# Dengzhi-USTC/A-robust-registration-loss

Measured on AMD Instinct MI355X. Metric: point-pairs/sec for loss fwd+bwd at B=8, N=M=4096, higher is better.
Workload: dtype f32

## Files before the change

a-robust-registration-loss_amd/csrc/rrl_cull.hip:

```cpp
#include <stdio.h>
#include <stdlib.h>

#include "rrl_ws.h"

#include "rrl_tree.h"
#include "rrl_chamfer_walk.h"


struct BuildArgs {
    const float *tri1, *tri2;
    const float *R, *t;
    float *tri1_out;
    float *ptri1, *ptri2;
    float4 *crec1, *crec2;
    float *apart;
    float4 *p0s1, *p0s2;
    int32_t *idx1, *idx2;
    float4 *grp1, *grp2;
    uint32_t *pmax;
    uint4 *zero_base;
    size_t zero_vec4;
    uint4 *g1;
    size_t g1_vec4;
    uint4 *z2;
// ... 577 lines not shown
        g.scale[c] = ext > 0.0f && ext < 3.0e38f ? 15.999f / ext : 0.0f;
    }
    g.p2 = fmaxf(fmaxf(red[0][6], red[1][6]), fmaxf(red[2][6], red[3][6]));
    return g;
}

__device__ __forceinline__ unsigned grid_cell(const CellGrid &g, const float4 r) {
    const float p[3] = {r.x, r.y, r.z};
    unsigned q[3];
#pragma unroll
    for (int c = 0; c < 3; ++c) {
        float v = (p[c] - g.mn[c]) * g.scale[c];
        q[c] = v >= 15.0f ? 15u : (v > 0.0f ? (unsigned)v : 0u);
    }
    return hilbert_cell(q[0], q[1], q[2]);
}

__global__ __launch_bounds__(256) void big_hist_kernel(const BuildArgs a, unsigned *__restrict__ histg) {
    __shared__ float red[4][8];
    const int cloud = blockIdx.z, b = blockIdx.y;
    const int n = cloud ? a.M : a.N;
    if ((int)blockIdx.x * 256 >= n) return;
    const int ng = (n + GRP - 1) / GRP;
    const float4 *crec = (cloud ? a.crec2 : a.crec1) + (size_t)b * ng * GRP;
    const CellGrid g = load_grid(a, cloud, b, n, red);
    if (blockIdx.x == 0 && threadIdx.x == 0) a.pmax[cloud * a.B + b] = __float_as_uint(g.p2);
    const int f = blockIdx.x * 256 + threadIdx.x;
    if (f < n) atomicAdd(&histg[((size_t)(cloud * a.B + b) * 2) * SORT_CELLS + grid_cell(g, crec[f])], 1u);
}

__global__ __launch_bounds__(256) void big_scatter_kernel(const BuildArgs a, unsigned *__restrict__ histg) {
    __shared__ float red[4][8];
    __shared__ unsigned base[SORT_CELLS];
    __shared__ unsigned wsum[4];
    const int cloud = blockIdx.z, b = blockIdx.y, tid = threadIdx.x, lane = tid & 63, wave = tid >> 6;
    const int n = cloud ? a.M : a.N;
    if ((int)blockIdx.x * 256 >= n) return;
    const int ng = (n + GRP - 1) / GRP;
    const float4 *crec = (cloud ? a.crec2 : a.crec1) + (size_t)b * ng * GRP;
    const int npad = (n + SGT - 1) / SGT * SGT;
    float4 *p0s = (cloud ? a.p0s2 : a.p0s1) + (size_t)b * npad;
    int32_t *idx = (cloud ? a.idx2 : a.idx1) + (size_t)b * npad;
    unsigned *cnt = histg + ((size_t)(cloud * a.B + b) * 2) * SORT_CELLS, *cur = cnt + SORT_CELLS;
    const int f = blockIdx.x * 256 + tid;
    const float4 r = f < n ? crec[f] : make_float4(0.0f, 0.0f, 0.0f, 0.0f);
    {
        unsigned h[16], tsum = 0;
#pragma unroll
        for (int k = 0; k < 16; ++k) { h[k] = cnt[16 * tid + k]; tsum += h[k]; }
        const unsigned inc = (unsigned)wave_incl_scan((int)tsum);
        if (lane == 63) wsum[wave] = inc;
        __syncthreads();
        unsigned run = inc - tsum;
        for (int w = 0; w < wave; ++w) run += wsum[w];
#pragma unroll
        for (int k = 0; k < 16; ++k) { base[16 * tid + k] = run; run += h[k]; }
    }
    const CellGrid g = load_grid(a, cloud, b, n, red);
    if (f < n) {
        const unsigned c = grid_cell(g, r);
        const unsigned s = base[c] + atomicAdd(&cur[c], 1u);
        p0s[s] = r;
        idx[s] = f;
    }
    if (blockIdx.x == 0)
        for (int s = n + tid; s < npad; s += 256) { p0s[s] = make_float4(0.0f, 0.0f, 0.0f, 0.0f); idx[s] = 0; }
}

__global__ __launch_bounds__(256) void big_sphere_kernel(const BuildArgs a) {
    const int cloud = blockIdx.z, b = blockIdx.y;
    const int n = cloud ? a.M : a.N;
    const int nsg = (n + SGT - 1) / SGT;
    const int hh = blockIdx.x * 256 + threadIdx.x;
    if (hh >= nsg * 2 * SGG) return;
    const float4 *r = (cloud ? a.p0s2 : a.p0s1) + (size_t)b * nsg * SGT;
    half_tree([&](int s_) { return r[s_]; }, hh, n, (cloud ? a.grp2 : a.grp1) + (size_t)b * nsg * NODE);
}

typedef const float __attribute__((address_space(4))) * kptr;
typedef const int __attribute__((address_space(4))) * kiptr;

static BuildArgs make_build_args(const float *tri1, const float *tri2, void *ws, const WsLayout &w, int B, int N, int M,
                                 int clouds, const RrlXform *xf, const float *line, int L, const RrlCall &o, bool chunked);
static unsigned rrl_chain_spin_limit(void) {
    static long v = -1;
    if (v < 0) { const char *e = getenv("RRL_CHAIN_SPIN"); v = e ? atol(e) : (1l << 18); if (v < 0 || v > 0x7fffffffl) v = 1l << 18; }
    return (unsigned)v;
}

namespace scan8 {
#include "rrl_cull_scan.inc"
}
#undef SPW
#undef SG_BITS
#undef HF_BITS
#undef WPB
#undef LPW
#undef ROWS
#undef WCCAP
#undef QA_CAP
#undef QC_CAP
#undef CULL_REGLINES
#ifndef SCAN16_QA_CAP
#define SCAN16_QA_CAP 384
#endif
#ifndef SCAN16_QC_CAP
#define SCAN16_QC_CAP 256
#endif
#ifndef SCAN16_WCCAP
#define SCAN16_WCCAP 128
#endif
namespace scan16 {
#define SPW 16
#define CULL_REGLINES 1
#define QA_CAP SCAN16_QA_CAP
#define QC_CAP SCAN16_QC_CAP
#define WCCAP SCAN16_WCCAP
#include "rrl_cull_scan.inc"
}
static_assert(scan8::kWPB == scan16::kWPB && scan8::kLPW == scan16::kLPW, "one line tiling for both variants");

struct CullGeom {
    int waves, spw, tiles, slices;
    bool fat, may_ride;
};
static CullGeom cull_geometry(int B, int N, int M, int L, int clouds, const RrlCall &o) {
    constexpr int WPB_ = scan8::kWPB, LPW_ = scan8::kLPW;
    const int nmax = clouds == 2 && M > N ? M : N;
    const int nsgmax = (nmax + SGT - 1) / SGT;
    const int lw = (L + LPW_ - 1) / LPW_;
    int waves = lw < WPB_ ? lw : WPB_, spw = scan8::kSPW;
    auto wgs = [&]() { return (long)clouds * B * ((lw + waves - 1) / waves) * ((nsgmax + spw - 1) / spw); };
    bool fat = (long)clouds * B * ((lw + waves - 1) / waves) * ((nsgmax + 15) / 16) >= 896 && lw >= WPB_;
    if (const char *e = getenv("RRL_CULL_FAT")) fat = e[0] == '1' ? (nsgmax > 8) : (e[0] == '0' ? false : fat);
    if (fat) spw = scan16::kSPW;
    while (!fat && wgs() < 768 && spw > 1) spw >>= 1;
    const bool may_ride = o.rider && !o.counters && (clouds == 2 || o.tar_ws) && lw >= WPB_ && B <= 32767 && N > 0 && M > 0;
    while (!fat && !may_ride && wgs() < 256 && waves > 2) waves >>= 1;
#ifdef RRL_EXPERIMENT
    if (const char *e = getenv("RRL_CULL_GEOM")) {
        int w_ = 0, s_ = 0;
        if (sscanf(e, "%d,%d", &w_, &s_) == 2 && w_ >= 1 && w_ <= WPB_ && s_ >= 1 && s_ <= scan16::kSPW) {
            waves = w_ < lw ? w_ : lw; spw = s_; fat = s_ > scan8::kSPW;
        }
    }
#endif
    CullGeom g;
    g.waves = waves; g.spw = spw; g.fat = fat; g.may_ride = may_ride;
    g.tiles = (lw + waves - 1) / waves; g.slices = (nsgmax + spw - 1) / spw;
    return g;
}

int rrl_cull_scan_can_fuse(int B, int N, int M, int L, const RrlCall &o) {
    if (B <= 0 || N <= 0 || M <= 0 || L <= 0 || (N > M ? N : M) > SORT_CAP) return 0;
    if (o.rider || o.counters || o.problems || o.tar_ws) return 0;
    if (const char *e = getenv("RRL_CHAIN")) if (e[0] == '0') return 0;
    const CullGeom g = cull_geometry(B, N, M, L, 2, o);
    if (g.waves != scan8::kWPB) return 0;
    const int spw = g.spw, nsg1 = (N + SGT - 1) / SGT, nsg2 = (M + SGT - 1) / SGT;
    const int nrec_b = (int)(((size_t)nsg1 * SGT + 64 * scan8::kWPB - 1) / (64 * scan8::kWPB));
    const long total = (long)B * (nrec_b + (long)g.tiles * ((nsg1 + spw - 1) / spw + (nsg2 + spw - 1) / spw));
    if (g.fat && total > 4000) return 0;
    if (nrec_b > 8 && total < 2048) return 0;
    return 1;
}

int rrl_launch_cull_scan(const float *line, void *ws, const WsLayout &w, int B, int N, int M, int L,
// ... 186 lines not shown
```

a-robust-registration-loss_amd/csrc/rrl_sparse.hip:

```cpp
#include <stdlib.h>
#include <string.h>

#include "rrl_ws.h"

#define FIX_SHIFT 40

#ifdef RRL_STAMPS
__device__ unsigned long long g_stamps[32];
#define STAMP(i) do { if (threadIdx.x == 0 && blockIdx.x == 0 && blockIdx.y == 0 && blockIdx.z == 0) g_stamps[i] = wall_clock64(); } while (0)
extern "C" int rrl_debug_stamps(unsigned long long *out) {
    return hipMemcpyFromSymbol(out, HIP_SYMBOL(g_stamps), sizeof(unsigned long long) * 32) == hipSuccess ? 0 : -1;
}
__device__ unsigned long long g_wstamps[12 * 2048];
#define STAMPW(i) do { if ((threadIdx.x & 63) == 0) { const unsigned wg_ = blockIdx.x + gridDim.x * (blockIdx.y + gridDim.y * blockIdx.z); \
    if (wg_ < 2048u) g_wstamps[(i) * 2048 + wg_] = wall_clock64(); } } while (0)
extern "C" int rrl_debug_wstamps(unsigned long long *out, int clear) {
    if (clear) { void *p_ = nullptr; if (hipGetSymbolAddress(&p_, HIP_SYMBOL(g_wstamps)) != hipSuccess) return -1; return hipMemset(p_, 0, sizeof(unsigned long long) * 12 * 2048) == hipSuccess ? 0 : -1; }
    return hipMemcpyFromSymbol(out, HIP_SYMBOL(g_wstamps), sizeof(unsigned long long) * 12 * 2048) == hipSuccess ? 0 : -1;
}
__device__ unsigned long long g_pstamps[8 * 2048];
#define STAMPP(i) do { if ((threadIdx.x & 63) == 0) { const unsigned wg_ = blockIdx.x + gridDim.x * (blockIdx.y + gridDim.y * blockIdx.z); \
    if (wg_ < 2048u) g_pstamps[(i) * 2048 + wg_] = wall_clock64(); } } while (0)
extern "C" int rrl_debug_pstamps(unsigned long long *out, int clear) {
    if (clear) { void *p_ = nullptr; if (hipGetSymbolAddress(&p_, HIP_SYMBOL(g_pstamps)) != hipSuccess) return -1; return hipMemset(p_, 0, sizeof(unsigned long long) * 8 * 2048) == hipSuccess ? 0 : -1; }
    return hipMemcpyFromSymbol(out, HIP_SYMBOL(g_pstamps), sizeof(unsigned long long) * 8 * 2048) == hipSuccess ? 0 : -1;
}
#define STAMPC(i) STAMPP(i)
#else
#define STAMP(i)
#define STAMPW(i)
#define STAMPP(i)
#endif
#include "rrl_sampler.h"

#include "rrl_stage_pair.inc"

static PairArgs pair_args(const float *tri1, const float *tri2, const float *line, void *ws, const WsLayout &w, int B, int N,
                          int M, int L, int s_m, int s_n, int e_m, int e_n, bool tally = true, const void *tar_ws = nullptr,
                          int Bt = 0) {
    PairArgs a;
    a.mhist = tally ? w.u32(ws, RRL_WS_MHIST) : nullptr;
    a.mctl = tally ? w.u32(ws, RRL_WS_MCTL) : nullptr;
    a.tri1 = tri1;
    a.tri2 = tri2;
    a.line = line;
    a.count1 = w.i32(ws, RRL_WS_COUNT1); a.hit1 = w.i32(ws, RRL_WS_HIT1);
    a.count2 = tar_ws ? w.i32(tar_ws, RRL_WS_COUNT2) : w.i32(ws, RRL_WS_COUNT2);
    a.hit2 = tar_ws ? w.i32(tar_ws, RRL_WS_HIT2) : w.i32(ws, RRL_WS_HIT2);
    a.kj = w.u8(ws, RRL_WS_KJ);
    a.sel_out = w.i32(ws, RRL_WS_SEL); a.nsel = w.i32(ws, RRL_WS_NSEL);
    a.hs1 = w.i32(ws, RRL_WS_HS1); a.hs2 = w.i32(ws, RRL_WS_HS2);
    a.w1 = w.f32(ws, RRL_WS_W1); a.w2 = w.f32(ws, RRL_WS_W2);
    a.Q1 = (float4 *)w.f32(ws, RRL_WS_Q1); a.Q2 = (float4 *)w.f32(ws, RRL_WS_Q2);
    a.D = w.f32(ws, RRL_WS_D); a.dc = w.f32(ws, RRL_WS_VALS);
    a.kjc = w.u8(ws, RRL_WS_KJC); a.blkcnt = w.i32(ws, RRL_WS_BLKCNT);
    a.lidc = w.u32(ws, RRL_WS_LIDC);
    a.vlist = w.f32(ws, RRL_WS_VLIST); a.vlcnt = w.i32(ws, RRL_WS_VLCNT);
    a.B = B; a.N = N; a.M = M; a.L = L;
    a.s_m = s_m; a.s_n = s_n; a.e_m = e_m; a.e_n = e_n;
    a.st1 = 9; a.st2 = 9;
    a.Bt = Bt;
    a.xcd_align = B % 8 == 0 && xcd_align_on();
    a.zc1 = a.zc2 = nullptr;
    return a;
}

static int line_pair_dist_impl(const float *tri1, const float *tri2, const float *line, void *ws, size_t ws_bytes, int B,
                               int N, int M, int L, int s_m, int s_n, int e_m, int e_n, const RrlCall &o, void *stream) {
    if (!tri1 || !tri2 || !line || !ws || B < 0 || N < 0 || M < 0 || L < 0 || L >= (1 << 24)) return RRL_E_ARG;
    if (s_m < 1 || s_n < 1 || e_m > RRL_MAX_HITS + 1 || e_n > RRL_MAX_HITS + 1) return RRL_E_RANGE;
    WsLayout w(B, N, M, L);
    if (ws_bytes < w.total) return RRL_E_WS;
    if (B == 0 || L == 0) return 0;
    PairArgs pa = pair_args(tri1, tri2, line, ws, w, B, N, M, L, s_m, s_n, e_m, e_n, true, o.tar_ws);
    pa.Bt = o.problems;
    if (o.plan.leave_clean) { pa.zc1 = w.i32(ws, RRL_WS_COUNT1); pa.zc2 = w.i32(ws, RRL_WS_COUNT2); }
    if (o.plan.reduce != RRL_RED_TAIL) pa.vlist = nullptr;
    if (o.plan.count_rides) {
        RrlCountRider *cr = o.count_rider;
        const int ctiles = (cr->n + 1023) / 1024;
        const CountKArgs c = {cr->rng_state, cr->r, cr->centers, cr->aabb2, cr->rows, cr->accept, cr->n_rows, cr->n,
                              cr->rounds, rrl_sample_prefilter(), ctiles, cr->rounds};
        const int pgx = (L + 1023) / 1024;
        hipLaunchKernelGGL(pair_count_kernel, dim3((unsigned)(ctiles * cr->rounds + pgx * B)), dim3(1024), 0,
                           (hipStream_t)stream, pa, c, pgx);
        RRL_LAUNCH_CHECK();
        cr->done = 1;
        return 0;
    }
    hipLaunchKernelGGL(line_pair_dist_kernel, dim3((unsigned)((L + 1023) / 1024), (unsigned)B), dim3(1024), 0,
                       (hipStream_t)stream, pa);
    RRL_LAUNCH_CHECK();
    return 0;
}

extern "C" int rrl_line_pair_dist_ex(const float *tri1, const float *tri2, const float *line,
                                     void *ws, size_t ws_bytes, int B, int N, int M, int L, int s_m,
                                     int s_n, int e_m, int e_n, int pool, const rrl_opts *opts, void *stream) {
    RrlCall o = rrl_resolve_opts(opts);
    rrl_plan(o, B, N, M, L, pool, RRL_SCAN_CULL, nullptr, nullptr, RRL_WANT_STAGE);
    return line_pair_dist_impl(tri1, tri2, line, ws, ws_bytes, B, N, M, L, s_m, s_n, e_m, e_n, o, stream);
}
extern "C" int rrl_line_pair_dist(const float *tri1, const float *tri2, const float *line,
                                  void *ws, size_t ws_bytes, int B, int N, int M, int L, int s_m,
                                  int s_n, int e_m, int e_n, int pool, void *stream) {
    return rrl_line_pair_dist_ex(tri1, tri2, line, ws, ws_bytes, B, N, M, L, s_m, s_n, e_m, e_n, pool, nullptr, stream);
}

#include "rrl_stage_reduce.inc"
#include "rrl_stage_tail.inc"

static int g_reduce_mode = -1;
extern "C" int rrl_set_reduce_mode(int mode) {
    if (mode < 0 || mode > 3) return RRL_E_ARG;
    g_reduce_mode = mode;
    return 0;
}
static int default_reduce_mode() {
    if (g_reduce_mode < 0) {
        const char *e = getenv("RRL_REDUCE");
        g_reduce_mode = !e ? 0 : (e[0] == 's' ? 1 : (e[0] == 't' ? 2 : (e[0] == 'x' ? 3 : 0)));
    }
    return g_reduce_mode;
}
static bool default_deterministic();
RrlCall rrl_resolve_opts(const rrl_opts *p) {
    RrlCall o{};
    rrl_opts v;
    memset(&v, 0, sizeof v);
    v.reduce_mode = v.deterministic = v.sort_parts = v.scan_variant = -1;
    if (p && p->struct_bytes >= 8) memcpy(&v, p, (size_t)p->struct_bytes < sizeof v ? (size_t)p->struct_bytes : sizeof v);
    o.flags = v.flags;
    o.reduce_mode = v.reduce_mode >= 0 && v.reduce_mode <= 3 ? v.reduce_mode : default_reduce_mode();
    o.deterministic = v.deterministic >= 0 ? (v.deterministic ? 1 : 0) : (default_deterministic() ? 1 : 0);
    o.sort_parts = v.sort_parts >= 0 && v.sort_parts <= 16 ? v.sort_parts : rrl_default_sort_parts();
    const int sv = v.scan_variant;
    o.scan_variant = (sv == 0 || sv == 1 || sv == 2 || sv == 4 || sv == 8) ? sv : rrl_default_scan_variant();
    o.order1 = v.order1;
    o.order2 = v.order2;
    if (v.scan_counters) { o.counters = (unsigned long long *)v.scan_counters; o.counter_rows = v.scan_counter_rows; }
    else rrl_default_scan_counters(&o.counters, &o.counter_rows);
    o.rider = v.chamfer;
    o.payload = v.payload;
    o.problems = v.problems > 0 ? v.problems : 0;
    o.chain_left = v.chain_left;
    return o;
}
static long g_spin_limit = -1;
extern "C" int rrl_set_spin_limit(long long polls) {
    if (polls < 0 || polls > 0xffffffffll) return RRL_E_ARG;
    g_spin_limit = (long)polls;
    return 0;
}
static unsigned spin_limit() {
    if (g_spin_limit < 0) {
        const char *e = getenv("RRL_SPIN_LIMIT");
        g_spin_limit = e ? atol(e) : (1l << 18);
        if (g_spin_limit < 0) g_spin_limit = 1l << 18;
    }
    return (unsigned)g_spin_limit;
}
static long xchg_capacity() {
    static long cap[64];
    int dev = 0;
    if (hipGetDevice(&dev) != hipSuccess || dev < 0 || dev >= 64) return 256;
    if (cap[dev] == 0) {
        hipDeviceProp_t p;
        int per_cu = 0;
        long c = 256;
        if (hipGetDeviceProperties(&p, dev) == hipSuccess &&
            hipOccupancyMaxActiveBlocksPerMultiprocessor(&per_cu, loss_reduce_tiled_kernel, 256, 0) == hipSuccess && per_cu > 0)
            c = (long)p.multiProcessorCount * per_cu;
#ifdef RRL_EXPERIMENT
        if (const char *e = getenv("RRL_XCHG_CAPACITY")) c = atol(e);
#endif
        cap[dev] = c < 1 ? 1 : (c > 4096 ? 4096 : c);
    }
    return cap[dev];
}
static long tail_max_wg() {
    static long v = -1;
    if (v < 0) {
        const char *e = nullptr;
#ifdef RRL_EXPERIMENT
        e = getenv("RRL_TAIL_MAX_WG");
#endif
        v = e ? atol(e) : 256;
        if (v < 1) v = 256;
    }
    return v;
}
static int reduce_kind(int mode, int B, int nblk, int pool, bool with_bwd) {
    if (pool || mode == 1) return RRL_RED_SINGLE;
    const bool xchg_ok = (long)B * nblk <= xchg_capacity();
    if (mode == 3) return xchg_ok && nblk >= 1 ? RRL_RED_XCHG : RRL_RED_SINGLE;
    const bool tail_ok = nblk <= TAIL_MAX_TILES && (long)B * nblk <= tail_max_wg();
    if (mode == 2 && tail_ok && nblk >= 1) return RRL_RED_TAIL;
    if (mode == 0 && tail_ok && with_bwd && nblk >= 2) return RRL_RED_TAIL;
    return xchg_ok && nblk >= 2 ? RRL_RED_XCHG : RRL_RED_SINGLE;
}
int rrl_cull_scan_can_fuse(int B, int N, int M, int L, const RrlCall &o);

int rrl_plan(RrlCall &o, int B, int N, int M, int L, int pool, int mode, const void *target_ws, const RrlXform *xf, int want) {
    RrlPlan &p = o.plan;
    p = RrlPlan{};
    const bool stage = want == RRL_WANT_STAGE, sorted = rrl_sorted_layout(N, M);
    const int nblk = (L + 1023) / 1024;
    p.scan_mode = mode == RRL_SCAN_CULL && !sorted ? RRL_SCAN_AUTO : mode;
    p.clouds = target_ws ? 1 : 2;
    const bool cull = p.scan_mode == RRL_SCAN_CULL;
    o.tar_ws = target_ws;
    o.xf = xf;
    if (stage) o.flags = 0;
    else if (o.problems >= B) o.problems = 0;
    if (!stage && o.problems > 0 && (B % o.problems != 0 || !xf || pool || target_ws || !cull || N <= 0 || M <= 0)) return RRL_E_ARG;
    if (o.prepared() && (!cull || (p.clouds == 2 && !o.order2 && !(o.flags & RRL_F_TARGET_KEPT)))) o.order1 = o.order2 = nullptr;
    p.build_clouds = o.target_kept() ? 1 : p.clouds;
    p.lmax_ready = !stage && sorted && B > 0 && (p.clouds == 2 && M > N ? M : N) > 0 && L > 0;
    const bool tile = !stage && L >= 1 && L <= 1024 && !pool && B > 0 && o.reduce_mode < 2;
    const bool ride = (want == RRL_WANT_DIRECT || (want == RRL_WANT_SCATTER && (tile || nblk >= 2))) && B > 0 && L > 0 &&
                      !o.deterministic;
    p.reduce = tile ? RRL_RED_TILE : reduce_kind(o.reduce_mode, B, nblk, pool, ride);
    p.tail_rpl2 = p.reduce == RRL_RED_TAIL && TAIL_LANES / nblk >= 48;
    p.bwd_rides = ride && (p.reduce == RRL_RED_TILE || p.reduce == RRL_RED_TAIL);
    p.payload_in_reduce = (want == RRL_WANT_SCATTER || want == RRL_WANT_SCATTER2) && o.payload && !p.bwd_rides && B > 0 &&
                          L > 1024 && p.reduce == RRL_RED_XCHG;
    const bool chain_path = B > 0 && L > 1024 && !pool && p.clouds == 2 && !o.problems && cull && N > 0 && M > 0 &&
                            (p.reduce == RRL_RED_XCHG || p.reduce == RRL_RED_TAIL);
    p.leave_clean = (o.flags & RRL_F_CHAIN) && chain_path;
    p.fused_build = p.leave_clean && (o.flags & RRL_F_CHAINED) && o.target_kept() && !o.count_rider && !o.write_rider &&
                    rrl_cull_scan_can_fuse(B, N, M, L, o);
    if (const RrlCountRider *cr = o.count_rider)
        p.count_rides = p.reduce != RRL_RED_TILE && B == 1 && L > 0 && cr->rounds > 0 && cr->n > 0 &&
                        (long)((cr->n + 1023) / 1024) * cr->rounds < 512 && cr->rows && cr->n_rows > 0;
    if (const RrlWriteRider *wr = o.write_rider) {
        const long wtiles = (wr->n + 1023) / 1024;
        const bool in_tail = p.bwd_rides && p.reduce == RRL_RED_TAIL, in_bwd = want == RRL_WANT_DIRECT && !p.bwd_rides;
        p.write_rides = (in_tail || in_bwd) && (!o.count_rider || p.count_rides) && B == 1 && L > 0 && wr->n > 0 &&
                        wr->rounds > 0 && wtiles * wr->rounds < 512 &&
                        sizeof(int32_t) * (size_t)wr->rounds * wtiles <= (in_tail ? 32 : 48) * 1024;
    }
    return 0;
}
struct TailBwd {
    const float *grad_loss, *src;
    float *gR, *gt, *payload;
    int transpose_r;
    float *grad_tri1;
};

static ReduceArgs reduce_args(void *ws, const WsLayout &w, float *loss, int B, int L, int s_m, int s_n, int e_m, int e_n,
                              int pool) {
    ReduceArgs r;
    r.kjc = w.u8(ws, RRL_WS_KJC); r.dc = w.f32(ws, RRL_WS_VALS); r.blkcnt = w.i32(ws, RRL_WS_BLKCNT);
    r.med_out = w.f32(ws, RRL_WS_MED); r.bcnt_out = w.i32(ws, RRL_WS_BCNT); r.bsum_out = w.i64(ws, RRL_WS_BSUM);
    r.info = w.i32(ws, RRL_WS_INFO); r.loss = loss; r.status = w.i32(ws, RRL_WS_STATUS);
    r.B = B; r.nblk = (L + 1023) / 1024;
    r.s_m = s_m; r.s_n = s_n; r.e_m = e_m; r.e_n = e_n; r.pool = pool;
    return r;
}

static int loss_reduce_impl(void *ws, size_t ws_bytes, float *loss, int B, int N, int M, int L, int s_m, int s_n, int e_m,
                            int e_n, int pool, const TailBwd *tb, const RrlCall &o, void *stream) {
    if (!ws || !loss || B < 0 || N < 0 || M < 0 || L < 0) return RRL_E_ARG;
    if (s_m < 1 || s_n < 1 || e_m > RRL_MAX_HITS + 1 || e_n > RRL_MAX_HITS + 1) return RRL_E_RANGE;
    WsLayout w(B, N, M, L);
    if (ws_bytes < w.total) return RRL_E_WS;
    if (B == 0) return 0;
    const int nblk = (L + 1023) / 1024;
    if (o.plan.reduce == RRL_RED_TAIL) {
        TailArgs t;
        t.lidc = w.u32(ws, RRL_WS_LIDC); t.dc = w.f32(ws, RRL_WS_VALS); t.blkcnt = w.i32(ws, RRL_WS_BLKCNT);
        t.vlist = w.f32(ws, RRL_WS_VLIST); t.vlcnt = w.i32(ws, RRL_WS_VLCNT);
        t.mhist = w.u32(ws, RRL_WS_MHIST); t.mctl = w.u32(ws, RRL_WS_MCTL);
        t.msum = (unsigned long long *)w.i64(ws, RRL_WS_MSUM);
        t.med_out = w.f32(ws, RRL_WS_MED); t.bcnt_out = w.i32(ws, RRL_WS_BCNT); t.bsum_out = w.i64(ws, RRL_WS_BSUM);
        t.info = w.i32(ws, RRL_WS_INFO); t.loss = loss; t.status = w.i32(ws, RRL_WS_STATUS);
        t.B = B; t.nblk = nblk; t.s_m = s_m; t.s_n = s_n; t.e_m = e_m; t.e_n = e_n;
        t.do_bwd = tb ? 1 : 0; t.N = N; t.L = L; t.transpose_r = tb ? tb->transpose_r : 0;
        t.hs1 = w.i32(ws, RRL_WS_HS1); t.w1 = w.f32(ws, RRL_WS_W1);
        t.Q1 = (const float4 *)w.f32(ws, RRL_WS_Q1); t.Q2 = (const float4 *)w.f32(ws, RRL_WS_Q2);
        t.grad_loss = tb ? tb->grad_loss : nullptr; t.src = tb ? tb->src : nullptr;
        t.gR = tb ? tb->gR : nullptr; t.gt = tb ? tb->gt : nullptr; t.payload = tb ? tb->payload : nullptr;
        t.grad_tri1 = tb ? tb->grad_tri1 : nullptr;
        t.Bt = o.problems;
        t.xcd_align = B % 8 == 0 && xcd_align_on();
        t.chain = o.plan.leave_clean ? w.u32(ws, RRL_WS_CHAIN) : nullptr;
        t.chain_flags = o.plan.fused_build;
        if (tb && o.plan.write_rides) {
            RrlWriteRider *wr = o.write_rider;
            const int wtiles = (wr->n + 1023) / 1024;
            const WriteKArgs wk = {wr->rng_state, wr->r, wr->centers, wr->accept, wr->lines, wr->filled, wr->n, wr->rounds, wtiles, wr->rounds};
            const dim3 g((unsigned)(wk.gx * wk.gy + nblk * B * TAIL_SUBS));
            const size_t lds = sizeof(int32_t) * (size_t)wk.rounds * wk.gx;
            if (t.grad_tri1) hipLaunchKernelGGL(tail_write_kernel<true>, g, dim3(TAIL_LANES), lds, (hipStream_t)stream, t, wk);
            else hipLaunchKernelGGL(tail_write_kernel<false>, g, dim3(TAIL_LANES), lds, (hipStream_t)stream, t, wk);
            wr->done = 1;
        } else {
            const dim3 g((unsigned)nblk, (unsigned)B, TAIL_SUBS);
#define RRL_TAIL(S_, R_) hipLaunchKernelGGL((loss_tail_kernel<S_, R_>), g, dim3(TAIL_LANES), 0, (hipStream_t)stream, t)
            if (t.grad_tri1) { if (o.plan.tail_rpl2) RRL_TAIL(true, 2); else RRL_TAIL(true, TAIL_RPL); }
            else { if (o.plan.tail_rpl2) RRL_TAIL(false, 2); else RRL_TAIL(false, TAIL_RPL); }
#undef RRL_TAIL
        }
        RRL_LAUNCH_CHECK();
        return 0;
    }
    if (o.plan.reduce == RRL_RED_XCHG) {
        TiledArgs t;
        t.kjc = w.u8(ws, RRL_WS_KJC); t.dc = w.f32(ws, RRL_WS_VALS); t.blkcnt = w.i32(ws, RRL_WS_BLKCNT);
        t.mhist = w.u32(ws, RRL_WS_MHIST); t.mctl = w.u32(ws, RRL_WS_MCTL); t.mcand = w.u32(ws, RRL_WS_MCAND);
        t.msum = (unsigned long long *)w.i64(ws, RRL_WS_MSUM);
        t.med_out = w.f32(ws, RRL_WS_MED); t.bcnt_out = w.i32(ws, RRL_WS_BCNT); t.bsum_out = w.i64(ws, RRL_WS_BSUM);
        t.info = w.i32(ws, RRL_WS_INFO); t.loss = loss; t.status = w.i32(ws, RRL_WS_STATUS);
        t.B = B; t.nblk = nblk; t.s_m = s_m; t.s_n = s_n; t.e_m = e_m; t.e_n = e_n;
        t.spin_limit = spin_limit();
        t.xcd_align = B % 8 == 0 && xcd_align_on();
        t.payload = o.plan.payload_in_reduce ? o.payload : nullptr;
        t.chain = o.plan.leave_clean ? w.u32(ws, RRL_WS_CHAIN) : nullptr;
        t.chain_flags = o.plan.fused_build;
        hipLaunchKernelGGL(loss_reduce_tiled_kernel, dim3((unsigned)nblk, (unsigned)B), dim3(256), 0, (hipStream_t)stream, t);
        RRL_LAUNCH_CHECK();
        return 0;
    }
    hipLaunchKernelGGL(loss_reduce_kernel, dim3((unsigned)(pool ? 1 : B)), dim3(1024), sizeof(int) * (size_t)(nblk + 1),
                       (hipStream_t)stream, reduce_args(ws, w, loss, B, L, s_m, s_n, e_m, e_n, pool));
    RRL_LAUNCH_CHECK();
    return 0;
}

extern "C" int rrl_loss_reduce_ex(void *ws, size_t ws_bytes, float *loss, int B, int N, int M, int L,
                                  int s_m, int s_n, int e_m, int e_n, int pool, const rrl_opts *opts, void *stream) {
    RrlCall o = rrl_resolve_opts(opts);
    rrl_plan(o, B, N, M, L, pool, RRL_SCAN_CULL, nullptr, nullptr, RRL_WANT_STAGE);
    return loss_reduce_impl(ws, ws_bytes, loss, B, N, M, L, s_m, s_n, e_m, e_n, pool, nullptr, o, stream);
}
extern "C" int rrl_loss_reduce(void *ws, size_t ws_bytes, float *loss, int B, int N, int M, int L,
                               int s_m, int s_n, int e_m, int e_n, int pool, void *stream) {
    return rrl_loss_reduce_ex(ws, ws_bytes, loss, B, N, M, L, s_m, s_n, e_m, e_n, pool, nullptr, stream);
}

__global__ void rows_blkcnt_kernel(int32_t *__restrict__ blkcnt, int nblk, int nrows) {
    const int t = blockIdx.x * blockDim.x + threadIdx.x;
    if (t < nblk) blkcnt[t] = min(1024, nrows - 1024 * t);
}

extern "C" int rrl_loss_reduce_rows(const float *rows16, const uint8_t *kj, int nrows, int32_t *blkcnt_scratch, float *loss,
                                    float *med, int32_t *bcnt, int64_t *bsum, int32_t *info, const int32_t *status,
                                    int s_m, int s_n, int e_m, int e_n, void *stream) {
    if (!rows16 || !kj || !blkcnt_scratch || !loss || !med || !bcnt || !bsum || !info || !status || nrows < 0) return RRL_E_ARG;
    if (s_m < 1 || s_n < 1 || e_m > RRL_MAX_HITS + 1 || e_n > RRL_MAX_HITS + 1) return RRL_E_RANGE;
    const int nblk = nrows > 0 ? (nrows + 1023) / 1024 : 1;
    hipLaunchKernelGGL(rows_blkcnt_kernel, dim3((unsigned)((nblk + 255) / 256)), dim3(256), 0, (hipStream_t)stream, blkcnt_scratch,
                       nblk, nrows);
    ReduceArgs r;
    r.kjc = kj; r.dc = rows16; r.blkcnt = blkcnt_scratch;
    r.med_out = med; r.bcnt_out = bcnt; r.bsum_out = bsum; r.info = info; r.loss = loss; r.status = status;
    r.B = 1; r.nblk = nblk; r.s_m = s_m; r.s_n = s_n; r.e_m = e_m; r.e_n = e_n; r.pool = 0;
    hipLaunchKernelGGL(loss_reduce_kernel, dim3(1), dim3(1024), sizeof(int) * (size_t)(nblk + 1), (hipStream_t)stream, r);
    RRL_LAUNCH_CHECK();
    return 0;
}

#include "rrl_stage_bwd.inc"

static int g_deterministic = -1;
extern "C" int rrl_set_deterministic(int on) {
    g_deterministic = on ? 1 : 0;
    return 0;
}
static bool default_deterministic() {
// ... 10 lines not shown
    a.hs1 = w.i32(ws, RRL_WS_HS1); a.hs2 = w.i32(ws, RRL_WS_HS2); a.bcnt = w.i32(ws, RRL_WS_BCNT); a.info = w.i32(ws, RRL_WS_INFO);
    a.w1 = w.f32(ws, RRL_WS_W1); a.w2 = w.f32(ws, RRL_WS_W2); a.D = w.f32(ws, RRL_WS_D); a.med = w.f32(ws, RRL_WS_MED);
    a.grad_loss = grad_loss;
    a.Q1 = (const float4 *)w.f32(ws, RRL_WS_Q1); a.Q2 = (const float4 *)w.f32(ws, RRL_WS_Q2);
    a.g1 = g1; a.g2 = g2; a.N = N; a.M = M; a.L = L;
    a.fx = nullptr; a.fxbits = 0; a.fxB = 0;
    return a;
}

static int scat_fx_bits_host(int L) {
    int lg = 1;
    while ((1 << lg) < L && lg < 30) ++lg;
    return 62 - lg;
}

static int loss_backward_impl(const float *tri1, const float *tri2, const void *ws,
                              size_t ws_bytes, const float *grad_loss, float *grad_tri1,
                              float *grad_tri2, int B, int N, int M, int L, int pool, bool zero1,
                              void *stream, bool deterministic = false) {
    if (!tri1 || !tri2 || !ws || !grad_loss || !grad_tri1) return RRL_E_ARG;
    if (B < 0 || N < 0 || M < 0 || L < 0) return RRL_E_ARG;
    WsLayout w(B, N, M, L);
    if (ws_bytes < w.total) return RRL_E_WS;
    hipStream_t s = (hipStream_t)stream;
    int rc;
    if (zero1 && (rc = rrl_fill(grad_tri1, 0u, sizeof(float) * 9 * (size_t)B * N, s))) return rc;
    if (grad_tri2 && (rc = rrl_fill(grad_tri2, 0u, sizeof(float) * 9 * (size_t)B * M, s))) return rc;
    if (B == 0 || L == 0) return 0;
    ScatArgs sa = scat_args(ws, w, grad_loss, grad_tri1, grad_tri2, N, M, L);
    if (deterministic && (N + M) > 0) {
        sa.fx = (unsigned long long *)((char *)const_cast<void *>(ws) + w.off[RRL_WS_GFIX]);
        sa.fxbits = scat_fx_bits_host(L);
        sa.fxB = B;
        if ((rc = rrl_fill(sa.fx, 0u, 8 * (size_t)B * (N + M) * 9 + 8 * (size_t)B, s))) return rc;
    }
    hipLaunchKernelGGL(loss_bwd_kernel, dim3((unsigned)((L + 1023) / 1024), (unsigned)B, BWDS_SUBS), dim3(256), 0, s, sa, B, pool,
                       B % 8 == 0 && xcd_align_on() ? 1 : 0);
    RRL_LAUNCH_CHECK();
    if (sa.fx) {
        const int nmax = grad_tri2 && M > N ? M : N;
        hipLaunchKernelGGL(scatter_fix_to_float_kernel, dim3((unsigned)(((size_t)nmax * 9 + 255) / 256), (unsigned)B, grad_tri2 ? 2u : 1u),
                           dim3(256), 0, s, sa, B, pool);
        RRL_LAUNCH_CHECK();
    }
    return 0;
}

extern "C" int rrl_loss_backward(const float *tri1, const float *tri2, const void *ws,
                                 size_t ws_bytes, const float *grad_loss, float *grad_tri1,
                                 float *grad_tri2, int B, int N, int M, int L, int pool,
                                 void *stream) {
    return loss_backward_impl(tri1, tri2, ws, ws_bytes, grad_loss, grad_tri1, grad_tri2, B, N, M, L,
                              pool, true, stream, default_deterministic());
}

int rrl_fused_backward(int B, int N, int M);
int rrl_launch_reg_bwd(const float *src, const float *R, float *g1, float *grad_src, float *partial,
                       float *gR, float *gt, float *payload, const float *loss, const int32_t *info,
                       int32_t *done, int B, int N, int transpose_r, hipStream_t s);

extern "C" size_t rrl_workspace_bytes(int B, int N, int M, int L) { return WsLayout(B, N, M, L).total; }

extern "C" int rrl_workspace_layout(int B, int N, int M, int L, size_t *offsets) {
    if (!offsets || B < 0 || N < 0 || M < 0 || L < 0) return RRL_E_ARG;
    WsLayout w(B, N, M, L);
    for (int i = 0; i < RRL_WS_FIELDS; ++i) offsets[i] = w.off[i];
    return 0;
}

int rrl_tri_prepare_clouds(const float *tri1, const float *tri2, void *ws, size_t ws_bytes, int B,
                           int N, int M, int L, int clouds, const RrlXform *xf, const float *line, const RrlCall &o,
                           void *stream);
int rrl_line_tri_scan_clouds(const float *line, void *ws, size_t ws_bytes, int B, int N, int M, int L,
                             int mode, int chunk, int clouds, int lmax_ready, const RrlCall &o, void *stream);

static int loss_forward_impl(const float *tri1, const float *tri2, const float *line, void *ws,
                             size_t ws_bytes, float *loss, int B, int N, int M, int L, int s_m,
                             int s_n, int e_m, int e_n, int pool, int chunk, RrlCall o, void *stream,
                             const TailBwd *tb = nullptr) {
    if (!tri1 || !tri2 || !line || !ws || !loss) return RRL_E_ARG;
    if (s_m < 1 || s_n < 1 || e_m > RRL_MAX_HITS + 1 || e_n > RRL_MAX_HITS + 1) return RRL_E_RANGE;
    if (o.tar_ws == ws) return RRL_E_ARG;
    const RrlPlan &p = o.plan;
    if (o.chain_left) *o.chain_left = p.leave_clean | (p.fused_build << 1);
    o.tri1_in = tri1;
    int rc;
    RrlRange step("rrl forward");
    if (!p.fused_build) {
        RrlRange r("K1' records + sort + tree");
        if ((rc = rrl_tri_prepare_clouds(tri1, tri2, ws, ws_bytes, B, N, M, L, p.build_clouds, o.xf, line, o, stream))) return rc;
    }
    {
        RrlRange r("K1 line<->triangle scan");
        if ((rc = rrl_line_tri_scan_clouds(line, ws, ws_bytes, B, N, M, L, p.scan_mode, chunk, p.clouds, p.lmax_ready, o, stream)))
            return rc;
    }
    if (p.reduce == RRL_RED_TILE) {
        RrlRange r("K2 + K3 + K4 (single tile)");
        WsLayout w(B, N, M, L);
        if (ws_bytes < w.total) return RRL_E_WS;
        const PairArgs pa = pair_args(tri1, tri2, line, ws, w, B, N, M, L, s_m, s_n, e_m, e_n, false, o.tar_ws, o.problems);
        const ReduceArgs ra = reduce_args(ws, w, loss, B, L, s_m, s_n, e_m, e_n, 0);
        const hipStream_t s = (hipStream_t)stream;
        if (tb && tb->grad_tri1) {
            hipLaunchKernelGGL(pair_reduce_scatter_kernel, dim3((unsigned)B), dim3(1024), sizeof(int) * 2, s, pa, ra,
                               scat_args(ws, w, tb->grad_loss, tb->grad_tri1, nullptr, N, M, L), tb->payload, w.u32(ws, RRL_WS_MCTL));
        } else if (tb) {
            SoloBwd sb;
            sb.kj = w.u8(ws, RRL_WS_KJ); sb.sel = w.i32(ws, RRL_WS_SEL); sb.nsel = w.i32(ws, RRL_WS_NSEL);
            sb.hs1 = w.i32(ws, RRL_WS_HS1); sb.bcnt = w.i32(ws, RRL_WS_BCNT); sb.info = w.i32(ws, RRL_WS_INFO);
            sb.w1 = w.f32(ws, RRL_WS_W1); sb.D = w.f32(ws, RRL_WS_D); sb.med = w.f32(ws, RRL_WS_MED);
            sb.grad_loss = tb->grad_loss; sb.src = tb->src; sb.loss = loss;
            sb.Q1 = (const float4 *)w.f32(ws, RRL_WS_Q1); sb.Q2 = (const float4 *)w.f32(ws, RRL_WS_Q2);
            sb.gR = tb->gR; sb.gt = tb->gt; sb.payload = tb->payload; sb.mctl = w.u32(ws, RRL_WS_MCTL);
            sb.B = B; sb.N = N; sb.L = L; sb.transpose_r = tb->transpose_r; sb.Bt = o.problems;
            hipLaunchKernelGGL(pair_reduce_bwd_kernel, dim3((unsigned)B), dim3(1024), sizeof(int) * 2, s, pa, ra, sb);
        } else {
            hipLaunchKernelGGL(pair_reduce_kernel, dim3((unsigned)B), dim3(1024), sizeof(int) * 2, s, pa, ra);
        }
        RRL_LAUNCH_CHECK();
        return 0;
    }
    {
        RrlRange r("K2 per-line distances");
        if ((rc = line_pair_dist_impl(tri1, tri2, line, ws, ws_bytes, B, N, M, L, s_m, s_n, e_m, e_n, o, stream))) return rc;
    }
    RrlRange r("K3+K4 median + Welsch reduce");
    return loss_reduce_impl(ws, ws_bytes, loss, B, N, M, L, s_m, s_n, e_m, e_n, pool, tb, o, stream);
}

extern "C" int rrl_loss_forward_ex(const float *tri1, const float *tri2, const float *line,
                                   void *ws, size_t ws_bytes, float *loss, int B, int N, int M,
                                   int L, int s_m, int s_n, int e_m, int e_n, int pool, int mode,
                                   int chunk, const void *target_ws, const rrl_opts *opts, void *stream) {
    RrlCall o = rrl_resolve_opts(opts);
    const int rc = rrl_plan(o, B, N, M, L, pool, mode, target_ws, nullptr, RRL_WANT_FORWARD);
    return rc ? rc : loss_forward_impl(tri1, tri2, line, ws, ws_bytes, loss, B, N, M, L, s_m, s_n, e_m, e_n, pool, chunk, o, stream);
}
extern "C" int rrl_loss_forward_cached(const float *tri1, const float *tri2, const float *line,
                                       void *ws, size_t ws_bytes, float *loss, int B, int N, int M,
                                       int L, int s_m, int s_n, int e_m, int e_n, int pool, int mode,
                                       int chunk, const void *target_ws, void *stream) {
    return rrl_loss_forward_ex(tri1, tri2, line, ws, ws_bytes, loss, B, N, M, L, s_m, s_n, e_m, e_n,
                               pool, mode, chunk, target_ws, nullptr, stream);
}

extern "C" int rrl_loss_forward_info(const float *tri1, const float *tri2, const float *line, void *ws,
                                     size_t ws_bytes, float *loss, int B, int N, int M, int L, int s_m,
                                     int s_n, int e_m, int e_n, int pool, int mode, int chunk,
                                     const void *target_ws, int32_t *host_info, void *stream) {
    if (!host_info) return RRL_E_ARG;
    int rc = rrl_loss_forward_ex(tri1, tri2, line, ws, ws_bytes, loss, B, N, M, L, s_m, s_n, e_m, e_n, pool, mode, chunk,
                                 target_ws, nullptr, stream);
    if (rc) return rc;
    const int G = pool ? 1 : B;
    if (G <= 0) return 0;
    WsLayout w(B, N, M, L);
    hipError_t e = hipMemcpyAsync(host_info, w.i32(ws, RRL_WS_INFO), sizeof(int32_t) * 4 * (size_t)G,
                                  hipMemcpyDeviceToHost, (hipStream_t)stream);
    if (e != hipSuccess) return (int)e;
    e = hipStreamSynchronize((hipStream_t)stream);
    return e == hipSuccess ? 0 : (int)e;
}

extern "C" int rrl_loss_forward(const float *tri1, const float *tri2, const float *line, void *ws,
                                size_t ws_bytes, float *loss, int B, int N, int M, int L, int s_m,
                                int s_n, int e_m, int e_n, int pool, int mode, int chunk,
                                void *stream) {
    return rrl_loss_forward_cached(tri1, tri2, line, ws, ws_bytes, loss, B, N, M, L, s_m, s_n, e_m,
                                   e_n, pool, mode, chunk, nullptr, stream);
}

extern "C" int rrl_registration_forward_ex(const float *src, const float *R, const float *t,
                                           const float *tri2, const float *line, void *ws,
                                           size_t ws_bytes, float *loss, int B, int N, int M,
                                           int L, int transpose_r, int s_m, int s_n, int e_m,
                                           int e_n, int mode, int chunk, const void *target_ws,
                                           const rrl_opts *opts, void *stream) {
    if (!src || !R || !t || !tri2 || !line || !ws || !loss) return RRL_E_ARG;
    if (B < 0 || N < 0 || M < 0 || L < 0) return RRL_E_ARG;
    WsLayout w(B, N, M, L);
    if (ws_bytes < w.total) return RRL_E_WS;
    const RrlXform xf = {src, R, t, transpose_r, 1};
    RrlCall o = rrl_resolve_opts(opts);
    const int rc = rrl_plan(o, B, N, M, L, 0, mode, target_ws, &xf, RRL_WANT_FORWARD);
    return rc ? rc : loss_forward_impl(w.f32(ws, RRL_WS_TRI1), tri2, line, ws, ws_bytes, loss, B, N, M, L, s_m, s_n, e_m, e_n, 0,
                                       chunk, o, stream);
}
extern "C" int rrl_registration_forward_cached(const float *src, const float *R, const float *t,
                                               const float *tri2, const float *line, void *ws,
                                               size_t ws_bytes, float *loss, int B, int N, int M,
                                               int L, int transpose_r, int s_m, int s_n, int e_m,
                                               int e_n, int mode, int chunk, const void *target_ws,
                                               void *stream) {
    return rrl_registration_forward_ex(src, R, t, tri2, line, ws, ws_bytes, loss, B, N, M, L, transpose_r, s_m, s_n,
                                       e_m, e_n, mode, chunk, target_ws, nullptr, stream);
}

extern "C" int rrl_registration_forward(const float *src, const float *R, const float *t,
                                        const float *tri2, const float *line, void *ws,
                                        size_t ws_bytes, float *loss, int B, int N, int M, int L,
                                        int transpose_r, int s_m, int s_n, int e_m, int e_n, int mode,
// ... 175 lines not shown
```

a-robust-registration-loss_amd/csrc/rrl_stage_pair.inc:

```
__device__ __forceinline__ void lds_barrier() { asm volatile("s_waitcnt lgkmcnt(0)\n\ts_barrier" ::: "memory"); }

#include "rrl_arith.h"

__device__ __forceinline__ void sort4(int *h, int n) {
#pragma unroll
    for (int i = 1; i < RRL_MAX_HITS; ++i)
#pragma unroll
        for (int j = RRL_MAX_HITS - 1; j >= i; --j)
            if (j < n && h[j] < h[j - 1]) { int t = h[j]; h[j] = h[j - 1]; h[j - 1] = t; }
}

#define SCAT_STRIDE 10
__device__ __forceinline__ void wave_scatter_rows(bool live, const float (&v)[9], unsigned rowkey, float *__restrict__ g1b,
                                                  float *__restrict__ g2b, unsigned *strip, int lane,
                                                  unsigned long long *fx1b = nullptr, unsigned long long *fx2b = nullptr,
                                                  double inv_unit = 0.0, int32_t *nonfinite = nullptr) {
    const unsigned long long mask = __ballot(live);
    const int nlive = __popcll(mask);
    if (nlive == 0) return;
    if (live) {
        unsigned *row = strip + __popcll(mask & ((1ull << lane) - 1ull)) * SCAT_STRIDE;
        row[0] = rowkey;
#pragma unroll
        for (int q = 0; q < 9; ++q) row[1 + q] = __float_as_uint(v[q]);
    }
    __builtin_amdgcn_fence(__ATOMIC_ACQ_REL, "wavefront");
    const int total = nlive * 9;
    for (int p = lane; p < total; p += 64) {
        const int rk = p / 9, e = p - rk * 9;
        const unsigned key = strip[rk * SCAT_STRIDE];
        const float val = __uint_as_float(strip[rk * SCAT_STRIDE + 1 + e]);
        if (fx1b) {
            if (!(fabsf(val) < INFINITY)) { atomicOr(&nonfinite[key >> 31], 1); continue; }
            const long long q = __double2ll_rn((double)val * inv_unit);
            if (q) atomicAdd(((key >> 31) ? fx2b : fx1b) + (size_t)(key & 0x7fffffffu) * 9 + e, (unsigned long long)q);
            continue;
        }
        float *dst = ((key >> 31) ? g2b : g1b) + (size_t)(key & 0x7fffffffu) * 9 + e;
        atomicAdd(dst, val);
    }
    __builtin_amdgcn_fence(__ATOMIC_ACQ_REL, "wavefront");
}

struct PairKeep {
    int total;
    int k, j;
    int f;
    float w[3];
    float4 q;
    float4 *sq;
    uint8_t *kjc_lds;
    float *dc_lds;
};

__device__ __forceinline__ void pair_hit(const float *__restrict__ tri1, const float *__restrict__ tri2,
                                         const float *__restrict__ line, const int32_t *__restrict__ hit1,
                                         const int32_t *__restrict__ hit2, int32_t *__restrict__ hs1,
                                         int32_t *__restrict__ hs2, float *__restrict__ w1,
                                         float *__restrict__ w2, float4 *__restrict__ Q1,
                                         float4 *__restrict__ Q2, float *__restrict__ D,
                                         float *__restrict__ dc_slot, float4 *s_q ,
                                         unsigned *s_mh ,
                                         int b, int N, int M, size_t gl, int k, int j, int sub, int st1,
                                         int st2, float *t2 ,
                                         int bi, size_t gli ,
                                         PairKeep *keep = nullptr) {
    const int cloud = sub >> 2, a = sub & 3;
    const int cnt = cloud ? j : k;
    float q[3] = {0.0f, 0.0f, 0.0f};
    if (a < cnt) {
        float ln[6];
        {
            const float2 *lp = (const float2 *)(line + gli * 6);
            const float2 a0 = lp[0], a1 = lp[1], a2 = lp[2];
            ln[0] = a0.x; ln[1] = a0.y; ln[2] = a1.x; ln[3] = a1.y; ln[4] = a2.x; ln[5] = a2.y;
        }
        int h[RRL_MAX_HITS];
        {
            const int4 r = cloud ? ((const int4 *)hit2)[gli] : ((const int4 *)hit1)[gl];
            const int rr[4] = {r.x, r.y, r.z, r.w};
#pragma unroll
            for (int t = 0; t < RRL_MAX_HITS; ++t) h[t] = t < cnt ? rr[t] : 0x7fffffff;
        }
        sort4(h, cnt);
        const int f = a == 0 ? h[0] : (a == 1 ? h[1] : (a == 2 ? h[2] : h[3]));
        const float *tb = cloud ? tri2 + (size_t)bi * M * st2 : tri1 + (size_t)b * N * st1;
        float w[3], c[9];
        tri_coords(tb, cloud ? st2 : st1, f, c);
        hit_weights(c, ln, w);
        inter_point(c, w, q);
        (cloud ? hs2 : hs1)[gl * RRL_MAX_HITS + a] = f;
        (cloud ? Q2 : Q1)[gl * RRL_MAX_HITS + a] = make_float4(q[0], q[1], q[2], 0.0f);
        float *wd = (cloud ? w2 : w1) + (gl * RRL_MAX_HITS + a) * 3;
#pragma unroll
        for (int cc = 0; cc < 3; ++cc) wd[cc] = w[cc];
        if (keep) {
            keep->f = f;
#pragma unroll
            for (int cc = 0; cc < 3; ++cc) keep->w[cc] = w[cc];
            keep->q = make_float4(q[0], q[1], q[2], 0.0f);
        }
    }
    s_q[sub] = make_float4(q[0], q[1], q[2], 0.0f);
    __builtin_amdgcn_fence(__ATOMIC_ACQ_REL, "wavefront");
#pragma unroll
    for (int e = 0; e < 2; ++e) {
        const int ee = 2 * sub + e, ra = ee >> 2, rb = ee & 3;
        t2[e] = INFINITY;
        if (ra < k && rb < j) {
            const float4 p1 = s_q[ra], p2 = s_q[4 + rb];
            float dx = p1.x - p2.x, dy = p1.y - p2.y, dz = p1.z - p2.z;
            float sq = dx * dx;
            sq = sq + dy * dy;
            sq = sq + dz * dz;
            D[gl * 16 + ra * j + rb] = sq;
            t2[e] = sq;
            if (s_mh) atomicAdd(&s_mh[(__float_as_uint(sq) >> 20) & 2047u], 1u);
        }
    }
    ((float2 *)dc_slot)[sub] = make_float2(t2[0], t2[1]);
}

__device__ __forceinline__ void xcd_sample_of(int lin, int gx, int &x, int &b) {
    const int slot = lin >> 3;
    x = slot % gx;
    b = (lin & 7) + 8 * (slot / gx);
}
static int xcd_align_on() {
    static int v = -1;
    if (v < 0) {
        v = 1;
#ifdef RRL_EXPERIMENT
        if (const char *e = getenv("RRL_XCD_ALIGN")) v = e[0] == '0' ? 0 : 1;
#endif
    }
    return v;
}

struct PairArgs {
    const float *tri1, *tri2, *line;
    const int32_t *count1, *hit1, *count2, *hit2;
    uint8_t *kj;
    int32_t *sel_out, *nsel, *hs1, *hs2;
    float *w1, *w2;
    float4 *Q1, *Q2;
    float *D, *dc;
    uint8_t *kjc;
    uint32_t *lidc;
    float *vlist;
    int32_t *vlcnt;
    int32_t *blkcnt;
    uint32_t *mhist, *mctl;
    int B, N, M, L, s_m, s_n, e_m, e_n, st1, st2;
    int Bt;
    int xcd_align;
    int32_t *zc1, *zc2;
};

__device__ __forceinline__ void pair_body(const PairArgs &a, int b, int tile, int ntile, PairKeep *keep = nullptr) {
    __shared__ int s_list[1024];
    __shared__ int s_wave[16];
    __shared__ int s_total;
    __shared__ float4 s_q[128][8];
    __shared__ unsigned s_mh[2048];
    __shared__ unsigned s_bc[16];
    __shared__ unsigned s_nv;
    const int tid = threadIdx.x, lane = tid & 63, wave = tid >> 6;
    const int L = a.L;
    const int bi = (a.Bt > 0 && b >= a.Bt) ? b % a.Bt : b;
    int base_reg = 0;
    if (wave == 0) STAMPP(0);
    const bool tally = a.mhist != nullptr;
    if (tally) {
        s_mh[tid] = 0u;
        s_mh[tid + 1024] = 0u;
        if (tid < 16) s_bc[tid] = 0u;
        if (tid == 0) s_nv = 0u;
    }
    {
        const int l = tile * 1024 + tid;
        bool sel = false;
        unsigned kjb = 0;
        if (l < L) {
            const size_t gl = (size_t)b * L + l;
            const int k = a.count1[gl], j = a.count2[(size_t)bi * L + l];
            if (a.zc1) { a.zc1[gl] = 0; a.zc2[gl] = 0; }
            sel = k >= a.s_m && k < a.e_m && j >= a.s_n && j < a.e_n;
            kjb = sel ? (unsigned)(k | (j << 4)) : 0u;
            a.kj[gl] = (uint8_t)kjb;
        }
        const unsigned long long mask = __ballot(sel);
        if (lane == 0) s_wave[wave] = __popcll(mask);
        if (wave == 0) STAMPP(1);
        lds_barrier();
        if (sel && tally) atomicAdd(&s_bc[((kjb & 15u) - 1u) * 4u + ((kjb >> 4) - 1u)], 1u);
        const int cw = lane < 16 ? s_wave[lane] : 0;
        const int iw = wave_incl_scan(cw);
        const int wbase = __builtin_amdgcn_readlane(iw - cw, wave), acc = __builtin_amdgcn_readlane(iw, 15);
        if (tid == 0) {
            s_total = acc;
            base_reg = acc ? atomicAdd(&a.nsel[b], acc) : 0;
        }
        if (sel) s_list[wbase + __popcll(mask & ((1ull << lane) - 1ull))] = (int)((unsigned)l | (kjb << 24));
        lds_barrier();
    }
    const size_t Lp = (size_t)ntile * 1024;
    const int total = s_total;
    STAMP(1);
    if (wave == 0) STAMPP(2);
    if (keep) {
        keep->total = total; keep->k = keep->j = 0; keep->f = 0; keep->sq = s_q[tid >> 3];
        keep->w[0] = keep->w[1] = keep->w[2] = 0.0f; keep->q = make_float4(0.0f, 0.0f, 0.0f, 0.0f);
    }
    if (tid == 0) a.blkcnt[(size_t)b * ntile + tile] = total;
    float *vl = tally && a.vlist ? a.vlist + ((size_t)b * ntile + tile) * 16384 : nullptr;
    for (int r0 = 0; r0 < total; r0 += 128) {
        const int rank = r0 + (tid >> 3), sub = tid & 7;
        float t2[2] = {INFINITY, INFINITY};
        unsigned nvl = 0;
        if (rank < total) {
            const unsigned e = (unsigned)s_list[rank];
            const int l = (int)(e & 0xffffffu), k = (int)((e >> 24) & 15u), j = (int)(e >> 28);
            const size_t gl = (size_t)b * L + l;
            const size_t slot = (size_t)b * Lp + (size_t)tile * 1024 + rank;
            if (sub == 0) {
                a.kjc[slot] = (uint8_t)(k | (j << 4));
                if (a.lidc) a.lidc[slot] = e;
            }
            pair_hit(a.tri1, a.tri2, a.line, a.hit1, a.hit2, a.hs1, a.hs2, a.w1, a.w2, a.Q1, a.Q2, a.D, a.dc + slot * 16,
                     s_q[tid >> 3], tally ? s_mh : nullptr, b, a.N, a.M, gl, k, j, sub, a.st1, a.st2, t2, bi, (size_t)bi * L + l,
                     r0 == 0 ? keep : nullptr);
            if (keep && r0 == 0) {
                keep->k = k; keep->j = j;
                if (keep->dc_lds) {
                    ((float2 *)(keep->dc_lds + rank * 16))[sub] = make_float2(t2[0], t2[1]);
                    if (sub == 0) keep->kjc_lds[rank] = (uint8_t)(k | (j << 4));
                }
            }
            nvl = (((2 * sub) >> 2) < k && ((2 * sub) & 3) < j ? 1u : 0u) | (((2 * sub + 1) >> 2) < k && ((2 * sub + 1) & 3) < j ? 2u : 0u);
        }
        if (vl) {
            const unsigned mine = (nvl & 1u) + (nvl >> 1);
            const unsigned incl = (unsigned)wave_incl_scan((int)mine);
            unsigned wbase = 0;
            if (lane == 63 && incl) wbase = atomicAdd(&s_nv, incl);
            wbase = (unsigned)__builtin_amdgcn_readlane((int)wbase, 63);
            unsigned at = wbase + incl - mine;
            if (nvl & 1u) vl[at++] = t2[0];
            if (nvl & 2u) vl[at] = t2[1];
        }
    }
    STAMP(2);
    if (wave == 0) STAMPP(3);
    if (tally) {
        lds_barrier();
        uint32_t *mh = a.mhist + (size_t)b * 2048;
#pragma unroll
        for (int q = 0; q < 2; ++q) {
            const unsigned v = s_mh[tid + 1024 * q];
            if (v) atomicAdd(&mh[tid + 1024 * q], v);
        }
        if (tid < 16 && s_bc[tid]) atomicAdd(&a.mctl[(size_t)b * 64 + tid], s_bc[tid]);
        if (vl) {
            const unsigned nv = s_nv;
            if (tid == 0) a.vlcnt[(size_t)b * ntile + tile] = (int)nv;
            if (tid < ((4u - (nv & 3u)) & 3u)) vl[nv + tid] = -1.0f;
        } else if (tid == 0 && a.vlcnt) {
            a.vlcnt[(size_t)b * ntile + tile] = -1;
        }
    }
    if (wave == 0) STAMPP(4);
    if (wave == 0) {
        const int base = __builtin_amdgcn_readfirstlane(base_reg);
        for (int i = lane; i < total; i += 64) a.sel_out[(size_t)b * L + base + i] = s_list[i] & 0xffffff;
    }
    if (wave == 0) STAMPP(5);
}

__global__ __launch_bounds__(1024) void line_pair_dist_kernel(const PairArgs a) {
    int tile = blockIdx.x, b = blockIdx.y;
    if (a.xcd_align) xcd_sample_of(tile + (int)gridDim.x * b, (int)gridDim.x, tile, b);
    pair_body(a, b, tile, (int)gridDim.x);
}

struct CountKArgs {
    const unsigned long long *rng_state;
    const float *r, *centers, *aabb2, *rows;
    unsigned long long *accept;
    int n_rows, n, rounds, prefilter, gx, gy;
};
__global__ __launch_bounds__(1024) void pair_count_kernel(const PairArgs a, const CountKArgs c, int pair_gx) {
    __shared__ SampleCountLds clds;
    const int ncount = c.gx * c.gy, lin = (int)blockIdx.x;
    if (lin < ncount) {
        sample_count_body(clds, nullptr, c.rng_state, c.r, c.centers, nullptr, c.aabb2, c.accept, 1, c.n, c.rounds, c.prefilter, 0,
                          lin % c.gx, lin / c.gx, 0, c.gx, c.rows, c.n_rows);
        return;
    }
    const int l2 = lin - ncount;
    pair_body(a, l2 / pair_gx, l2 % pair_gx, pair_gx);
}
```

a-robust-registration-loss_amd/csrc/rrl_stage_tail.inc:

```
#define TAIL_MAX_TILES 32
#define TAIL_LANES 512
#define TAIL_LINES 64
#ifndef TAIL_SUBS
#define TAIL_SUBS 4
#endif
#ifndef TAIL_RPL
#define TAIL_RPL 4
#endif
#define MCTL_LSUM 34

struct TailArgs {
    const uint32_t *lidc;
    const float *dc;
    const float *vlist;
    const int32_t *vlcnt;
    const int32_t *blkcnt;
    const uint32_t *mhist;
    uint32_t *mctl;
    unsigned long long *msum;
    float *med_out;
    int32_t *bcnt_out;
    int64_t *bsum_out;
    int32_t *info;
    float *loss;
    const int32_t *status;
    int B, nblk, s_m, s_n, e_m, e_n;
    int do_bwd, N, L, transpose_r;
    const int32_t *hs1;
    const float *w1;
    const float4 *Q1, *Q2;
    const float *grad_loss, *src;
    float *gR, *gt, *payload;
    float *grad_tri1;
    int Bt;
    int xcd_align;
    uint32_t *chain;
    int chain_flags;
};


__device__ __forceinline__ void tail_payload(const TailArgs &a, float lv) {
    atomicAdd(&a.payload[1], 1.0f);
    if (lv != lv) { atomicMax((unsigned *)&a.payload[0], 0x7fc00000u); return; }
    const unsigned long long mine = (unsigned long long)((double)lv * (double)(1ll << FIX_SHIFT) + 0.5);
    const unsigned long long old = __hip_atomic_fetch_add((unsigned long long *)(a.mctl + MCTL_LSUM), mine, __ATOMIC_RELAXED,
                                                          __HIP_MEMORY_SCOPE_AGENT);
    const float tot = (float)((double)(old + mine) * (1.0 / (double)(1ll << FIX_SHIFT)));
    atomicMax((unsigned *)&a.payload[0], __float_as_uint(tot));
}

__device__ __forceinline__ void tiled_payload(float *payload, uint32_t *mctl, float lv) {
    TailArgs t;
    t.payload = payload; t.mctl = mctl;
    tail_payload(t, lv);
}

template <bool SCATTER, int RPL>
__device__ __forceinline__ void tail_body(const TailArgs &a, int tile_in, int b_in, int sub) {
    __shared__ unsigned s_vals[MCAND_CAP];
    __shared__ unsigned s_wtot[TAIL_LANES / 64];
    __shared__ unsigned s_pick[3];
    __shared__ unsigned s_whist[128];
    __shared__ unsigned long long s_sum[32];
    __shared__ unsigned s_flag[2];
    __shared__ unsigned s_med, s_ncand;
    __shared__ int s_cnt[16];
    __shared__ int s_pref[TAIL_MAX_TILES + 1];
    __shared__ int s_vpref[TAIL_MAX_TILES + 1];
    __shared__ int s_misc[3];
    __shared__ float s_red[4][12];
    __shared__ unsigned s_scat[4][64 * SCAT_STRIDE];
    constexpr int NW = TAIL_LANES / 64, BPL = 2048 / TAIL_LANES;
    const int tid = threadIdx.x, lane = tid & 63, wave = tid >> 6;
    const int nblk = a.nblk;
    int tile = tile_in, b = b_in;
    if (a.xcd_align) xcd_sample_of(tile + nblk * b, nblk, tile, b);
    const size_t Lp = (size_t)nblk * 1024;
    uint32_t *ctl = a.mctl + (size_t)b * 64;
    const float *__restrict__ dc = a.dc;
    const uint32_t *__restrict__ lidc = a.lidc;
    const size_t slot0 = (size_t)b * Lp + (size_t)tile * 1024;
    const bool do_bwd = a.do_bwd != 0;
    constexpr bool scatter = SCATTER;
    if (wave == 0) STAMPW(0);

    const int mycnt = a.blkcnt[(size_t)b * nblk + tile];
    const int bc = tid < nblk ? a.blkcnt[(size_t)b * nblk + tid] : 0;
    const int vraw = tid < nblk ? a.vlcnt[(size_t)b * nblk + tid] : 0;
    const int vc = vraw > 0 ? (vraw + 3) >> 2 : 0;
    const int h = tid & 3;
    int r = sub * TAIL_LINES + (tid >> 2);
    unsigned kl_raw = 0u;
    float4 dr_raw = make_float4(INFINITY, INFINITY, INFINITY, INFINITY);
    if (tid < 4 * TAIL_LINES) {
        kl_raw = lidc[slot0 + r];
        dr_raw = ((const float4 *)(dc + (slot0 + r) * 16))[h];
    }
    unsigned hb[BPL];
    {
        const uint4 hq = ((const uint4 *)(a.mhist + (size_t)b * 2048))[tid];
        hb[0] = hq.x; hb[1] = hq.y; hb[2] = hq.z; hb[3] = hq.w;
        static_assert(BPL == 4, "one 16-byte load of the histogram per lane");
    }
    const unsigned bkt = tid < 16 ? ctl[tid] : 0u;
    const float gl_in0 = do_bwd ? a.grad_loss[b] : 0.0f;
    int st0;
    bool chain_tmo = false;
    if (a.chain_flags) {
        const uint4 cw = *(const uint4 *)(a.chain + 4 * (size_t)b);
        st0 = (int)cw.y;
        chain_tmo = cw.w != 0u;
    } else {
        st0 = a.status[0];
    }
    const int LPT = TAIL_LANES / nblk;
    const int vt = tid / LPT, vq = tid - vt * LPT;
    const bool vlane = vt < nblk;
    const float4 *__restrict__ vbase = (const float4 *)(a.vlist + ((size_t)b * nblk + (vlane ? vt : 0)) * 16384);
    float4 vpre[RPL];
#pragma unroll
    for (int u = 0; u < RPL; ++u)
        vpre[u] = vlane ? vbase[vq + LPT * u] : make_float4(-1.0f, -1.0f, -1.0f, -1.0f);
    if (sub * TAIL_LINES >= mycnt && !(tile == 0 && sub == 0)) return;
    bool mine_on = tid < 4 * TAIL_LINES && r < mycnt;
    unsigned kl = mine_on ? kl_raw : 0u;
    float dr[4];
    dr[0] = mine_on ? dr_raw.x : INFINITY; dr[1] = mine_on ? dr_raw.y : INFINITY;
    dr[2] = mine_on ? dr_raw.z : INFINITY; dr[3] = mine_on ? dr_raw.w : INFINITY;
    auto load_line = [&]() {
        kl = 0u;
#pragma unroll
        for (int q = 0; q < 4; ++q) dr[q] = INFINITY;
        if (mine_on) {
            kl = lidc[slot0 + r];
            const float4 v = ((const float4 *)(dc + (slot0 + r) * 16))[h];
            dr[0] = v.x; dr[1] = v.y; dr[2] = v.z; dr[3] = v.w;
        }
    };
    const float gl_in = gl_in0;
    if (tid < 32) s_sum[tid] = 0ull;
    if (tid < 2) s_flag[tid] = 0u;
    if (tid == 0) s_ncand = 0u;
    if (tid < 16) s_cnt[tid] = (int)bkt;
    __builtin_amdgcn_fence(__ATOMIC_ACQ_REL, "wavefront");
    if (vraw < 0) atomicOr(&s_flag[1], 1u);
    if (wave == 0) {
        const int incl = wave_incl_scan(bc), vincl = wave_incl_scan(vc);
        if (lane < nblk) { s_pref[lane + 1] = incl; s_vpref[lane + 1] = vincl; }
        if (lane == 0) { s_pref[0] = 0; s_vpref[0] = 0; }
        const int wl = min((bc + TAIL_LINES - 1) / TAIL_LINES, TAIL_SUBS);
        const int nl = wave_sum_i(lane < nblk ? (lane == 0 && wl == 0 ? 1 : wl) : 0);
        const int vm = (int)wave_max((float)vc);
        const int kk = lane / 4 + 1, jj = (lane & 3) + 1;
        const int cn = __popcll(__ballot(lane < 16 && bkt > 0u && kk >= a.s_m && kk < a.e_m && jj >= a.s_n && jj < a.e_n));
        if (lane == 0) { s_misc[0] = nl; s_misc[1] = vm; s_misc[2] = cn; }
    }
    int k, j;

    bool bwd_live;
    float4 q1;
    float qx[4], qy[4], qz[4], wq[3], xs[9];
    int fhit;
    auto request_line = [&]() {
        k = (int)((kl >> 24) & 15u); j = (int)(kl >> 28);
        bwd_live = do_bwd && mine_on && h < k;
        q1 = make_float4(0.0f, 0.0f, 0.0f, 0.0f);
        fhit = 0;
#pragma unroll
        for (int q = 0; q < 3; ++q) wq[q] = 0.0f;
#pragma unroll
        for (int o = 0; o < RRL_MAX_HITS; ++o) { qx[o] = qy[o] = qz[o] = 0.0f; }
        if (bwd_live) {
            const size_t gl = (size_t)b * a.L + (kl & 0xffffffu);
            fhit = a.hs1[gl * 4 + h];
            q1 = a.Q1[gl * 4 + h];
            const float *w = a.w1 + (gl * 4 + h) * 3;
#pragma unroll
            for (int q = 0; q < 3; ++q) wq[q] = w[q];
#pragma unroll
            for (int o = 0; o < RRL_MAX_HITS; ++o)
                if (o < j) { const float4 t = a.Q2[gl * 4 + o]; qx[o] = t.x; qy[o] = t.y; qz[o] = t.z; }
        }
    };
    auto request_source = [&]() {
#pragma unroll
        for (int q = 0; q < 9; ++q) xs[q] = 0.0f;
        if (bwd_live && !scatter) {
            const float *x = a.src + ((size_t)((a.Bt > 0 && b >= a.Bt) ? b % a.Bt : b) * a.N + fhit) * 9;
#pragma unroll
            for (int q = 0; q < 9; ++q) xs[q] = x[q];
        }
    };
    request_line();
    lds_barrier();
    if (wave == 0) STAMPW(8);
    const int myvc = vlane ? s_vpref[vt + 1] - s_vpref[vt] : 0;
    const int nlive = s_misc[0], vmax = s_misc[1];

    auto pick_bin = [&](unsigned rank_in, bool have_rank) -> unsigned {
        unsigned tsum = 0;
#pragma unroll
        for (int q = 0; q < BPL; ++q) tsum += hb[q];
        const unsigned incl = (unsigned)wave_incl_scan((int)tsum);
        if (have_rank) lds_barrier();
        if (lane == 63) s_wtot[wave] = incl;
        lds_barrier();
        unsigned base = 0, total = 0;
#pragma unroll
        for (int w = 0; w < NW; ++w) {
            const unsigned v = s_wtot[w];
            if (w < wave) base += v;
            total += v;
        }
        const unsigned rank = have_rank ? rank_in : (total ? (total - 1) / 2 : 0u);
        unsigned e = base + incl - tsum;
        if (rank >= e && rank < e + tsum) {
#pragma unroll
            for (int q = 0; q < BPL; ++q) {
                if (rank >= e && rank < e + hb[q]) { s_pick[0] = (unsigned)(BPL * tid + q); s_pick[1] = rank - e; s_pick[2] = hb[q]; }
                e += hb[q];
            }
        }
        lds_barrier();
        return total;
    };
    const unsigned n = pick_bin(0u, false);
    if (wave == 0) STAMPW(1);
    if (n == 0) {
        if (tid < 16) a.bcnt_out[b * 16 + tid] = 0;
        if (tid < 32) a.bsum_out[(size_t)b * 32 + tid] = 0;
        if (tid == 0) {
            a.med_out[b] = 0.0f;
            a.loss[b] = 0.0f;
            a.info[b * 4 + 0] = 0; a.info[b * 4 + 1] = 0; a.info[b * 4 + 2] = 0; a.info[b * 4 + 3] = st0;
            if (chain_tmo) a.loss[b] = __builtin_nanf("");
            if (a.chain) *(uint4 *)(a.chain + 4 * (size_t)b) = make_uint4(0u, 0u, 0u, 0u);
        }
        return;
    }
    const unsigned bin = s_pick[0], r1 = s_pick[1], pop = s_pick[2];
    unsigned prefix = bin << 20;

    auto stream_rows = [&](bool pre, auto &&after_issue, auto &&fn) {
        bool first = true;
        for (int g0 = 0; g0 < vmax; g0 += LPT * RPL) {
            float4 v[RPL];
#pragma unroll
            for (int u = 0; u < RPL; ++u) {
                const int g = g0 + vq + LPT * u;
                v[u] = make_float4(-1.0f, -1.0f, -1.0f, -1.0f);
                if (g < myvc) v[u] = pre && g0 == 0 ? vpre[u] : vbase[g];
            }
            if (first) { after_issue(); first = false; }
            fn(v);
        }
        if (first) after_issue();
    };
    auto each16 = [](const float4 *v, auto &&g) {
#pragma unroll
        for (int u = 0; u < RPL; ++u) {
            g(__float_as_uint(v[u].x)); g(__float_as_uint(v[u].y));
            g(__float_as_uint(v[u].z)); g(__float_as_uint(v[u].w));
        }
    };

    if (pop <= MCAND_CAP) {
        stream_rows(true, [&]() { request_source(); }, [&](const float4 *v) {
            unsigned mine = 0;
            each16(v, [&](unsigned x) { mine += (x >> 20) == bin ? 1u : 0u; });
            const unsigned incl = (unsigned)wave_incl_scan((int)mine);
            unsigned wbase = 0;
            if (lane == 63 && incl) wbase = atomicAdd(&s_ncand, incl);
            wbase = (unsigned)__builtin_amdgcn_readlane((int)wbase, 63);
            unsigned at = wbase + incl - mine;
            each16(v, [&](unsigned x) {
                if ((x >> 20) == bin) { if (at < MCAND_CAP) s_vals[at] = x; ++at; }
            });
        });
        lds_barrier();
        if (wave == 0) STAMPW(9);
        if (tid < 64) {
            const unsigned m = wave_select20(s_vals, pop, prefix, r1, s_whist, tid);
            if (tid == 0) s_med = m;
        }
        if (wave == 0) STAMPW(10);
        lds_barrier();
        prefix = s_med;
    } else {
        request_source();
        unsigned rk = r1;
        for (int pass = 1; pass <= 2; ++pass) {
            const int sh = pass == 1 ? 9 : 0, width = pass == 1 ? 11 : 9, hi = sh + width;
            const unsigned dmask = (1u << width) - 1u;
            lds_barrier();
#pragma unroll
            for (int q = 0; q < BPL; ++q) s_vals[tid + TAIL_LANES * q] = 0u;
            lds_barrier();
            const unsigned pre = prefix;
            stream_rows(false, [&]() {}, [&](const float4 *v) {
                each16(v, [&](unsigned x) {
                    if (((x ^ pre) >> hi) == 0u) atomicAdd(&s_vals[(x >> sh) & dmask], 1u);
                });
            });
            lds_barrier();
#pragma unroll
            for (int q = 0; q < BPL; ++q) hb[q] = s_vals[BPL * tid + q];
            pick_bin(rk, true);
            prefix |= s_pick[0] << sh;
            rk = s_pick[1];
        }
    }
    const float med = __uint_as_float(prefix);
    if (wave == 0) STAMPW(2);

    const int C = s_misc[2];
    auto finish = [&]() {
    STAMPW(3);
    if (lane < 32) {
        const unsigned long long v = s_sum[lane];
        if (v) atomicAdd(&a.msum[(size_t)b * 32 + lane], v);
    }
    if (lane == 32 && s_flag[1]) atomicOr(&ctl[MCTL_BAD], 1u);
    asm volatile("s_waitcnt vmcnt(0)" ::: "memory");
    STAMPW(4);
    unsigned last = 0;
    if (lane == 0)
        last = __hip_atomic_fetch_add(&ctl[MCTL_TICK2], 1u, __ATOMIC_RELAXED, __HIP_MEMORY_SCOPE_AGENT) == (unsigned)(nlive - 1) ? 1u : 0u;
    STAMPW(5);
    if (!__builtin_amdgcn_readfirstlane((int)last)) return;

    unsigned long long tot = 0ull;
    unsigned anybad = 0u;
    if (lane < 32) {
        tot = __hip_atomic_load(&a.msum[(size_t)b * 32 + lane], __ATOMIC_RELAXED, __HIP_MEMORY_SCOPE_AGENT);
        a.bsum_out[(size_t)b * 32 + lane] = (int64_t)tot;
        __hip_atomic_store(&a.msum[(size_t)b * 32 + lane], 0ull, __ATOMIC_RELAXED, __HIP_MEMORY_SCOPE_AGENT);
    } else if (lane < 48) {
        a.bcnt_out[b * 16 + lane - 32] = s_cnt[lane - 32];
    } else if (lane == 48) {
        anybad = ld_agent(&ctl[MCTL_BAD]);
    }
    const bool bad = __builtin_amdgcn_readlane((int)anybad, 48) != 0;
    const unsigned long long trow = __shfl(tot, (2 * lane) & 63), tcol = __shfl(tot, (2 * lane + 1) & 63);
    const BucketFinal f = bucket_final(trow, tcol, lane < 16 ? s_cnt[lane] : 0, lane, a.s_m, a.s_n, a.e_m, a.e_n);
    STAMPW(11);
    if (lane == 0) {
        const float accl = f.acc;
        const int Cn = f.C, nselected = f.nselected, nvalues = f.nvalues;
        const float lv = bad || chain_tmo ? __builtin_nanf("") : (Cn ? accl / (float)Cn : 0.0f);
        a.med_out[b] = med;
        a.loss[b] = lv;
        a.info[b * 4 + 0] = Cn;
        a.info[b * 4 + 1] = nselected;
        a.info[b * 4 + 2] = nvalues;
        a.info[b * 4 + 3] = st0;
        st_agent(&ctl[MCTL_TICK2], 0u); st_agent(&ctl[MCTL_BAD], 0u);
        if (a.chain) *(uint4 *)(a.chain + 4 * (size_t)b) = make_uint4(0u, 0u, 0u, 0u);
        if (do_bwd && a.payload && Cn > 0) tail_payload(a, lv);
    }
    STAMPW(6);
    };
    const bool single_chunk = mycnt <= TAIL_SUBS * TAIL_LINES;
    float acc[12];
#pragma unroll
    for (int q = 0; q < 12; ++q) acc[q] = 0.0f;
    for (int chunk = sub;; chunk += TAIL_SUBS) {
    if (chunk != sub) {
        r = chunk * TAIL_LINES + (tid >> 2);
        mine_on = tid < 4 * TAIL_LINES && r < mycnt;
        load_line();
        request_line();
        request_source();
    }
    int arg_b_own = 0, arg_a[4] = {0, 0, 0, 0};
    float er[4] = {0.0f, 0.0f, 0.0f, 0.0f};
    if (wave < 4) {
        const int jmax = (int)wave_max((float)j);
        float wr[4];
#pragma unroll
        for (int bb = 0; bb < RRL_MAX_HITS; ++bb) {
            const float d = dr[bb];
            wr[bb] = INFINITY;
            if (bb < jmax) {
                const float e = expf(-(d / med) / 2.0f);
                er[bb] = e;
                if (d < INFINITY) wr[bb] = 1.0f - e;
            }
        }
        float bestw = wr[0];
#pragma unroll
        for (int bb = 1; bb < RRL_MAX_HITS; ++bb)
            if (wr[bb] < bestw) { bestw = wr[bb]; arg_b_own = bb; }
        const float dmin = fminf(fminf(dr[0], dr[1]), fminf(dr[2], dr[3]));
        const float rowterm = dr[0] == dmin ? wr[0] : (dr[1] == dmin ? wr[1] : (dr[2] == dmin ? wr[2] : wr[3]));
        float W[16], Dm[16];
#pragma unroll
        for (int bb = 0; bb < RRL_MAX_HITS; ++bb) {
            W[0 + bb] = quad_bcast<0>(wr[bb]); W[4 + bb] = quad_bcast<1>(wr[bb]);
            W[8 + bb] = quad_bcast<2>(wr[bb]); W[12 + bb] = quad_bcast<3>(wr[bb]);
            Dm[0 + bb] = quad_bcast<0>(dr[bb]); Dm[4 + bb] = quad_bcast<1>(dr[bb]);
            Dm[8 + bb] = quad_bcast<2>(dr[bb]); Dm[12 + bb] = quad_bcast<3>(dr[bb]);
        }
        float colterm[4];
#pragma unroll
        for (int bb = 0; bb < RRL_MAX_HITS; ++bb) {
            float best = W[bb];
            int m = 0;
#pragma unroll
            for (int aa = 1; aa < RRL_MAX_HITS; ++aa)
                if (W[aa * 4 + bb] < best) { best = W[aa * 4 + bb]; m = aa; }
            arg_a[bb] = m;
            const float cmin = fminf(fminf(Dm[bb], Dm[4 + bb]), fminf(Dm[8 + bb], Dm[12 + bb]));
            colterm[bb] = Dm[bb] == cmin ? W[bb] : (Dm[4 + bb] == cmin ? W[4 + bb] : (Dm[8 + bb] == cmin ? W[8 + bb] : W[12 + bb]));
        }
        const float rt0 = quad_bcast<0>(rowterm), rt1 = quad_bcast<1>(rowterm), rt2 = quad_bcast<2>(rowterm), rt3 = quad_bcast<3>(rowterm);
        if (mine_on && h == 0) {
            float row = 0.0f, col = 0.0f;
            if (0 < k) row += rt0;
            if (1 < k) row += rt1;
            if (2 < k) row += rt2;
            if (3 < k) row += rt3;
#pragma unroll
            for (int q = 0; q < RRL_MAX_HITS; ++q)
                if (q < j) col += colterm[q];
            if (!(row <= 4.0f) || !(col <= 4.0f)) { atomicOr(&s_flag[1], 1u); row = col = 0.0f; }
            const int bi = (k - 1) * 4 + (j - 1);
            atomicAdd(&s_sum[bi * 2 + 0], (unsigned long long)((double)row * (double)(1ll << FIX_SHIFT) + 0.5));
            atomicAdd(&s_sum[bi * 2 + 1], (unsigned long long)((double)col * (double)(1ll << FIX_SHIFT) + 0.5));
        }
    }
    if (single_chunk) {
        lds_barrier();
        if (wave == NW - 1) finish();
    }
    float sv[9] = {0.0f, 0.0f, 0.0f, 0.0f, 0.0f, 0.0f, 0.0f, 0.0f, 0.0f};
    bool sc_live = false;
    if (bwd_live && C > 0) {
        const int S = s_cnt[(k - 1) * 4 + (j - 1)];
        const float wkj = expf(-0.5f * (float)abs(k - j));
        const float scale = gl_in * wkj / (float)C;
        const float inv_row = 1.0f / ((float)S * (float)k), inv_col = 1.0f / ((float)S * (float)j);
        float gq[3] = {0.0f, 0.0f, 0.0f};
#pragma unroll
        for (int o = 0; o < RRL_MAX_HITS; ++o) {
            if (o >= j) continue;
            float sw = 0.0f;
            if (arg_b_own == o) sw += inv_row;
            if (arg_a[o] == h) sw += inv_col;
            if (sw == 0.0f) continue;
            const float gD = scale * sw * er[o] / (2.0f * med);
            gq[0] += 2.0f * (q1.x - qx[o]) * gD;
            gq[1] += 2.0f * (q1.y - qy[o]) * gD;
            gq[2] += 2.0f * (q1.z - qz[o]) * gD;
        }
        if (scatter) {
#pragma unroll
            for (int kk = 0; kk < 3; ++kk) {
                const float wk = wq[kk] / 3.0f;
#pragma unroll
                for (int cc = 0; cc < 3; ++cc) sv[3 * kk + cc] = wk * gq[cc];
            }
            sc_live = true;
        } else {
#pragma unroll
        for (int kk = 0; kk < 3; ++kk) {
            const float wk = wq[kk] / 3.0f;
            float gv[3];
#pragma unroll
            for (int cc = 0; cc < 3; ++cc) gv[cc] = wk * gq[cc];
#pragma unroll
            for (int cc = 0; cc < 3; ++cc) {
                const float xc = xs[3 * kk + cc];
#pragma unroll
                for (int jj = 0; jj < 3; ++jj) acc[cc * 3 + jj] = fmaf(xc, gv[jj], acc[cc * 3 + jj]);
                acc[9 + cc] += gv[cc];
            }
        }
        }
    }
    if (scatter && wave < 4)
        wave_scatter_rows(sc_live, sv, (unsigned)fhit, a.grad_tri1 + (size_t)b * a.N * 9, nullptr, s_scat[wave], lane);
    if ((chunk + TAIL_SUBS) * TAIL_LINES >= mycnt) break;
    }
    if (do_bwd && !scatter && wave < 4) {
#pragma unroll
        for (int q = 0; q < 12; ++q) acc[q] = wave_sum(acc[q]);
        if (lane == 0)
#pragma unroll
            for (int q = 0; q < 12; ++q) s_red[wave][q] = acc[q];
    }
    __syncthreads();
#ifdef TAIL_EXP_NOFINAL
    return;
#endif
    if (wave == 1 && do_bwd && !scatter && mycnt > 0 && lane < 12) {
        const int q = lane;
        const float v = (s_red[0][q] + s_red[1][q]) + (s_red[2][q] + s_red[3][q]);
        int o = q;
        if (q < 9 && a.transpose_r) o = (q % 3) * 3 + q / 3;
        if (q < 9) atomicAdd(&a.gR[b * 9 + o], v); else atomicAdd(&a.gt[b * 3 + (q - 9)], v);
        if (a.payload) atomicAdd(&a.payload[2 + o], v);
    }
    if (wave == 0) STAMPW(7);
    if (wave != 0 || single_chunk) return;
    finish();
}

template <bool SCATTER, int RPL>
__global__ __launch_bounds__(TAIL_LANES) __attribute__((amdgpu_waves_per_eu(4, 8))) void loss_tail_kernel(const TailArgs a) {
    tail_body<SCATTER, RPL>(a, (int)blockIdx.x, (int)blockIdx.y, (int)blockIdx.z);
}

struct WriteKArgs {
    unsigned long long *rng_state;
    const float *r, *centers;
    const unsigned long long *accept;
    float *lines;
    int32_t *filled;
    int n, rounds, gx, gy;
};
template <bool SCATTER>
__global__ __launch_bounds__(TAIL_LANES) __attribute__((amdgpu_waves_per_eu(4, 8))) void tail_write_kernel(const TailArgs a,
                                                                                                          const WriteKArgs c) {
    extern __shared__ int s_tc_dyn[];
    const int nwrite = c.gx * c.gy, lin = (int)blockIdx.x;
    if (lin < nwrite) {
        sample_write_body<TAIL_LANES>(s_tc_dyn, nullptr, c.rng_state, c.r, c.centers, nullptr, nullptr, c.accept, c.lines, c.filled, 1,
                                      c.n, c.rounds, lin % c.gx, lin / c.gx, 0, c.gx, (unsigned)nwrite);
        return;
    }
    const int l2 = lin - nwrite, per = a.nblk * a.B;
    tail_body<SCATTER, TAIL_RPL>(a, l2 % a.nblk, (l2 / a.nblk) % a.B, l2 / per);
}

__global__ __launch_bounds__(1024) void pair_reduce_kernel(const PairArgs pa, const ReduceArgs ra) {
    __shared__ __attribute__((aligned(16))) float s_dct[128 * 16];
    __shared__ uint8_t s_kjct[128];
    PairKeep kp;
    kp.kjc_lds = s_kjct; kp.dc_lds = s_dct;
    pair_body(pa, (int)blockIdx.x, 0, 1, &kp);
    const bool small = kp.total <= 128;
    if (!small) __threadfence_block();
    __syncthreads();
    SoloReduce so;
    so.total = kp.total; so.kjc = small ? s_kjct : nullptr; so.dc = small ? s_dct : nullptr; so.fwave = 0;
    reduce_body(ra, (int)blockIdx.x, &so);
}
```

a-robust-registration-loss_amd/csrc/rrl_ws.h:

```cpp
#pragma once
#include "rrl_common.h"

struct WsLayout {
    size_t off[RRL_WS_FIELDS];
    size_t total, zero_bytes;
    size_t state_off, state_bytes;

    __host__ WsLayout(int B, int N, int M, int L) {
        const size_t b = (size_t)(B > 0 ? B : 0), n = (size_t)(N > 0 ? N : 0),
                     m = (size_t)(M > 0 ? M : 0), l = (size_t)(L > 0 ? L : 0);
        const size_t bytes[RRL_WS_FIELDS] = {
            4 * 4,
            4 * b,
            4 * b,
            4 * 2 * b,
            4 * b * l,
            4 * b * l,
            4 * b * l * 4,
            4 * b * l * 4,
            4 * b * n * 12,
            4 * b * m * 12,
            16 * b * ((n + 63) / 64) * 64,
            16 * b * ((m + 63) / 64) * 64,
            4 * b * ((n + 63) / 64) * 64,
// ... 12 lines not shown
            4 * b * l * 16,
            4 * b * l * 16,
            4 * b * l * 16,
            4 * b * ((l + 1023) / 1024) * 1024 * 16,
            4 * b,
            4 * b * 16,
            8 * b * 32,
            4 * b * 4,
            4 * b * n * 9,
            4 * b * n * 9,
            4 * b * 12 * ((3 * n + 1023) / 1024 + 1),
            4 * (b * 12 + 16),
            b * ((l + 1023) / 1024) * 1024,
            4 * b * ((l + 1023) / 1024 + 1),
            (n > 4096 || m > 4096) ? 4 * 2 * b * 2 * 4096 : 16,
            4 * b * n,
            4 * b * m,
            4 * b * 2048,
            4 * b * 64,
            8 * b * 32,
            4 * b * 2048,
            4 * b * 64 * 2,
            4 * b * ((l + 1023) / 1024) * 1024,
            4 * b * ((l + 1023) / 1024) * 16384,
            4 * b * ((l + 1023) / 1024 + 1),
            4 * b * 4,
            8 * b * (n + m) * 9 + 4 * 2 * b,
        };
        size_t o = 0;
        for (int i = 0; i < RRL_WS_FIELDS; ++i) {
            off[i] = o;
            o += (bytes[i] + 255) & ~(size_t)255;
            if (i == RRL_WS_COUNT2) zero_bytes = o;
            if (i == RRL_WS_MSUM) { state_off = off[RRL_WS_MHIST]; state_bytes = o - state_off; }
        }
        total = o;
    }
    __host__ float *f32(void *ws, int f) const { return (float *)((char *)ws + off[f]); }
    __host__ int32_t *i32(void *ws, int f) const { return (int32_t *)((char *)ws + off[f]); }
    __host__ uint8_t *u8(void *ws, int f) const { return (uint8_t *)((char *)ws + off[f]); }
    __host__ int64_t *i64(void *ws, int f) const { return (int64_t *)((char *)ws + off[f]); }
    __host__ uint32_t *u32(void *ws, int f) const { return (uint32_t *)((char *)ws + off[f]); }
    __host__ const float *f32(const void *ws, int f) const { return (const float *)((const char *)ws + off[f]); }
    __host__ const int32_t *i32(const void *ws, int f) const { return (const int32_t *)((const char *)ws + off[f]); }
    __host__ const uint8_t *u8(const void *ws, int f) const { return (const uint8_t *)((const char *)ws + off[f]); }
    __host__ const uint32_t *u32(const void *ws, int f) const { return (const uint32_t *)((const char *)ws + off[f]); }
};

typedef rrl_chamfer_rider RrlChamRider;

struct RrlCountRider {
    const unsigned long long *rng_state;
    const float *r, *centers, *aabb2;
    const float *rows;
    int n_rows;
    unsigned long long *accept;
    int n, rounds;
    int done;
};

struct RrlWriteRider {
    unsigned long long *rng_state;
    const float *r, *centers;
    const unsigned long long *accept;
    float *lines;
    int32_t *filled;
    int n, rounds;
    int done;
};

struct RrlXform;
enum { RRL_WANT_STAGE, RRL_WANT_FORWARD, RRL_WANT_SCATTER, RRL_WANT_SCATTER2, RRL_WANT_DIRECT };
enum { RRL_RED_SINGLE, RRL_RED_XCHG, RRL_RED_TAIL, RRL_RED_TILE };
struct RrlPlan {
    int scan_mode;
    int clouds, build_clouds;
    int lmax_ready;
    int reduce, tail_rpl2;
    int bwd_rides;
    int payload_in_reduce;
    int leave_clean;
    int fused_build;
    int count_rides, write_rides;
};
struct RrlCall {
    int flags;
    int reduce_mode;
    int deterministic;
    int sort_parts;
    int scan_variant;
    const int32_t *order1, *order2;
    unsigned long long *counters;
    long long counter_rows;
    void *clear_ptr;
    size_t clear_bytes;
    RrlChamRider *rider;
    RrlCountRider *count_rider;
    RrlWriteRider *write_rider;
    int problems;
    float *payload;
    const void *tar_ws;
    int32_t *chain_left;
    const RrlXform *xf;
    const float *tri1_in;
    RrlPlan plan;
    __host__ bool prepared() const { return order1 != nullptr; }
    __host__ bool target_kept() const { return order1 != nullptr && (flags & RRL_F_TARGET_KEPT); }
};
RrlCall rrl_resolve_opts(const rrl_opts *o);
int rrl_plan(RrlCall &o, int B, int N, int M, int L, int pool, int mode, const void *target_ws, const RrlXform *xf, int want);
inline bool rrl_sorted_layout(int N, int M) { return (N > M ? N : M) <= rrl_sort_capacity(); }
int rrl_sample_count_pass(const uint64_t *rng_state, const float *r, const float *centers, const float *aabb1, const float *aabb2,
                          int32_t *tile_counts, int B, int n, int rounds, void *stream);
int rrl_sample_write_pass(uint64_t *rng_state, const float *r, const float *centers, float *lines, int32_t *filled,
                          int32_t *tile_counts, int B, int n, int rounds, void *stream);
int rrl_sample_prefilter(void);
int rrl_registration_step_call(const float *src, const float *R, const float *t, const float *tri2, const float *line,
                               void *ws, size_t ws_bytes, float *loss, const float *grad_loss, float *gR, float *gt,
                               float *payload, int B, int N, int M, int L, int transpose_r, int s_m, int s_n, int e_m, int e_n,
                               int mode, int chunk, const void *target_ws, RrlCall o, void *stream);
int rrl_default_sort_parts(void);
void rrl_default_scan_counters(unsigned long long **buf, long long *rows);
int rrl_default_scan_variant(void);

struct RrlXform {
    const float *src, *R, *t;
    int transpose_r;
    int zero_g1;
};
```

a-robust-registration-loss_amd/rrl_hip/_lib.py:

```python
import ctypes
import os

import torch

from .build import LIB

_c = ctypes
_P = _c.c_void_p
_I = _c.c_int

_Z = _c.c_size_t
_SIGS = {
    "rrl_workspace_layout": [_I, _I, _I, _I, _P],
    "rrl_wide_workspace_layout": [_I, _I, _I, _I, _P],
    "rrl_loss_forward_wide": [_P, _P, _P, _P, _Z, _P, _Z, _P] + [_I] * 11 + [_P, _P],
    "rrl_loss_backward_wide": [_P, _Z, _P, _P, _P] + [_I] * 5 + [_P],
    "rrl_loss_forward": [_P, _P, _P, _P, _Z, _P] + [_I] * 11 + [_P],
    "rrl_loss_backward": [_P, _P, _P, _Z, _P, _P, _P] + [_I] * 5 + [_P],
    "rrl_registration_forward": [_P] * 6 + [_Z, _P] + [_I] * 11 + [_P],
    "rrl_registration_forward_cached": [_P] * 6 + [_Z, _P] + [_I] * 11 + [_P, _P],
    "rrl_loss_forward_cached": [_P, _P, _P, _P, _Z, _P] + [_I] * 11 + [_P, _P],
    "rrl_loss_forward_info": [_P, _P, _P, _P, _Z, _P] + [_I] * 11 + [_P, _P, _P],
    "rrl_registration_backward": [_P] * 4 + [_Z] + [_P] * 6 + [_I] * 5 + [_P],
    "rrl_registration_step": [_P] * 6 + [_Z] + [_P] * 5 + [_I] * 11 + [_P, _P],
    "rrl_loss_forward_ex": [_P, _P, _P, _P, _Z, _P] + [_I] * 11 + [_P, _P, _P],
    "rrl_registration_forward_ex": [_P] * 6 + [_Z, _P] + [_I] * 11 + [_P, _P, _P],
    "rrl_registration_backward_ex": [_P] * 4 + [_Z] + [_P] * 6 + [_I] * 5 + [_P, _P],
    "rrl_registration_step_ex": [_P] * 6 + [_Z] + [_P] * 5 + [_I] * 11 + [_P, _P, _P],
    "rrl_loss_step_ex": [_P] * 6 + [_Z] + [_P] * 4 + [_I] * 11 + [_P, _P, _P],
    "rrl_cloud_order": [_P, _P, _P, _Z, _I, _I, _P],
    "rrl_cloud_order_points": [_P, _P, _P, _Z, _I, _I, _P],
    "rrl_tri_prepare_ex": [_P, _P, _P, _Z, _I, _I, _I, _I, _P, _P],
    "rrl_line_tri_scan_ex": [_P, _P, _Z] + [_I] * 6 + [_P, _P],
    "rrl_loss_reduce_ex": [_P, _Z, _P] + [_I] * 9 + [_P, _P],
    "rrl_line_pair_dist_ex": [_P, _P, _P, _P, _Z] + [_I] * 9 + [_P, _P],
    "rrl_tri_prepare": [_P, _P, _P, _Z, _I, _I, _I, _I, _P],
    "rrl_line_tri_scan": [_P, _P, _Z] + [_I] * 6 + [_P],
    "rrl_line_pair_dist": [_P, _P, _P, _P, _Z] + [_I] * 9 + [_P],
    "rrl_loss_reduce": [_P, _Z, _P] + [_I] * 9 + [_P],
    "rrl_loss_reduce_rows": [_P, _P, _I, _P, _P, _P, _P, _P, _P, _P, _I, _I, _I, _I, _P],
    "rrl_shard_payload": [_P, _P, _Z, _P, _P, _P, _I, _I, _I, _I, _P],
    "rrl_set_scan_variant": [_I],
    "rrl_demo_epoch": [_P, _P],
    "rrl_set_spin_limit": [_c.c_longlong],
    "rrl_debug_occupy": [_I, _I, _c.c_longlong, _P],
    "rrl_set_deterministic": [_I],
    "rrl_set_reduce_mode": [_I],
    "rrl_set_sort_parts": [_I],
    "rrl_scan_timing_enable": [_I],
    "rrl_scan_timing_collect": [_P, _I],
    "rrl_scan_counters": [_P, _c.c_longlong],
    "rrl_chamfer_counters": [_P, _c.c_longlong],
    "rrl_chamfer_group_means": [_P, _Z, _P, _I, _I, _I, _I, _P],
    "rrl_rigid_apply_fwd": [_P, _P, _P, _P, _I, _I, _I, _I, _P],
    "rrl_rigid_bwd_blocks": [_I],
    "rrl_rigid_apply_bwd": [_P] * 7 + [_I] * 4 + [_P],
    "rrl_chamfer_fwd": [_P] * 5 + [_I] * 3 + [_P],
    "rrl_chamfer_bwd": [_P] * 7 + [_I] * 3 + [_P],
    "rrl_chamfer_tree_fwd": [_P, _P, _P, _Z, _P, _P, _P, _I, _I, _I, _P],
    "rrl_chamfer_from_loss": [_P, _P, _Z, _I, _I, _I, _I, _P, _Z, _P, _P, _P, _P],
    "rrl_chamfer_tree_fwd_ex": [_P, _P, _P, _Z, _P, _P, _P, _I, _I, _I, _P, _P, _P, _c.c_longlong, _P],
    "rrl_chamfer_from_loss_ex": [_P, _P, _Z, _I, _I, _I, _I, _P, _Z, _P, _P, _P, _P, _c.c_longlong, _P],
    "rrl_aabb": [_P, _P, _I, _I, _P],
    "rrl_box_accept": [_P, _P, _P, _P, _P, _I, _I, _P],
    "rrl_log_row": [_P, _P, _P, _P, _P, _c.c_longlong, _P, _P],
    "rrl_se3_adam_step": [_P] * 8 + [_c.c_double] * 3 + [_P] * 7 + [_c.c_longlong, _P, _P, _I, _P, _P],
    "rrl_rigid_apply_aabb": [_P, _P, _P, _P, _P, _I, _I, _I, _P],
    "rrl_se3_exp": [_P, _P, _P, _I, _P],
    "rrl_se3_exp_bwd": [_P, _P, _P, _P, _I, _P],
    "rrl_adam_gated": [_P] * 7 + [_I, _c.c_double, _c.c_double, _c.c_double, _P],
    "rrl_dense_scan": [_P, _P, _P, _P, _P, _I, _I, _I, _P],
    "rrl_fps": [_P, _P, _P, _P, _I, _I, _I, _P],
    "rrl_knn3": [_P, _P, _P, _I, _I, _I, _P],
    "rrl_sample_lines": [_P] * 8 + [_I] * 3 + [_P],
    "rrl_sample_lines_rng": [_P] * 8 + [_I] * 3 + [_P],
}
EXPORTS = sorted(list(_SIGS) + ["rrl_version", "rrl_workspace_bytes", "rrl_chamfer_workspace_bytes",
                                 "rrl_cloud_order_workspace_bytes", "rrl_wide_workspace_bytes", "rrl_sort_capacity"])

F_TARGET_KEPT = 1
F_CHAIN = 2
F_CHAINED = 4


class ChamferRider(ctypes.Structure):
    _fields_ = [("ws", _P), ("ws_bytes", _Z), ("best_x", _P), ("best_y", _P), ("value", _P), ("done", _c.c_int32)]


class Opts(ctypes.Structure):
    _fields_ = [("struct_bytes", _c.c_int32), ("flags", _c.c_int32), ("reduce_mode", _c.c_int32),
                ("deterministic", _c.c_int32), ("sort_parts", _c.c_int32), ("scan_variant", _c.c_int32),
                ("order1", _P), ("order2", _P), ("scan_counters", _P), ("scan_counter_rows", _c.c_longlong),
                ("chamfer", _P), ("payload", _P), ("problems", _c.c_int32), ("chain_left", _P)]

    def __init__(self, flags=0, reduce_mode=-1, deterministic=-1, sort_parts=-1, scan_variant=-1, order1=None,
                 order2=None, scan_counters=None, scan_counter_rows=0, chamfer=None, payload=None, problems=0,
                 chain_left=None):
        super().__init__(ctypes.sizeof(Opts), int(flags), int(reduce_mode), int(deterministic), int(sort_parts),
                         int(scan_variant), order1, order2, scan_counters, int(scan_counter_rows), chamfer, payload,
                         int(problems), chain_left)

class DemoEpochArgs(ctypes.Structure):
    _fields_ = [("struct_bytes", _c.c_int32), ("N", _c.c_int32), ("M", _c.c_int32), ("L", _c.c_int32),
                ("rounds", _c.c_int32), ("transpose_r", _c.c_int32),
                ("rng_state", _P), ("radius", _P), ("centers", _P), ("box1", _P), ("box2", _P), ("lines", _P),
                ("filled", _P), ("tile_counts", _P),
                ("src_tri", _P), ("tar_tri", _P), ("R", _P), ("T", _P), ("ws", _P), ("ws_bytes", _Z), ("loss", _P),
                ("grad_loss", _P), ("gR", _P), ("gt", _P), ("opts", _P),
                ("cham_ws", _P), ("cham_ws_bytes", _Z), ("best_x", _P), ("best_y", _P), ("cham_value", _P),
                ("xi", _P), ("m", _P), ("v", _P), ("adam_state", _P), ("lr", _P), ("b1", _c.c_double), ("b2", _c.c_double),
                ("eps", _c.c_double), ("table", _P), ("cursor", _P), ("table_rows", _c.c_longlong), ("row", _P),
                ("pipeline", _P)]


_lib = None


class RRLError(RuntimeError):
    pass


def load():
    global _lib
    if _lib is not None:
        return _lib
    if not os.path.exists(LIB):
        raise RRLError(
# ... 29 lines not shown
```

a-robust-registration-loss_amd/rrl_hip/ops.py:

```python
import ctypes
import os
import sys

import torch

from . import _lib
from ._lib import RRLError, check

SCAN_STRICT, SCAN_LAZY, SCAN_AUTO, SCAN_CULL = 0, 1, 2, 3
_MODES = {"strict": SCAN_STRICT, "lazy": SCAN_LAZY, "auto": SCAN_AUTO, "cull": SCAN_CULL}

_WS_FIELDS = [
    ("status", torch.int32, lambda B, N, M, L, G: (4,)),
    ("nvals", torch.int32, lambda B, N, M, L, G: (B,)),
    ("nsel", torch.int32, lambda B, N, M, L, G: (B,)),
    ("pmax", torch.float32, lambda B, N, M, L, G: (2, B)),
    ("count1", torch.int32, lambda B, N, M, L, G: (B, L)),
    ("count2", torch.int32, lambda B, N, M, L, G: (B, L)),
    ("hit1", torch.int32, lambda B, N, M, L, G: (B, L, 4)),
    ("hit2", torch.int32, lambda B, N, M, L, G: (B, L, 4)),
    ("ptri1", torch.float32, lambda B, N, M, L, G: (B, N, 12)),
    ("ptri2", torch.float32, lambda B, N, M, L, G: (B, M, 12)),
    ("p0s1", torch.float32, lambda B, N, M, L, G: (B, (N + 63) // 64 * 64, 4)),
    ("p0s2", torch.float32, lambda B, N, M, L, G: (B, (M + 63) // 64 * 64, 4)),
# ... 297 lines not shown
    return _p(tgt.ws)


_scratch_bytes = {}


def _scratch_size(entry, *dims):
    nb = _scratch_bytes.get((entry, *dims))
    if nb is None:
        nb = _scratch_bytes[(entry, *dims)] = int(getattr(_lib.load(), entry)(*dims))
    return nb


_sort_cap = []


def sort_capacity():
    if not _sort_cap:
        _sort_cap.append(int(_lib.load().rrl_sort_capacity()))
    return _sort_cap[0]


def cloud_order(tri):
    dev = _home(tri)
    if not isinstance(tri, torch.Tensor) or tri.dim() != 3 or tri.shape[-1] not in (3, 9):
        raise ValueError("cloud_order takes pseudo-triangles (B, n, 9) or points (B, n, 3)")
    t = _prep(tri, "tri", None, dev)
    B, n, _ = t.shape
    if n > sort_capacity():
        raise ValueError(f"clouds beyond {sort_capacity()} triangles are not sorted (the dense scan serves them)")
    order = torch.zeros(B, (n + 63) // 64 * 64, dtype=torch.int32, device=dev)
    if B == 0 or n == 0:
        return order
    ws = torch.empty(_scratch_size("rrl_cloud_order_workspace_bytes", B, n), dtype=torch.uint8, device=dev)
    _run(dev, "rrl_cloud_order" if t.shape[-1] == 9 else "rrl_cloud_order_points", _p(t), _p(order), _p(ws), ws.numel(), B, n)
    return order


def _check_order(order, B, n, dev, name):
    if order is None:
        return None
    if not (isinstance(order, torch.Tensor) and order.dtype == torch.int32 and order.is_cuda and order.device == dev
            and order.is_contiguous() and tuple(order.shape) == (B, (n + 63) // 64 * 64)):
        raise ValueError(f"{name} must be the contiguous int32 (B, 64 ceil(n / 64)) = {(B, (n + 63) // 64 * 64)} tensor of "
                         f"ops.cloud_order on the op's GPU ({dev}); got "
                         + (f"{order.dtype} {tuple(order.shape)} on {order.device}" if isinstance(order, torch.Tensor) else repr(type(order))))
    if ORDER_DEBUG and n > 0:
        srt = torch.sort(order[:, :n].to(torch.int64), dim=1).values
        if not bool((srt == torch.arange(n, device=dev)).all()):
            raise ValueError(f"{name}: every row's first n entries must be a permutation of [0, n)")
    return order


ORDER_DEBUG = os.environ.get("RRL_ORDER_DEBUG", "0") == "1"


_REDUCE = {"auto": 0, "single": 1, "tiled": 2, "xchg": 3}


class ChamferRide:

    def __init__(self, B, N, M, dev):
        nb = _scratch_size("rrl_chamfer_workspace_bytes", B, N, M)
        self.dims = (B, N, M)
        self.ws = torch.empty(nb, dtype=torch.uint8, device=dev)
        self.bx = torch.empty(B, N, dtype=torch.int64, device=dev)
        self.by = torch.empty(B, M, dtype=torch.int64, device=dev)
        self.val = torch.empty(1, device=dev)
        self.c = _lib.ChamferRider(_p(self.ws), nb, _p(self.bx), _p(self.by), _p(self.val), 0)

    @property
    def done(self):
        return bool(self.c.done)

    def arm(self):
        self.c.done = 0
        return self


def make_opts(order1=None, order2=None, target_kept=False, reduce_mode=None, deterministic=None, sort_parts=None,
              scan_variant=None, counters=None, chamfer=None, payload=None, problems=None, chain=0, chain_left=None):
    if order1 is None and order2 is None and not target_kept and reduce_mode is None and deterministic is None \
            and sort_parts is None and scan_variant is None and counters is None and chamfer is None and payload is None \
            and not problems and not chain:
        return None
    o = _lib.Opts(flags=(_lib.F_TARGET_KEPT if target_kept else 0) | int(chain),
                  chain_left=ctypes.addressof(chain_left) if chain_left is not None else None,
                  reduce_mode=-1 if reduce_mode is None else _REDUCE.get(reduce_mode, reduce_mode),
                  deterministic=-1 if deterministic is None else int(bool(deterministic)),
                  sort_parts=-1 if sort_parts is None else int(sort_parts),
                  scan_variant=-1 if scan_variant is None else int(scan_variant),
                  order1=order1.data_ptr() if order1 is not None else None,
                  order2=order2.data_ptr() if order2 is not None else None,
                  scan_counters=counters.data_ptr() if counters is not None else None,
                  scan_counter_rows=counters.shape[0] if counters is not None else 0,
                  chamfer=ctypes.addressof(chamfer.c) if chamfer is not None else None,
                  payload=payload.data_ptr() if payload is not None else None, problems=int(problems or 0))
    o.keep = (order1, order2, counters, chamfer, payload, chain_left)
    o.ride = chamfer
    return o


def _optr(opts):
    return ctypes.byref(opts) if opts is not None else None


def _arm_ride(opts):
    ride = getattr(opts, "ride", None)
    if ride is not None:
        ride.arm()
    return ride


def _keep_ride(st, ride):
    st.cham_ride = ride if (ride is not None and ride.done) else None


def loss_forward_raw(tri1, tri2, line, rng=(1, 1, 5, 5), pool=False, mode="cull", chunk=0,
                     staged=False, target_from=None, opts=None, state=None):
    lib = _lib.load()
    B, N, _ = tri1.shape
    M, L = tri2.shape[1], line.shape[1]
    G = 1 if pool else B
    s_m, s_n, e_m, e_n = _check_range(rng, "loss_forward_raw (target_from / cached forwards)")
    dev = tri1.device
    if tri2.device != dev or line.device != dev:
        raise ValueError("tri1, tri2 and line must live on the same GPU")
    if state is not None:
        if tuple(state.dims) != (B, N, M, L, G) or state.ws.device != dev:
            raise ValueError("state was made for another shape / device")
        st = state
    else:
        st = LossState(B, N, M, L, G, dev)
    st.target_state = getattr(target_from, "target_state", None) or target_from
    ws, nb = _p(st.ws), st.nbytes
    op = _optr(opts)
    ride = _arm_ride(opts)
    with _guard(dev):
        s = _stream(dev)
        if not staged:
            check(lib.rrl_loss_forward_ex(_p(tri1), _p(tri2), _p(line), ws, nb, _p(st.loss), B, N, M,
                                          L, s_m, s_n, e_m, e_n, int(pool), _MODES[mode], int(chunk),
                                          _target_ws(target_from, B, N, M, L), op, s),
                  "rrl_loss_forward")
            _keep_ride(st, ride)
            return st
        check(lib.rrl_tri_prepare_ex(_p(tri1), _p(tri2), ws, nb, B, N, M, L, op, s), "rrl_tri_prepare")
        if staged == "mixed":
            op = None
        check(lib.rrl_line_tri_scan_ex(_p(line), ws, nb, B, N, M, L, _MODES[mode], int(chunk), op, s),
              "rrl_line_tri_scan")
        check(lib.rrl_line_pair_dist_ex(_p(tri1), _p(tri2), _p(line), ws, nb, B, N, M, L, s_m, s_n, e_m,
                                        e_n, int(pool), op, s), "rrl_line_pair_dist")
        check(lib.rrl_loss_reduce_ex(ws, nb, _p(st.loss), B, N, M, L, s_m, s_n, e_m, e_n, int(pool), op, s),
              "rrl_loss_reduce")
    _keep_ride(st, ride)
    return st


def loss_forward_wide(tri1, tri2, line, rng, pool=False, mode="cull", chunk=0, opts=None):
    if _deterministic[0] or (opts is not None and opts.deterministic == 1):
        raise ValueError(_wide_refusal("deterministic-gradient mode (set_deterministic(True))"))
    (s_m, s_n, e_m, e_n), _ = _classify_range(rng)
    B, N, _ = tri1.shape
    M, L = tri2.shape[1], line.shape[1]
    G = 1 if pool else B
    dev = tri1.device
# ... 358 lines not shown
        ctx.set_materialize_grads(False)
        _IntersectionLoss.last_state = st
        return st.loss.view(-1), info, status

    @staticmethod
    def backward(ctx, g_loss, _g1, _g2):
        if g_loss is None or ctx.st is None:
            return (None,) * 12
        st, src, Rm, tri2 = ctx.st, ctx.src, ctx.Rm, ctx.tri2
        tr, want_payload, Rshape, tshape, sdev, Rdev, tdev = ctx.meta
        B, N, M, L, _ = st.dims
        if ctx.multi and ctx.needs_input_grad[0]:
            raise RRLError("a multi-pose evaluation returns dL/dR, dL/dt only (src_tri must not require grad)")
        g = g_loss if (g_loss.device == src.device and g_loss.is_contiguous()) else \
            g_loss.to(device=src.device, dtype=torch.float32).contiguous()
        if not ctx.needs_input_grad[0] and not getattr(st, "gacc_used", False):
            out = st.gacc
            st.gacc_used = True
        else:
            out = torch.empty(B * 12 + 14, dtype=torch.float32, device=src.device)
        gR, gt, payload = out[:B * 9], out[B * 9:B * 12], out[B * 12:B * 12 + 14]
        gsrc = torch.empty_like(src) if ctx.needs_input_grad[0] else None
        with _guard(src.device):
            check(_lib.load().rrl_registration_backward_ex(
                _p(src), _p(Rm), _p(tri2), _p(st.ws), st.nbytes, _p(st.loss), _p(g), _p(gsrc), _p(gR),
                _p(gt), _p(payload) if want_payload else None, B, N, M, L, tr, _optr(ctx.opts), _stream(src.device)),
                "rrl_registration_backward")
        st.payload = payload if want_payload else None
        return (gsrc.to(sdev) if gsrc is not None else None, gR.reshape(Rshape).to(Rdev),
                gt.reshape(tshape).to(tdev), None, None, None, None, None, None, None, None, None)


def registration_loss(src_tri, R, t, tar_tri, line, rng=(1, 1, 5, 5), transpose_r=True,
                      mode="cull", chunk=0, want_payload=False, target_from=None, order1=None, order2=None, opts=None,
                      chamfer=False):
    Bt = src_tri.shape[0]
    Binst = R.reshape(-1, 3, 3).shape[0]
    problems = Bt if (Binst != Bt and Bt > 0 and Binst % Bt == 0) else 0
    if problems and (target_from is not None or mode != "cull"):
        raise ValueError("a multi-pose evaluation scans its target itself, in scan mode cull")
    if opts is None and (chamfer or order1 is not None or order2 is not None or problems):
        opts = _with_ride(None, order1, order2, chamfer, Binst, src_tri.reshape(Bt, -1, 9).shape[1],
                          tar_tri.reshape(tar_tri.shape[0], -1, 9).shape[1], _home(src_tri, tar_tri, line, R, t), problems)
    return _RegistrationLoss.apply(src_tri, R, t, tar_tri, line, tuple(rng), transpose_r, mode,
                                   chunk, want_payload, target_from, opts)


class _Step:

    def __init__(self, what, src_tri, tar_tri, n_lines, rng, transpose_r, mode, chunk, prepared, src_order, tar_order,
                 chamfer, poses, chain):
        dev = _home(src_tri, tar_tri)
        self.dev = dev
        self.src = _prep(src_tri, "src_tri", 9, dev)
        self.tar = _prep(tar_tri, "tar_tri", 9, dev)
        if self.src.dim() != 3 or self.tar.dim() != 3 or self.src.shape[0] != self.tar.shape[0]:
            raise ValueError("src_tri/tar_tri must be (B, n, 9) with the same B")
        Bt, N, _ = self.src.shape
        M, L = self.tar.shape[1], int(n_lines)
        if Bt == 0 or L <= 0:
            raise ValueError(f"{what} needs a non-empty batch and line set")
        self.poses, self.Bt = int(poses), Bt
        if self.poses < 1 or (self.poses > 1 and (mode != "cull" or max(N, M) > sort_capacity())):
            raise ValueError(f"poses must be >= 1; a multi-pose step runs scan mode cull on clouds <= {sort_capacity()} "
                             "triangles")
        B = Bt * self.poses
        self.dims = (B, N, M, L)
        self.rng = _check_range(rng, what)
        self.tr, self.mode, self.chunk = int(bool(transpose_r)), _MODES[mode], int(chunk)
        self.st = LossState(B, N, M, L, B, dev)
        self.ride = ChamferRide(B, N, M, dev) if chamfer else None
        self.chamfer_value = None
        self._extra = dict(chamfer=self.ride, problems=Bt if self.poses > 1 else None)
        self.ones = torch.ones(B, dtype=torch.float32, device=dev)
        if prepared is None:
            prepared = os.environ.get("RRL_PREPARED", "1") != "0"
        self.prepared = bool(prepared) and mode == "cull" and max(N, M) <= sort_capacity()
        self._kept_key = None
        self.keep_target = True
        self.chain = bool(chain)
        self._chain_left = ctypes.c_int32(0)
        self._chain_ready = False
        self.fused = False
        self.order1 = self.order2 = None
        if self.prepared:
            self.order1 = _check_order(src_order, Bt, N, dev, "src_order") if src_order is not None else cloud_order(self.src)
            self.order2 = _check_order(tar_order, Bt, M, dev, "tar_order") if tar_order is not None else cloud_order(self.tar)
        self._lib = _lib.load()

    def invalidate_target(self):
        self._kept_key = None

    def _set_opts(self):
        kw = dict(order1=self.order1, order2=self.order2, **self._extra)
        self._opts = make_opts(**kw)
        self._opts_kept = make_opts(target_kept=True, **kw) if self.prepared else self._opts
        self._optr, self._optr_kept = _optr(self._opts), _optr(self._opts_kept)
        self._chain_ready = False
        if self.prepared:
            kw["chain_left"] = self._chain_left
            self._opts_c = (make_opts(chain=_lib.F_CHAIN, **kw), make_opts(target_kept=True, chain=_lib.F_CHAIN, **kw),
                            make_opts(target_kept=True, chain=_lib.F_CHAIN | _lib.F_CHAINED, **kw))
            self._optr_c = tuple(_optr(o) for o in self._opts_c)

    def _pick(self, chain, target_from=None):
        op, key = self._optr, None
        if self.prepared:
            key = _write_key(self.tar) if (self.keep_target and target_from is None) else None
            kept = key is not None and key == self._kept_key
            if chain:
                op = self._optr_c[2 if (kept and self._chain_ready) else (1 if kept else 0)]
            elif kept:
                op = self._optr_kept
            self._kept_key = None
        self._chain_ready = False
        self._chain_left.value = 0
        return op, key

    def _done(self, key):
        self._kept_key = key
        self._chain_ready = self.prepared and bool(self._chain_left.value & 1)
        self.fused = bool(self._chain_left.value & 2)
        self.st.counts_cleared = self._chain_ready
        _IntersectionLoss.last_state = self.st
        if self.ride is not None:
            _keep_ride(self.st, self.ride)
            self.chamfer_value = chamfer_from_state(self.st)
        return self._out


class RegistrationStep(_Step):

    ONE_CALL = os.environ.get("RRL_ONE_CALL", "1") != "0"

    def __init__(self, src_tri, tar_tri, n_lines, rng=(1, 1, 5, 5), transpose_r=True, mode="cull", chunk=0,
                 want_payload=False, prepared=None, src_order=None, tar_order=None, reduce_mode=None, deterministic=None,
                 sort_parts=None, chamfer=False, poses=1, chain=False):
        super().__init__("RegistrationStep", src_tri, tar_tri, n_lines, rng, transpose_r, mode, chunk, prepared, src_order,
                         tar_order, chamfer, poses, chain)
        self._extra.update(reduce_mode=reduce_mode, deterministic=deterministic, sort_parts=sort_parts)
        B, N, M, L = self.dims
        gacc = self.st.gacc
        self.gR, self.gt = gacc[:B * 9].view(B, 3, 3), gacc[B * 9:B * 12].view(B, 3)
        self.payload = gacc[B * 12:B * 12 + 14] if want_payload else None
        self._fixed_f = (_p(self.st.ws), self.st.nbytes, _p(self.st.loss), B, N, M, L, self.tr, *self.rng, self.mode,
                         self.chunk, None)
        self._fixed_b = (_p(self.st.ws), self.st.nbytes, _p(self.st.loss))
        self._tail_b = (None, _p(gacc[:B * 9]), _p(gacc[B * 9:B * 12]), _p(self.payload), B, N, M, L, self.tr)
        self._head_s = (_p(self.st.ws), self.st.nbytes, _p(self.st.loss))
        self._tail_s = (_p(gacc[:B * 9]), _p(gacc[B * 9:B * 12]), _p(self.payload), B, N, M, L, self.tr, *self.rng,
                        self.mode, self.chunk, None)
        self._out = (self.st.loss.view(-1), self.gR, self.gt, self.payload, self.st.info)
        self._set_opts()

    def __call__(self, R, t, line, grad_loss=None, src_tri=None, tar_tri=None, target_from=None, src_order=None,
                 tar_order=None):
        B, N, M, L = self.dims
        Bt = self.Bt
        dev = self.dev
        if src_tri is not None:
            self.src = _prep(src_tri, "src_tri", 9, dev)
        if tar_tri is not None:
            self.tar = _prep(tar_tri, "tar_tri", 9, dev)
        if tuple(self.src.shape) != (Bt, N, 9) or tuple(self.tar.shape) != (Bt, M, 9):
            raise ValueError(f"src_tri {(Bt, N, 9)} / tar_tri {(Bt, M, 9)} expected")
        if self.poses > 1 and target_from is not None:
            raise ValueError("a multi-pose step scans its target itself")
        if self.prepared and (src_tri is not None or src_order is not None or tar_tri is not None or tar_order is not None):
            if src_tri is not None or src_order is not None:
                self.order1 = _check_order(src_order, Bt, N, dev, "src_order") if src_order is not None else cloud_order(self.src)
            if tar_tri is not None or tar_order is not None:
                self.order2 = _check_order(tar_order, Bt, M, dev, "tar_order") if tar_order is not None else cloud_order(self.tar)
                self._kept_key = None
            self._set_opts()
        op, key = self._pick(self.chain and RegistrationStep.ONE_CALL and target_from is None, target_from)
        Rm, tv, ln = _prep(R, "R", None, dev), _prep(t, "t", None, dev), _prep(line, "line", 6, dev)
        if Rm.numel() != B * 9 or tv.numel() != B * 3 or tuple(ln.shape) != (Bt, L, 6):
            raise ValueError("R (poses * B, 3, 3), t (poses * B, 3), line (B, L, 6) expected")
        g = self.ones if grad_loss is None else _prep(grad_loss, "grad_loss", None, dev)
        lib, s = self._lib, _stream(dev)
        tail_s, fixed_f = self._tail_s, self._fixed_f
        if target_from is not None:
            if target_from is self.st:
                raise ValueError("target_from must be another evaluation's state")
            tws = _target_ws(target_from, B, N, M, L)
            tail_s, fixed_f = tail_s[:-1] + (tws,), fixed_f[:-1] + (tws,)
        self.st.target_state = getattr(target_from, "target_state", None) or target_from
        if self.ride is not None:
            self.ride.arm()
        with _guard(dev):
            if RegistrationStep.ONE_CALL:
                check(lib.rrl_registration_step_ex(_p(self.src), _p(Rm), _p(tv), _p(self.tar), _p(ln), *self._head_s, _p(g),
                                                   *tail_s, op, s), "rrl_registration_step")
            else:
                check(lib.rrl_registration_forward_ex(_p(self.src), _p(Rm), _p(tv), _p(self.tar), _p(ln), *fixed_f, op, s),
                      "rrl_registration_forward")
                check(lib.rrl_registration_backward_ex(_p(self.src), _p(Rm), _p(self.tar), *self._fixed_b, _p(g), *self._tail_b, op, s),
                      "rrl_registration_backward")
        return self._done(key)


class LossStep(_Step):

    def __init__(self, src_tri, tar_tri, n_lines, rng=(1, 1, 5, 5), transpose_r=True, mode="cull", chunk=0,
                 prepared=None, src_order=None, tar_order=None, chamfer=False, want_payload=False, poses=1, chain=True,
                 deterministic=None):
        super().__init__("LossStep", src_tri, tar_tri, n_lines, rng, transpose_r, mode, chunk, prepared, src_order,
                         tar_order, chamfer, poses, chain)
        B, N, M, L = self.dims
        self.grad = torch.empty(B, N, 9, dtype=torch.float32, device=self.dev)
        self.payload = self.st.gacc[B * 12:B * 12 + 14] if want_payload else None
        self._extra.update(payload=self.payload, deterministic=deterministic)
        if self.prepared:
            self._extra["chain_left"] = self._chain_left
        self._out = (self.st.loss.view(-1), self.grad, self.st.info)
        self._c_fixed = (_p(self.st.ws), self.st.nbytes, _p(self.st.loss))
        self._c_tail = (_p(self.grad), None, B, N, M, L, self.tr, *self.rng, self.mode, self.chunk, None)
        self._p_ones = _p(self.ones)
        self._set_opts()

    def __call__(self, R, t, line, grad_loss=None):
        B, N, M, L = self.dims
        dev = self.dev
        Rm = _prep(R, "R", None, dev) if R is not None else None
        tv = _prep(t, "t", None, dev) if t is not None else None
        ln = _prep(line, "line", 6, dev)
        if (Rm is None) != (tv is None) or (Rm is not None and (Rm.numel() != B * 9 or tv.numel() != B * 3)) \
                or tuple(ln.shape) != (self.Bt, L, 6) or (self.poses > 1 and Rm is None):
            raise ValueError("R (poses * B, 3, 3) and t (poses * B, 3) (or both None for poses = 1), line (B, L, 6) expected")
        g = self.ones if grad_loss is None else _prep(grad_loss, "grad_loss", None, dev)
        op, key = self._pick(self.chain)
        if self.ride is not None:
            self.ride.arm()
        with _guard(dev):
            check(self._lib.rrl_loss_step_ex(_p(self.src), _p(Rm), _p(tv), _p(self.tar), _p(ln), *self._c_fixed,
                                             self._p_ones if g is self.ones else _p(g), *self._c_tail, op, _stream(dev)),
                  "rrl_loss_step")
        return self._done(key)


def registration_step_raw(src_tri, R, t, tar_tri, line, rng=(1, 1, 5, 5), transpose_r=True, order1=None, order2=None,
                          chamfer=False):
    dev = src_tri.device
    Bt, N, _ = src_tri.shape
    M, L = tar_tri.shape[1], line.shape[1]
    B = R.shape[0]
    if not (tar_tri.shape[0] == line.shape[0] == Bt and t.shape[0] == B) or Bt == 0 or B % Bt or L <= 0:
        raise ValueError("src_tri / tar_tri / line share B_t > 0; R, t hold k * B_t poses; L > 0")
    problems = Bt if B != Bt else 0
    s_m, s_n, e_m, e_n = _check_range(rng, "registration_step_raw")
    st = LossState(B, N, M, L, B, dev)
    ride = ChamferRide(B, N, M, dev) if chamfer else None
    opts = make_opts(order1=_check_order(order1, Bt, N, dev, "order1"), order2=_check_order(order2, Bt, M, dev, "order2"),
                     chamfer=ride, problems=problems)
    gacc = st.gacc
    ones = _ones_cache.get((B, dev))
    if ones is None:
        if len(_ones_cache) > 32:
            _ones_cache.clear()
        ones = _ones_cache[(B, dev)] = torch.ones(B, dtype=torch.float32, device=dev)
    _arm_ride(opts)
    with _guard(dev):
        check(_lib.load().rrl_registration_step_ex(
            _p(src_tri), _p(R), _p(t), _p(tar_tri), _p(line), _p(st.ws), st.nbytes, _p(st.loss), _p(ones),
            _p(gacc[:B * 9]), _p(gacc[B * 9:B * 12]), None, B, N, M, L, int(transpose_r), s_m, s_n, e_m, e_n, SCAN_CULL, 0, None,
            _optr(opts), _stream(dev)), "rrl_registration_step")
    st.target_state = None
    _keep_ride(st, ride)
    _IntersectionLoss.last_state = st
    return st.loss.view(-1), gacc[:B * 9].view(B, 3, 3), gacc[B * 9:B * 12].view(B, 3), st.info, st


_ones_cache = {}


def set_deterministic(on):
    check(_lib.load().rrl_set_deterministic(int(bool(on))), "rrl_set_deterministic")
    _deterministic[0] = bool(on)


def set_reduce_mode(mode):
    check(_lib.load().rrl_set_reduce_mode(_REDUCE[mode]), "rrl_set_reduce_mode")


def set_spin_limit(polls):
    check(_lib.load().rrl_set_spin_limit(int(1 << 18 if polls is None else polls)), "rrl_set_spin_limit")


def debug_occupy(workgroups, lanes, seconds, stream=None):
    dev = require_gpu()
    raw = ctypes.c_void_p(stream.cuda_stream) if stream is not None else _stream(dev)
    check(_lib.load().rrl_debug_occupy(int(workgroups), int(lanes), int(seconds * 1e8), raw), "rrl_debug_occupy")


def set_sort_parts(parts):
    check(_lib.load().rrl_set_sort_parts(int(parts)), "rrl_set_sort_parts")


def last_state():
    return _IntersectionLoss.last_state


def scan_timing(every):
    check(_lib.load().rrl_scan_timing_enable(int(every)), "rrl_scan_timing_enable")


def scan_timing_collect(max_n=1024):
    buf = (ctypes.c_float * max_n)()
    n = _lib.load().rrl_scan_timing_collect(buf, max_n)
    return [float(buf[i]) for i in range(n)]


_counter_buf = None


def scan_counters(on, rows=1 << 17, raw=False):
    global _counter_buf
    prev = _counter_buf
    if on:
        _counter_buf = torch.zeros(int(rows), 16, dtype=torch.int64, device=require_gpu())
        check(_lib.load().rrl_scan_counters(_p(_counter_buf), int(rows)), "rrl_scan_counters")
    else:
        _counter_buf = None
        check(_lib.load().rrl_scan_counters(None, 0), "rrl_scan_counters")
    if prev is None:
        return None
    return prev if raw else prev.sum(0)


_cham_counter_buf = None


def chamfer_counters(on, raw=False, rows=1 << 19):
    global _cham_counter_buf
    prev = _cham_counter_buf
    _cham_counter_buf = torch.zeros(16 * int(rows), dtype=torch.int64, device=require_gpu()) if on else None
    check(_lib.load().rrl_chamfer_counters(_p(_cham_counter_buf), int(rows) if on else 0), "rrl_chamfer_counters")
    if prev is None:
        return None
    return prev.reshape(-1, 16) if raw else prev.reshape(-1, 16).sum(0)


class _RigidApply(torch.autograd.Function):
    @staticmethod
    def forward(ctx, x, R, t, transpose_r, channel_first):
        dev = _home(x, R, t)
        xs = _prep(x, "x", None, dev)
        Rm, tv = _prep(R, "R", None, dev), _prep(t, "t", None, dev)
        B = Rm.shape[0]
        n = xs.numel() // (3 * B)
        y = torch.empty_like(xs)
        _run(dev, "rrl_rigid_apply_fwd", _p(xs), _p(Rm), _p(tv), _p(y), B, n, int(transpose_r), int(channel_first))
        ctx.save_for_backward(xs, Rm)
        ctx.meta = (B, n, int(transpose_r), int(channel_first), x.device, R.device, t.device,
                    R.shape, t.shape)
        return y.to(x.device)

    @staticmethod
    def backward(ctx, gy):
        lib = _lib.load()
        xs, Rm = ctx.saved_tensors
        B, n, tr, cf, xdev, Rdev, tdev, Rshape, tshape = ctx.meta
        g = gy.detach().to(device=xs.device, dtype=torch.float32).contiguous()
        gx = torch.empty_like(xs) if ctx.needs_input_grad[0] else None
        gR = torch.empty(B, 3, 3, device=xs.device)
        gt = torch.empty(B, 3, device=xs.device)
        nblk = lib.rrl_rigid_bwd_blocks(n)
        partial = torch.empty(B, max(nblk, 1), 12, device=xs.device)
        _run(xs.device, "rrl_rigid_apply_bwd", _p(xs), _p(Rm), _p(g), _p(gx), _p(gR), _p(gt), _p(partial), B, n, tr, cf)
        return (gx.to(xdev) if gx is not None else None, gR.reshape(Rshape).to(Rdev),
                gt.reshape(tshape).to(tdev), None, None)
# ... 258 lines not shown
```

include/rrl.h:

```cpp
#ifndef RRL_H
#define RRL_H

#include <stddef.h>
#include <stdint.h>

#ifdef __cplusplus
extern "C" {
#endif

#define RRL_MAX_HITS 4
#define RRL_WIDE_MAX_HITS 8
#define RRL_E_ARG (-1)
#define RRL_E_RANGE (-2)
#define RRL_E_WS (-3)

#define RRL_SCAN_STRICT 0
#define RRL_SCAN_LAZY 1
#define RRL_SCAN_AUTO 2
#define RRL_SCAN_CULL 3

enum {
    RRL_WS_STATUS = 0,
    RRL_WS_NVALS,
    RRL_WS_NSEL,
// ... 129 lines not shown
                          int e_m, int e_n, int pool, int mode, int chunk, const void *target_ws,
                          int32_t *host_info, void *stream);
int rrl_set_deterministic(int on);
int rrl_registration_backward(const float *src, const float *R, const float *tri2, void *ws,
                              size_t ws_bytes, const float *loss, const float *grad_loss,
                              float *grad_src, float *gR, float *gt, float *payload, int B, int N,
                              int M, int L, int transpose_r, void *stream);

int rrl_registration_step(const float *src, const float *R, const float *t, const float *tri2,
                          const float *line, void *ws, size_t ws_bytes, float *loss, const float *grad_loss,
                          float *gR, float *gt, float *payload, int B, int N, int M, int L, int transpose_r,
                          int s_m, int s_n, int e_m, int e_n, int mode, int chunk, const void *target_ws,
                          void *stream);

size_t rrl_cloud_order_workspace_bytes(int B, int n);
int rrl_cloud_order(const float *tri, int32_t *order, void *ws, size_t ws_bytes, int B, int n, void *stream);
int rrl_cloud_order_points(const float *pts, int32_t *order, void *ws, size_t ws_bytes, int B, int n, void *stream);

int rrl_loss_forward_ex(const float *tri1, const float *tri2, const float *line, void *ws, size_t ws_bytes,
                        float *loss, int B, int N, int M, int L, int s_m, int s_n, int e_m, int e_n, int pool,
                        int mode, int chunk, const void *target_ws, const rrl_opts *opts, void *stream);
int rrl_registration_forward_ex(const float *src, const float *R, const float *t, const float *tri2,
                                const float *line, void *ws, size_t ws_bytes, float *loss, int B, int N, int M,
                                int L, int transpose_r, int s_m, int s_n, int e_m, int e_n, int mode, int chunk,
                                const void *target_ws, const rrl_opts *opts, void *stream);
int rrl_registration_backward_ex(const float *src, const float *R, const float *tri2, void *ws, size_t ws_bytes,
                                 const float *loss, const float *grad_loss, float *grad_src, float *gR, float *gt,
                                 float *payload, int B, int N, int M, int L, int transpose_r, const rrl_opts *opts,
                                 void *stream);
int rrl_registration_step_ex(const float *src, const float *R, const float *t, const float *tri2,
                             const float *line, void *ws, size_t ws_bytes, float *loss, const float *grad_loss,
                             float *gR, float *gt, float *payload, int B, int N, int M, int L, int transpose_r,
                             int s_m, int s_n, int e_m, int e_n, int mode, int chunk, const void *target_ws,
                             const rrl_opts *opts, void *stream);

int rrl_loss_step_ex(const float *tri1, const float *R, const float *t, const float *tri2, const float *line,
                     void *ws, size_t ws_bytes, float *loss, const float *grad_loss, float *grad_tri1,
                     float *grad_tri2, int B, int N, int M, int L, int transpose_r, int s_m, int s_n, int e_m,
                     int e_n, int mode, int chunk, const void *target_ws, const rrl_opts *opts, void *stream);

size_t rrl_wide_workspace_bytes(int B, int N, int M, int L);
int rrl_wide_workspace_layout(int B, int N, int M, int L, size_t *offsets);
int rrl_loss_forward_wide(const float *tri1, const float *tri2, const float *line, void *ws, size_t ws_bytes, void *wws,
                          size_t wws_bytes, float *loss, int B, int N, int M, int L, int s_m, int s_n, int e_m, int e_n,
                          int pool, int mode, int chunk, const rrl_opts *opts, void *stream);
int rrl_loss_backward_wide(const void *wws, size_t wws_bytes, const float *grad_loss, float *grad_tri1, float *grad_tri2,
                           int B, int N, int M, int L, int pool, void *stream);


int rrl_tri_prepare(const float *tri1, const float *tri2, void *ws, size_t ws_bytes, int B, int N,
                    int M, int L, void *stream);

int rrl_tri_prepare_ex(const float *tri1, const float *tri2, void *ws, size_t ws_bytes, int B, int N,
                       int M, int L, const rrl_opts *opts, void *stream);

int rrl_line_tri_scan(const float *line, void *ws, size_t ws_bytes, int B, int N, int M, int L,
                      int mode, int chunk, void *stream);

int rrl_line_tri_scan_ex(const float *line, void *ws, size_t ws_bytes, int B, int N, int M, int L,
                         int mode, int chunk, const rrl_opts *opts, void *stream);
int rrl_line_pair_dist_ex(const float *tri1, const float *tri2, const float *line, void *ws,
                          size_t ws_bytes, int B, int N, int M, int L, int s_m, int s_n, int e_m,
                          int e_n, int pool, const rrl_opts *opts, void *stream);

int rrl_line_pair_dist(const float *tri1, const float *tri2, const float *line, void *ws,
                       size_t ws_bytes, int B, int N, int M, int L, int s_m, int s_n, int e_m,
                       int e_n, int pool, void *stream);

int rrl_loss_reduce(void *ws, size_t ws_bytes, float *loss, int B, int N, int M, int L, int s_m,
                    int s_n, int e_m, int e_n, int pool, void *stream);

int rrl_loss_reduce_ex(void *ws, size_t ws_bytes, float *loss, int B, int N, int M, int L, int s_m,
                       int s_n, int e_m, int e_n, int pool, const rrl_opts *opts, void *stream);

int rrl_loss_reduce_rows(const float *rows16, const uint8_t *kj, int nrows, int32_t *blkcnt_scratch, float *loss,
                         float *med, int32_t *bcnt, int64_t *bsum, int32_t *info, const int32_t *status, int s_m,
                         int s_n, int e_m, int e_n, void *stream);

int rrl_set_reduce_mode(int mode);

int rrl_set_sort_parts(int parts);

int rrl_set_spin_limit(long long polls);
int rrl_debug_occupy(int workgroups, int lanes, long long ticks, void *stream);

int rrl_set_scan_variant(int lines_per_lane);

int rrl_scan_timing_enable(int on);
int rrl_scan_timing_collect(float *ms, int max_n);

int rrl_scan_counters(uint64_t *dev_counters, long long rows);

int rrl_shard_payload(const float *loss, const void *ws, size_t ws_bytes, const float *gR,
                      const float *gt, float *out, int B, int N, int M, int L, void *stream);

int rrl_rigid_apply_fwd(const float *x, const float *R, const float *t, float *y, int B, int n,
                        int transpose_r, int channel_first, void *stream);
int rrl_rigid_bwd_blocks(int n);
int rrl_rigid_apply_bwd(const float *x, const float *R, const float *gy, float *gx, float *gR,
                        float *gt, float *partial, int B, int n, int transpose_r,
                        int channel_first, void *stream);

int rrl_se3_exp(const float *xi, float *R, float *T, int B, void *stream);
int rrl_se3_exp_bwd(const float *xi, const float *gR, const float *gT, float *gxi, int B, void *stream);
int rrl_adam_gated(float *p, const float *g, float *m, float *v, float *state, const float *lr,
                   const int32_t *gate, int n, double b1, double b2, double eps, void *stream);

int rrl_log_row(const float *loss, const float *value, const int32_t *info, float *table,
                long long *cursor, long long nrows, float *row, void *stream);

int rrl_se3_adam_step(float *xi, const float *gR, const float *gT, float *m, float *v, float *state,
                      const float *lr, const int32_t *gate, double b1, double b2, double eps, float *R, float *T,
                      float *gxi, const float *loss, const float *value, float *table, long long *cursor,
                      long long nrows, float *row, const float *aabb_rows, int n_aabb_rows, float *box, void *stream);

typedef struct rrl_demo_epoch_args {
    int32_t struct_bytes, N, M, L, rounds, transpose_r;
    uint64_t *rng_state; const float *radius, *centers; float *box1; const float *box2; float *lines; int32_t *filled, *tile_counts;
    const float *src_tri, *tar_tri; float *R, *T; void *ws; size_t ws_bytes; float *loss; const float *grad_loss; float *gR, *gt;
    const rrl_opts *opts;
    void *cham_ws; size_t cham_ws_bytes; uint64_t *best_x, *best_y; float *cham_value;
    float *xi, *m, *v, *adam_state; const float *lr; double b1, b2, eps; float *table; long long *cursor; long long table_rows; float *row;
    int32_t *pipeline;
} rrl_demo_epoch_args;
int rrl_demo_epoch(const rrl_demo_epoch_args *args, void *stream);

int rrl_chamfer_fwd(const float *x, const float *y, uint64_t *best_x, uint64_t *best_y,
                    float *value, int B, int N, int M, void *stream);
size_t rrl_chamfer_workspace_bytes(int B, int N, int M);
int rrl_chamfer_tree_fwd(const float *x, const float *y, void *ws, size_t ws_bytes, uint64_t *best_x,
                         uint64_t *best_y, float *value, int B, int N, int M, void *stream);
int rrl_chamfer_from_loss(void *ws_src, const void *ws_tar, size_t loss_ws_bytes, int B, int N, int M,
                          int L, void *ws, size_t ws_bytes, uint64_t *best_x, uint64_t *best_y, float *value,
                          void *stream);
int rrl_chamfer_counters(uint64_t *dev_counters, long long rows);
int rrl_chamfer_group_means(const void *cham_ws, size_t cham_ws_bytes, float *values, int G, int B, int N, int M,
                            void *stream);
int rrl_chamfer_tree_fwd_ex(const float *x, const float *y, void *ws, size_t ws_bytes, uint64_t *best_x,
                            uint64_t *best_y, float *value, int B, int N, int M, const int32_t *order_x,
                            const int32_t *order_y, uint64_t *counters, long long counter_rows, void *stream);
int rrl_chamfer_from_loss_ex(void *ws_src, const void *ws_tar, size_t loss_ws_bytes, int B, int N, int M,
                             int L, void *ws, size_t ws_bytes, uint64_t *best_x, uint64_t *best_y, float *value,
                             uint64_t *counters, long long counter_rows, void *stream);
int rrl_chamfer_bwd(const float *x, const float *y, const uint64_t *best_x,
                    const uint64_t *best_y, const float *grad_value, float *gx, float *gy, int B,
                    int N, int M, void *stream);

int rrl_dense_scan(const float *tri, const float *line, float *norm_d, uint8_t *label,
                   int32_t *status, int B, int N, int L, void *stream);

int rrl_aabb(const float *v, float *aabb, int B, int n, void *stream);
int rrl_rigid_apply_aabb(const float *x, const float *R, const float *t, float *y, float *aabb, int B, int n,
                         int transpose_r, void *stream);
int rrl_box_accept(const float *lines, const float *aabb1, const float *aabb2, uint8_t *mask,
                   int32_t *hits, int B, int n, void *stream);
int rrl_sample_lines(const float *rands, const float *r, const float *centers, const float *aabb1,
                     const float *aabb2, float *lines, int32_t *filled, int32_t *tile_counts, int B,
                     int n, int rounds, void *stream);
int rrl_sample_lines_rng(uint64_t *rng_state, const float *r, const float *centers, const float *aabb1,
                         const float *aabb2, float *lines, int32_t *filled, int32_t *tile_counts, int B,
                         int n, int rounds, void *stream);

int rrl_fps(const float *pts, const int32_t *start, int32_t *out_idx, float *dist_scratch, int B,
            int n, int S, void *stream);
int rrl_knn3(const float *pts, const int32_t *query_idx, int32_t *nn, int B, int n, int S,
             void *stream);
// ... 6 lines not shown
```

Baseline: 44600 billion.

## Fuse pair and tail reduce stages into one persistent launch with flag handoff

Adds a combined pair_tail kernel. Its leading blocks run the pair stage and publish their outputs with cache-bypassing stores plus an arrival counter, and its trailing blocks run the tail reduction and backward pass. This replaces separate launches and their inter-kernel gaps with in-kernel producer/consumer synchronisation, gated by an occupancy-based capacity check. It also generalises the tail geometry to wider workgroups. The cost is spin-waiting, reliance on co-residency of producer and consumer blocks, and extra atomic-store traffic.

```diff
diff --git a/a-robust-registration-loss_amd/csrc/rrl_cull.hip b/a-robust-registration-loss_amd/csrc/rrl_cull.hip
--- a/a-robust-registration-loss_amd/csrc/rrl_cull.hip
+++ b/a-robust-registration-loss_amd/csrc/rrl_cull.hip
@@ -683,7 +683,7 @@
 
 static BuildArgs make_build_args(const float *tri1, const float *tri2, void *ws, const WsLayout &w, int B, int N, int M,
                                  int clouds, const RrlXform *xf, const float *line, int L, const RrlCall &o, bool chunked);
-static unsigned rrl_chain_spin_limit(void) {
+unsigned rrl_chain_spin_limit(void) {
     static long v = -1;
     if (v < 0) { const char *e = getenv("RRL_CHAIN_SPIN"); v = e ? atol(e) : (1l << 18); if (v < 0 || v > 0x7fffffffl) v = 1l << 18; }
     return (unsigned)v;
diff --git a/a-robust-registration-loss_amd/csrc/rrl_sparse.hip b/a-robust-registration-loss_amd/csrc/rrl_sparse.hip
--- a/a-robust-registration-loss_amd/csrc/rrl_sparse.hip
+++ b/a-robust-registration-loss_amd/csrc/rrl_sparse.hip
@@ -65,6 +65,15 @@
     return a;
 }
 
+static PairArgs call_pair_args(const float *tri1, const float *tri2, const float *line, void *ws, const WsLayout &w, int B, int N,
+                               int M, int L, int s_m, int s_n, int e_m, int e_n, const RrlCall &o) {
+    PairArgs pa = pair_args(tri1, tri2, line, ws, w, B, N, M, L, s_m, s_n, e_m, e_n, true, o.tar_ws);
+    pa.Bt = o.problems;
+    if (o.plan.leave_clean) { pa.zc1 = w.i32(ws, RRL_WS_COUNT1); pa.zc2 = w.i32(ws, RRL_WS_COUNT2); }
+    if (o.plan.reduce != RRL_RED_TAIL) pa.vlist = nullptr;
+    return pa;
+}
+
 static int line_pair_dist_impl(const float *tri1, const float *tri2, const float *line, void *ws, size_t ws_bytes, int B,
                                int N, int M, int L, int s_m, int s_n, int e_m, int e_n, const RrlCall &o, void *stream) {
     if (!tri1 || !tri2 || !line || !ws || B < 0 || N < 0 || M < 0 || L < 0 || L >= (1 << 24)) return RRL_E_ARG;
@@ -72,10 +81,7 @@
     WsLayout w(B, N, M, L);
     if (ws_bytes < w.total) return RRL_E_WS;
     if (B == 0 || L == 0) return 0;
-    PairArgs pa = pair_args(tri1, tri2, line, ws, w, B, N, M, L, s_m, s_n, e_m, e_n, true, o.tar_ws);
-    pa.Bt = o.problems;
-    if (o.plan.leave_clean) { pa.zc1 = w.i32(ws, RRL_WS_COUNT1); pa.zc2 = w.i32(ws, RRL_WS_COUNT2); }
-    if (o.plan.reduce != RRL_RED_TAIL) pa.vlist = nullptr;
+    const PairArgs pa = call_pair_args(tri1, tri2, line, ws, w, B, N, M, L, s_m, s_n, e_m, e_n, o);
     if (o.plan.count_rides) {
         RrlCountRider *cr = o.count_rider;
         const int ctiles = (cr->n + 1023) / 1024;
@@ -109,6 +115,8 @@
 
 #include "rrl_stage_reduce.inc"
 #include "rrl_stage_tail.inc"
+unsigned rrl_chain_spin_limit(void);
+#include "rrl_stage_pairtail.inc"
 
 static int g_reduce_mode = -1;
 extern "C" int rrl_set_reduce_mode(int mode) {
@@ -240,6 +248,8 @@
                         wr->rounds > 0 && wtiles * wr->rounds < 512 &&
                         sizeof(int32_t) * (size_t)wr->rounds * wtiles <= (in_tail ? 32 : 48) * 1024;
     }
+    p.pair_tail = !stage && p.reduce == RRL_RED_TAIL && !o.deterministic && !o.count_rider && !o.write_rider && B > 0 &&
+                  pair_tail_serves(B, nblk);
     return 0;
 }
 struct TailBwd {
@@ -260,6 +270,31 @@
     return r;
 }
 
+static TailArgs tail_args(void *ws, const WsLayout &w, float *loss, int B, int N, int L, int s_m, int s_n, int e_m, int e_n,
+                          const TailBwd *tb, const RrlCall &o) {
+    const int nblk = (L + 1023) / 1024;
+    TailArgs t;
+    t.lidc = w.u32(ws, RRL_WS_LIDC); t.dc = w.f32(ws, RRL_WS_VALS); t.blkcnt = w.i32(ws, RRL_WS_BLKCNT);
+    t.vlist = w.f32(ws, RRL_WS_VLIST); t.vlcnt = w.i32(ws, RRL_WS_VLCNT);
+    t.mhist = w.u32(ws, RRL_WS_MHIST); t.mctl = w.u32(ws, RRL_WS_MCTL);
+    t.msum = (unsigned long long *)w.i64(ws, RRL_WS_MSUM);
+    t.med_out = w.f32(ws, RRL_WS_MED); t.bcnt_out = w.i32(ws, RRL_WS_BCNT); t.bsum_out = w.i64(ws, RRL_WS_BSUM);
+    t.info = w.i32(ws, RRL_WS_INFO); t.loss = loss; t.status = w.i32(ws, RRL_WS_STATUS);
+    t.B = B; t.nblk = nblk; t.s_m = s_m; t.s_n = s_n; t.e_m = e_m; t.e_n = e_n;
+    t.do_bwd = tb ? 1 : 0; t.N = N; t.L = L; t.transpose_r = tb ? tb->transpose_r : 0;
+    t.hs1 = w.i32(ws, RRL_WS_HS1); t.w1 = w.f32(ws, RRL_WS_W1);
+    t.Q1 = (const float4 *)w.f32(ws, RRL_WS_Q1); t.Q2 = (const float4 *)w.f32(ws, RRL_WS_Q2);
+    t.grad_loss = tb ? tb->grad_loss : nullptr; t.src = tb ? tb->src : nullptr;
+    t.gR = tb ? tb->gR : nullptr; t.gt = tb ? tb->gt : nullptr; t.payload = tb ? tb->payload : nullptr;
+    t.grad_tri1 = tb ? tb->grad_tri1 : nullptr;
+    t.Bt = o.problems;
+    t.xcd_align = B % 8 == 0 && xcd_align_on();
+    t.chain = o.plan.leave_clean ? w.u32(ws, RRL_WS_CHAIN) : nullptr;
+    t.chain_flags = o.plan.fused_build;
+    t.spin_limit = rrl_chain_spin_limit();
+    return t;
+}
+
 static int loss_reduce_impl(void *ws, size_t ws_bytes, float *loss, int B, int N, int M, int L, int s_m, int s_n, int e_m,
                             int e_n, int pool, const TailBwd *tb, const RrlCall &o, void *stream) {
     if (!ws || !loss || B < 0 || N < 0 || M < 0 || L < 0) return RRL_E_ARG;
@@ -269,24 +304,7 @@
     if (B == 0) return 0;
     const int nblk = (L + 1023) / 1024;
     if (o.plan.reduce == RRL_RED_TAIL) {
-        TailArgs t;
-        t.lidc = w.u32(ws, RRL_WS_LIDC); t.dc = w.f32(ws, RRL_WS_VALS); t.blkcnt = w.i32(ws, RRL_WS_BLKCNT);
-        t.vlist = w.f32(ws, RRL_WS_VLIST); t.vlcnt = w.i32(ws, RRL_WS_VLCNT);
-        t.mhist = w.u32(ws, RRL_WS_MHIST); t.mctl = w.u32(ws, RRL_WS_MCTL);
-        t.msum = (unsigned long long *)w.i64(ws, RRL_WS_MSUM);
-        t.med_out = w.f32(ws, RRL_WS_MED); t.bcnt_out = w.i32(ws, RRL_WS_BCNT); t.bsum_out = w.i64(ws, RRL_WS_BSUM);
-        t.info = w.i32(ws, RRL_WS_INFO); t.loss = loss; t.status = w.i32(ws, RRL_WS_STATUS);
-        t.B = B; t.nblk = nblk; t.s_m = s_m; t.s_n = s_n; t.e_m = e_m; t.e_n = e_n;
-        t.do_bwd = tb ? 1 : 0; t.N = N; t.L = L; t.transpose_r = tb ? tb->transpose_r : 0;
-        t.hs1 = w.i32(ws, RRL_WS_HS1); t.w1 = w.f32(ws, RRL_WS_W1);
-        t.Q1 = (const float4 *)w.f32(ws, RRL_WS_Q1); t.Q2 = (const float4 *)w.f32(ws, RRL_WS_Q2);
-        t.grad_loss = tb ? tb->grad_loss : nullptr; t.src = tb ? tb->src : nullptr;
-        t.gR = tb ? tb->gR : nullptr; t.gt = tb ? tb->gt : nullptr; t.payload = tb ? tb->payload : nullptr;
-        t.grad_tri1 = tb ? tb->grad_tri1 : nullptr;
-        t.Bt = o.problems;
-        t.xcd_align = B % 8 == 0 && xcd_align_on();
-        t.chain = o.plan.leave_clean ? w.u32(ws, RRL_WS_CHAIN) : nullptr;
-        t.chain_flags = o.plan.fused_build;
+        const TailArgs t = tail_args(ws, w, loss, B, N, L, s_m, s_n, e_m, e_n, tb, o);
         if (tb && o.plan.write_rides) {
             RrlWriteRider *wr = o.write_rider;
             const int wtiles = (wr->n + 1023) / 1024;
@@ -463,7 +481,7 @@
     if (s_m < 1 || s_n < 1 || e_m > RRL_MAX_HITS + 1 || e_n > RRL_MAX_HITS + 1) return RRL_E_RANGE;
     if (o.tar_ws == ws) return RRL_E_ARG;
     const RrlPlan &p = o.plan;
-    if (o.chain_left) *o.chain_left = p.leave_clean | (p.fused_build << 1);
+    if (o.chain_left) *o.chain_left = p.leave_clean | (p.fused_build << 1) | (p.pair_tail << 2);
     o.tri1_in = tri1;
     int rc;
     RrlRange step("rrl forward");
@@ -499,6 +517,15 @@
         } else {
             hipLaunchKernelGGL(pair_reduce_kernel, dim3((unsigned)B), dim3(1024), sizeof(int) * 2, s, pa, ra);
         }
+        RRL_LAUNCH_CHECK();
+        return 0;
+    }
+    if (p.pair_tail) {
+        RrlRange r("K2 + K3 + K4 (one launch)");
+        WsLayout w(B, N, M, L);
+        if (ws_bytes < w.total) return RRL_E_WS;
+        launch_pair_tail(call_pair_args(tri1, tri2, line, ws, w, B, N, M, L, s_m, s_n, e_m, e_n, o),
+                         tail_args(ws, w, loss, B, N, L, s_m, s_n, e_m, e_n, tb, o), (hipStream_t)stream);
         RRL_LAUNCH_CHECK();
         return 0;
     }
diff --git a/a-robust-registration-loss_amd/csrc/rrl_stage_pair.inc b/a-robust-registration-loss_amd/csrc/rrl_stage_pair.inc
--- a/a-robust-registration-loss_amd/csrc/rrl_stage_pair.inc
+++ b/a-robust-registration-loss_amd/csrc/rrl_stage_pair.inc
@@ -1,4 +1,7 @@
 __device__ __forceinline__ void lds_barrier() { asm volatile("s_waitcnt lgkmcnt(0)\n\ts_barrier" ::: "memory"); }
+
+#define MCTL_PT_ARR 24
+#define MCTL_PT_TMO 25
 
 #include "rrl_arith.h"
 
@@ -53,6 +56,7 @@
     float *dc_lds;
 };
 
+template <bool PUB = false>
 __device__ __forceinline__ void pair_hit(const float *__restrict__ tri1, const float *__restrict__ tri2,
                                          const float *__restrict__ line, const int32_t *__restrict__ hit1,
                                          const int32_t *__restrict__ hit2, int32_t *__restrict__ hs1,
@@ -64,7 +68,7 @@
                                          int b, int N, int M, size_t gl, int k, int j, int sub, int st1,
                                          int st2, float *t2 ,
                                          int bi, size_t gli ,
-                                         PairKeep *keep = nullptr) {
+                                         PairKeep *keep = nullptr, const float *dc_base = nullptr ) {
     const int cloud = sub >> 2, a = sub & 3;
     const int cnt = cloud ? j : k;
     float q[3] = {0.0f, 0.0f, 0.0f};
@@ -89,11 +93,27 @@
         tri_coords(tb, cloud ? st2 : st1, f, c);
         hit_weights(c, ln, w);
         inter_point(c, w, q);
-        (cloud ? hs2 : hs1)[gl * RRL_MAX_HITS + a] = f;
-        (cloud ? Q2 : Q1)[gl * RRL_MAX_HITS + a] = make_float4(q[0], q[1], q[2], 0.0f);
         float *wd = (cloud ? w2 : w1) + (gl * RRL_MAX_HITS + a) * 3;
-#pragma unroll
-        for (int cc = 0; cc < 3; ++cc) wd[cc] = w[cc];
+        if constexpr (PUB) {
+            const float4 qv = make_float4(q[0], q[1], q[2], 0.0f);
+            const unsigned qo = (unsigned)((gl * RRL_MAX_HITS + a) * 16);
+            if (cloud) {
+                st16_sc1(rrl_rsrc(Q2, 0x7ffffff0u), qo, qv);
+                hs2[gl * RRL_MAX_HITS + a] = f;
+#pragma unroll
+                for (int cc = 0; cc < 3; ++cc) wd[cc] = w[cc];
+            } else {
+                st16_sc1(rrl_rsrc(Q1, 0x7ffffff0u), qo, qv);
+                __hip_atomic_store(&hs1[gl * RRL_MAX_HITS + a], f, __ATOMIC_RELAXED, __HIP_MEMORY_SCOPE_AGENT);
+#pragma unroll
+                for (int cc = 0; cc < 3; ++cc) st4_sc1(&wd[cc], w[cc]);
+            }
+        } else {
+            (cloud ? hs2 : hs1)[gl * RRL_MAX_HITS + a] = f;
+            (cloud ? Q2 : Q1)[gl * RRL_MAX_HITS + a] = make_float4(q[0], q[1], q[2], 0.0f);
+#pragma unroll
+            for (int cc = 0; cc < 3; ++cc) wd[cc] = w[cc];
+        }
         if (keep) {
             keep->f = f;
 #pragma unroll
@@ -118,7 +138,12 @@
             if (s_mh) atomicAdd(&s_mh[(__float_as_uint(sq) >> 20) & 2047u], 1u);
         }
     }
-    ((float2 *)dc_slot)[sub] = make_float2(t2[0], t2[1]);
+    if constexpr (PUB) {
+        const float o0 = __shfl_xor(t2[0], 1), o1 = __shfl_xor(t2[1], 1);
+        if (!(sub & 1)) st16_sc1(rrl_rsrc(dc_base, 0x7ffffff0u), (unsigned)((dc_slot - dc_base) * 4 + (sub >> 1) * 16), make_float4(t2[0], t2[1], o0, o1));
+    } else {
+        ((float2 *)dc_slot)[sub] = make_float2(t2[0], t2[1]);
+    }
 }
 
 __device__ __forceinline__ void xcd_sample_of(int lin, int gx, int &x, int &b) {
@@ -157,6 +182,7 @@
     int32_t *zc1, *zc2;
 };
 
+template <bool PUB = false>
 __device__ __forceinline__ void pair_body(const PairArgs &a, int b, int tile, int ntile, PairKeep *keep = nullptr) {
     __shared__ int s_list[1024];
     __shared__ int s_wave[16];
@@ -212,7 +238,10 @@
         keep->total = total; keep->k = keep->j = 0; keep->f = 0; keep->sq = s_q[tid >> 3];
         keep->w[0] = keep->w[1] = keep->w[2] = 0.0f; keep->q = make_float4(0.0f, 0.0f, 0.0f, 0.0f);
     }
-    if (tid == 0) a.blkcnt[(size_t)b * ntile + tile] = total;
+    if (tid == 0) {
+        if constexpr (PUB) __hip_atomic_store(&a.blkcnt[(size_t)b * ntile + tile], total, __ATOMIC_RELAXED, __HIP_MEMORY_SCOPE_AGENT);
+        else a.blkcnt[(size_t)b * ntile + tile] = total;
+    }
     float *vl = tally && a.vlist ? a.vlist + ((size_t)b * ntile + tile) * 16384 : nullptr;
     for (int r0 = 0; r0 < total; r0 += 128) {
         const int rank = r0 + (tid >> 3), sub = tid & 7;
@@ -225,11 +254,12 @@
             const size_t slot = (size_t)b * Lp + (size_t)tile * 1024 + rank;
             if (sub == 0) {
                 a.kjc[slot] = (uint8_t)(k | (j << 4));
-                if (a.lidc) a.lidc[slot] = e;
-            }
-            pair_hit(a.tri1, a.tri2, a.line, a.hit1, a.hit2, a.hs1, a.hs2, a.w1, a.w2, a.Q1, a.Q2, a.D, a.dc + slot * 16,
+                if constexpr (PUB) __hip_atomic_store(&a.lidc[slot], e, __ATOMIC_RELAXED, __HIP_MEMORY_SCOPE_AGENT);
+                else if (a.lidc) a.lidc[slot] = e;
+            }
+            pair_hit<PUB>(a.tri1, a.tri2, a.line, a.hit1, a.hit2, a.hs1, a.hs2, a.w1, a.w2, a.Q1, a.Q2, a.D, a.dc + slot * 16,
                      s_q[tid >> 3], tally ? s_mh : nullptr, b, a.N, a.M, gl, k, j, sub, a.st1, a.st2, t2, bi, (size_t)bi * L + l,
-                     r0 == 0 ? keep : nullptr);
+                     r0 == 0 ? keep : nullptr, a.dc);
             if (keep && r0 == 0) {
                 keep->k = k; keep->j = j;
                 if (keep->dc_lds) {
@@ -246,8 +276,13 @@
             if (lane == 63 && incl) wbase = atomicAdd(&s_nv, incl);
             wbase = (unsigned)__builtin_amdgcn_readlane((int)wbase, 63);
             unsigned at = wbase + incl - mine;
-            if (nvl & 1u) vl[at++] = t2[0];
-            if (nvl & 2u) vl[at] = t2[1];
+            if constexpr (PUB) {
+                if (nvl & 1u) st4_sc1(&vl[at++], t2[0]);
+                if (nvl & 2u) st4_sc1(&vl[at], t2[1]);
+            } else {
+                if (nvl & 1u) vl[at++] = t2[0];
+                if (nvl & 2u) vl[at] = t2[1];
+            }
         }
     }
     STAMP(2);
@@ -263,13 +298,24 @@
         if (tid < 16 && s_bc[tid]) atomicAdd(&a.mctl[(size_t)b * 64 + tid], s_bc[tid]);
         if (vl) {
             const unsigned nv = s_nv;
-            if (tid == 0) a.vlcnt[(size_t)b * ntile + tile] = (int)nv;
-            if (tid < ((4u - (nv & 3u)) & 3u)) vl[nv + tid] = -1.0f;
+            if constexpr (PUB) {
+                if (tid == 0) __hip_atomic_store(&a.vlcnt[(size_t)b * ntile + tile], (int)nv, __ATOMIC_RELAXED, __HIP_MEMORY_SCOPE_AGENT);
+                if (tid < ((4u - (nv & 3u)) & 3u)) st4_sc1(&vl[nv + tid], -1.0f);
+            } else {
+                if (tid == 0) a.vlcnt[(size_t)b * ntile + tile] = (int)nv;
+                if (tid < ((4u - (nv & 3u)) & 3u)) vl[nv + tid] = -1.0f;
+            }
         } else if (tid == 0 && a.vlcnt) {
             a.vlcnt[(size_t)b * ntile + tile] = -1;
         }
     }
     if (wave == 0) STAMPP(4);
+    if constexpr (PUB) {
+        asm volatile("s_waitcnt vmcnt(0)" ::: "memory");
+        __syncthreads();
+        if (tid == 0) __hip_atomic_fetch_add(&a.mctl[(size_t)b * 64 + MCTL_PT_ARR], 1u, __ATOMIC_RELAXED, __HIP_MEMORY_SCOPE_AGENT);
+        if (wave == 0) STAMPP(6);
+    }
     if (wave == 0) {
         const int base = __builtin_amdgcn_readfirstlane(base_reg);
         for (int i = lane; i < total; i += 64) a.sel_out[(size_t)b * L + base + i] = s_list[i] & 0xffffff;
diff --git a/a-robust-registration-loss_amd/csrc/rrl_stage_pairtail.inc b/a-robust-registration-loss_amd/csrc/rrl_stage_pairtail.inc
--- /dev/null
+++ b/a-robust-registration-loss_amd/csrc/rrl_stage_pairtail.inc
@@ -0,0 +1,53 @@
+#define PT_LANES 1024
+#define PT_LINES 64
+#define PT_SUBS 2
+typedef TailGeo<PT_LANES, PT_LINES, PT_SUBS, true> TailGeoOne;
+
+template <bool SCATTER>
+__global__ __launch_bounds__(PT_LANES) void pair_tail_kernel(const PairArgs pa, const TailArgs ta) {
+    const int nblk = ta.nblk, npair = nblk * ta.B, lin = (int)blockIdx.x;
+    if (lin < npair) {
+        int tile = lin % nblk, b = lin / nblk;
+        if (pa.xcd_align) xcd_sample_of(lin, nblk, tile, b);
+        pair_body<true>(pa, b, tile, nblk);
+        return;
+    }
+    const int l2 = lin - npair;
+    tail_body<SCATTER, 2, TailGeoOne>(ta, l2 % nblk, (l2 / nblk) % ta.B, l2 / npair);
+}
+
+static int g_pair_tail = -1;
+extern "C" int rrl_set_pair_tail(int on) {
+    if (on < -1 || on > 1) return RRL_E_ARG;
+    g_pair_tail = on;
+    return 0;
+}
+static bool pair_tail_on() {
+    if (g_pair_tail < 0) { const char *e = getenv("RRL_PAIR_TAIL"); g_pair_tail = e && e[0] == '0' ? 0 : 1; }
+    return g_pair_tail != 0;
+}
+static long pair_tail_capacity() {
+    static long cap[64];
+    int dev = 0;
+    if (hipGetDevice(&dev) != hipSuccess || dev < 0 || dev >= 64) return 0;
+    if (cap[dev] == 0) {
+        hipDeviceProp_t p;
+        int a = 0, c = 0;
+        long v = -1;
+        if (hipGetDeviceProperties(&p, dev) == hipSuccess &&
+            hipOccupancyMaxActiveBlocksPerMultiprocessor(&a, pair_tail_kernel<true>, PT_LANES, 0) == hipSuccess &&
+            hipOccupancyMaxActiveBlocksPerMultiprocessor(&c, pair_tail_kernel<false>, PT_LANES, 0) == hipSuccess && a > 0 && c > 0)
+            v = (long)p.multiProcessorCount * (a < c ? a : c);
+        cap[dev] = v;
+    }
+    return cap[dev] < 0 ? 0 : cap[dev];
+}
+static bool pair_tail_serves(int B, int nblk) {
+    return pair_tail_on() && nblk >= 2 && nblk <= TAIL_MAX_TILES && (long)B * nblk * (1 + PT_SUBS) <= pair_tail_capacity();
+}
+
+static void launch_pair_tail(const PairArgs &pa, const TailArgs &t, hipStream_t s) {
+    const dim3 g((unsigned)(t.nblk * t.B * (1 + PT_SUBS)));
+    if (t.grad_tri1) hipLaunchKernelGGL(pair_tail_kernel<true>, g, dim3(PT_LANES), 0, s, pa, t);
+    else hipLaunchKernelGGL(pair_tail_kernel<false>, g, dim3(PT_LANES), 0, s, pa, t);
+}
diff --git a/a-robust-registration-loss_amd/csrc/rrl_stage_tail.inc b/a-robust-registration-loss_amd/csrc/rrl_stage_tail.inc
--- a/a-robust-registration-loss_amd/csrc/rrl_stage_tail.inc
+++ b/a-robust-registration-loss_amd/csrc/rrl_stage_tail.inc
@@ -36,7 +36,26 @@
     int xcd_align;
     uint32_t *chain;
     int chain_flags;
+    unsigned spin_limit;
 };
+
+template <int LANES_, int LINES_, int SUBS_, bool ONE_>
+struct TailGeo {
+    static constexpr int LANES = LANES_, LINES = LINES_, SUBS = SUBS_;
+    static constexpr bool ONE = ONE_;
+};
+typedef TailGeo<TAIL_LANES, TAIL_LINES, TAIL_SUBS, false> TailGeoSep;
+
+template <bool SC1, typename T>
+__device__ __forceinline__ T ld4(const T *p) {
+    if constexpr (SC1) return __hip_atomic_load(p, __ATOMIC_RELAXED, __HIP_MEMORY_SCOPE_AGENT);
+    else return *p;
+}
+template <bool SC1>
+__device__ __forceinline__ float4 ld16(const void *base, size_t byte_off) {
+    if constexpr (SC1) return ld16_sc1(rrl_rsrc(base, 0x7ffffff0u), (unsigned)byte_off);
+    else return *(const float4 *)((const char *)base + byte_off);
+}
 
 
 __device__ __forceinline__ void tail_payload(const TailArgs &a, float lv) {
@@ -55,10 +74,12 @@
     tail_payload(t, lv);
 }
 
-template <bool SCATTER, int RPL>
+template <bool SCATTER, int RPL, typename G = TailGeoSep>
 __device__ __forceinline__ void tail_body(const TailArgs &a, int tile_in, int b_in, int sub) {
+    constexpr int LW = 4 * G::LINES / 64;
+    constexpr bool ONE = G::ONE;
     __shared__ unsigned s_vals[MCAND_CAP];
-    __shared__ unsigned s_wtot[TAIL_LANES / 64];
+    __shared__ unsigned s_wtot[G::LANES / 64];
     __shared__ unsigned s_pick[3];
     __shared__ unsigned s_whist[128];
     __shared__ unsigned long long s_sum[32];
@@ -68,9 +89,10 @@
     __shared__ int s_pref[TAIL_MAX_TILES + 1];
     __shared__ int s_vpref[TAIL_MAX_TILES + 1];
     __shared__ int s_misc[3];
-    __shared__ float s_red[4][12];
-    __shared__ unsigned s_scat[4][64 * SCAT_STRIDE];
-    constexpr int NW = TAIL_LANES / 64, BPL = 2048 / TAIL_LANES;
+    __shared__ float s_red[LW][12];
+    __shared__ unsigned s_scat[LW][64 * SCAT_STRIDE];
+    __shared__ unsigned s_tmo;
+    constexpr int NW = G::LANES / 64, BPL = 2048 / G::LANES;
     const int tid = threadIdx.x, lane = tid & 63, wave = tid >> 6;
     const int nblk = a.nblk;
     int tile = tile_in, b = b_in;
@@ -83,46 +105,95 @@
     const bool do_bwd = a.do_bwd != 0;
     constexpr bool scatter = SCATTER;
     if (wave == 0) STAMPW(0);
-
-    const int mycnt = a.blkcnt[(size_t)b * nblk + tile];
-    const int bc = tid < nblk ? a.blkcnt[(size_t)b * nblk + tid] : 0;
-    const int vraw = tid < nblk ? a.vlcnt[(size_t)b * nblk + tid] : 0;
+    float gl_in0 = 0.0f;
+    int st0 = 0;
+    bool chain_tmo = false;
+    auto load_indep = [&]() {
+        gl_in0 = do_bwd ? a.grad_loss[b] : 0.0f;
+        if (a.chain_flags) {
+            const uint4 cw = *(const uint4 *)(a.chain + 4 * (size_t)b);
+            st0 = (int)cw.y;
+            chain_tmo = cw.w != 0u;
+        } else {
+            st0 = a.status[0];
+        }
+    };
+    float med = 0.0f;
+    bool have_med = false;
+    if constexpr (ONE) {
+        load_indep();
+        if (tid == 0) {
+            bool ok = false;
+            for (unsigned it = 0; it < a.spin_limit; ++it) {
+                if (ld_agent(&ctl[MCTL_PT_ARR]) >= (unsigned)nblk) { ok = true; break; }
+                __builtin_amdgcn_s_sleep(1);
+            }
+            if (!ok) __hip_atomic_fetch_add(&ctl[MCTL_PT_TMO], 1u, __ATOMIC_RELAXED, __HIP_MEMORY_SCOPE_AGENT);
+            s_tmo = ok ? 0u : 1u;
+        }
+        lds_barrier();
+        if (wave == 0) STAMPP(7);
+        if (s_tmo) {
+            if (wave != 0) return;
+            unsigned last = 0;
+            if (lane == 0)
+                last = __hip_atomic_fetch_add(&ctl[MCTL_TICK2], 1u, __ATOMIC_RELAXED, __HIP_MEMORY_SCOPE_AGENT) == (unsigned)(nblk * G::SUBS - 1) ? 1u : 0u;
+            if (!__builtin_amdgcn_readfirstlane((int)last)) return;
+            if (lane < 32) {
+                a.bsum_out[(size_t)b * 32 + lane] = 0;
+                __hip_atomic_store(&a.msum[(size_t)b * 32 + lane], 0ull, __ATOMIC_RELAXED, __HIP_MEMORY_SCOPE_AGENT);
+            }
+            if (lane < 16) a.bcnt_out[b * 16 + lane] = 0;
+            if (lane == 0) {
+                a.med_out[b] = 0.0f;
+                a.loss[b] = __builtin_nanf("");
+                a.info[b * 4 + 0] = 0; a.info[b * 4 + 1] = 0; a.info[b * 4 + 2] = 0; a.info[b * 4 + 3] = st0;
+                st_agent(&ctl[MCTL_TICK2], 0u); st_agent(&ctl[MCTL_BAD], 0u); st_agent(&ctl[MCTL_MEDBITS], 0u); st_agent(&ctl[MCTL_PT_ARR], 0u);
+                if (a.chain) *(uint4 *)(a.chain + 4 * (size_t)b) = make_uint4(0u, 0u, 0u, 0u);
+                if (do_bwd && a.payload) tail_payload(a, __builtin_nanf(""));
+            }
+            return;
+        }
+    }
+
+    const int mycnt = ld4<ONE>(&a.blkcnt[(size_t)b * nblk + tile]);
+    const int bc = tid < nblk ? ld4<ONE>(&a.blkcnt[(size_t)b * nblk + tid]) : 0;
+    const int vraw = tid < nblk ? ld4<ONE>(&a.vlcnt[(size_t)b * nblk + tid]) : 0;
     const int vc = vraw > 0 ? (vraw + 3) >> 2 : 0;
     const int h = tid & 3;
-    int r = sub * TAIL_LINES + (tid >> 2);
+    int r = sub * G::LINES + (tid >> 2);
     unsigned kl_raw = 0u;
     float4 dr_raw = make_float4(INFINITY, INFINITY, INFINITY, INFINITY);
-    if (tid < 4 * TAIL_LINES) {
-        kl_raw = lidc[slot0 + r];
-        dr_raw = ((const float4 *)(dc + (slot0 + r) * 16))[h];
+    if (tid < 4 * G::LINES) {
+        kl_raw = ld4<ONE>(&lidc[slot0 + r]);
+        dr_raw = ld16<ONE>(dc, ((slot0 + r) * 16 + 4 * h) * sizeof(float));
     }
     unsigned hb[BPL];
     {
-        const uint4 hq = ((const uint4 *)(a.mhist + (size_t)b * 2048))[tid];
-        hb[0] = hq.x; hb[1] = hq.y; hb[2] = hq.z; hb[3] = hq.w;
-        static_assert(BPL == 4, "one 16-byte load of the histogram per lane");
-    }
-    const unsigned bkt = tid < 16 ? ctl[tid] : 0u;
-    const float gl_in0 = do_bwd ? a.grad_loss[b] : 0.0f;
-    int st0;
-    bool chain_tmo = false;
-    if (a.chain_flags) {
-        const uint4 cw = *(const uint4 *)(a.chain + 4 * (size_t)b);
-        st0 = (int)cw.y;
-        chain_tmo = cw.w != 0u;
-    } else {
-        st0 = a.status[0];
-    }
-    const int LPT = TAIL_LANES / nblk;
+        static_assert(BPL == 4 || (BPL == 2 && ONE), "one 16-byte load of the histogram per lane (8 bytes: the 1024-lane tail role)");
+        if constexpr (BPL == 4) {
+            const uint4 hq = ((const uint4 *)(a.mhist + (size_t)b * 2048))[tid];
+            hb[0] = hq.x; hb[1] = hq.y; hb[2] = hq.z; hb[3] = hq.w;
+        } else {
+            typedef unsigned int v2u_ __attribute__((ext_vector_type(2)));
+            const v2u_ hq = __builtin_amdgcn_raw_buffer_load_b64(rrl_rsrc(a.mhist + (size_t)b * 2048, 8192), tid * 8, 0, 16);
+            hb[0] = hq.x; hb[1] = hq.y;
+        }
+    }
+    const unsigned bkt = tid < 16 ? ld4<ONE>(&ctl[tid]) : 0u;
+    if constexpr (!ONE) load_indep();
+    const int LPT = G::LANES / nblk;
     const int vt = tid / LPT, vq = tid - vt * LPT;
     const bool vlane = vt < nblk;
-    const float4 *__restrict__ vbase = (const float4 *)(a.vlist + ((size_t)b * nblk + (vlane ? vt : 0)) * 16384);
+    const float *__restrict__ vsample = a.vlist + (size_t)b * nblk * 16384;
+    const size_t vboff = (size_t)(vlane ? vt : 0) * 16384 * sizeof(float);
     float4 vpre[RPL];
 #pragma unroll
     for (int u = 0; u < RPL; ++u)
-        vpre[u] = vlane ? vbase[vq + LPT * u] : make_float4(-1.0f, -1.0f, -1.0f, -1.0f);
-    if (sub * TAIL_LINES >= mycnt && !(tile == 0 && sub == 0)) return;
-    bool mine_on = tid < 4 * TAIL_LINES && r < mycnt;
+        vpre[u] = vlane ? ld16<ONE>(vsample, vboff + 16 * (size_t)(vq + LPT * u)) : make_float4(-1.0f, -1.0f, -1.0f, -1.0f);
+    if constexpr (!ONE)
+        if (sub * G::LINES >= mycnt && !(tile == 0 && sub == 0)) return;
+    bool mine_on = tid < 4 * G::LINES && r < mycnt;
     unsigned kl = mine_on ? kl_raw : 0u;
     float dr[4];
     dr[0] = mine_on ? dr_raw.x : INFINITY; dr[1] = mine_on ? dr_raw.y : INFINITY;
@@ -132,23 +203,83 @@
 #pragma unroll
         for (int q = 0; q < 4; ++q) dr[q] = INFINITY;
         if (mine_on) {
-            kl = lidc[slot0 + r];
-            const float4 v = ((const float4 *)(dc + (slot0 + r) * 16))[h];
+            kl = ld4<ONE>(&lidc[slot0 + r]);
+            const float4 v = ld16<ONE>(dc, ((slot0 + r) * 16 + 4 * h) * sizeof(float));
             dr[0] = v.x; dr[1] = v.y; dr[2] = v.z; dr[3] = v.w;
         }
     };
     const float gl_in = gl_in0;
+    auto finish = [&]() {
+    const int narrive = ONE ? nblk * G::SUBS : s_misc[0];
+    STAMPW(3);
+    if (lane < 32) {
+        const unsigned long long v = s_sum[lane];
+        if (v) atomicAdd(&a.msum[(size_t)b * 32 + lane], v);
+    }
+    if (lane == 32 && s_flag[1]) atomicOr(&ctl[MCTL_BAD], 1u);
+    if (ONE && lane == 33 && have_med) st_agent(&ctl[MCTL_MEDBITS], __float_as_uint(med));
+    asm volatile("s_waitcnt vmcnt(0)" ::: "memory");
+    STAMPW(4);
+    unsigned last = 0;
+    if (lane == 0)
+        last = __hip_atomic_fetch_add(&ctl[MCTL_TICK2], 1u, __ATOMIC_RELAXED, __HIP_MEMORY_SCOPE_AGENT) == (unsigned)(narrive - 1) ? 1u : 0u;
+    STAMPW(5);
+    if (!__builtin_amdgcn_readfirstlane((int)last)) return;
+
+    unsigned long long tot = 0ull;
+    unsigned anybad = 0u, medw = 0u, pt_tmo = 0u;
+    if (lane < 32) {
+        tot = __hip_atomic_load(&a.msum[(size_t)b * 32 + lane], __ATOMIC_RELAXED, __HIP_MEMORY_SCOPE_AGENT);
+        a.bsum_out[(size_t)b * 32 + lane] = (int64_t)tot;
+        __hip_atomic_store(&a.msum[(size_t)b * 32 + lane], 0ull, __ATOMIC_RELAXED, __HIP_MEMORY_SCOPE_AGENT);
+    } else if (lane < 48) {
+        a.bcnt_out[b * 16 + lane - 32] = s_cnt[lane - 32];
+    } else if (lane == 48) {
+        anybad = ld_agent(&ctl[MCTL_BAD]);
+    } else if (ONE && lane == 49) {
+        medw = ld_agent(&ctl[MCTL_MEDBITS]);
+    } else if (ONE && lane == 50) {
+        pt_tmo = ld_agent(&ctl[MCTL_PT_TMO]);
+    }
+    const bool bad = __builtin_amdgcn_readlane((int)anybad, 48) != 0 || (ONE && __builtin_amdgcn_readlane((int)pt_tmo, 50) != 0);
+    const float med_fin = ONE && !have_med ? __uint_as_float((unsigned)__builtin_amdgcn_readlane((int)medw, 49)) : med;
+    const unsigned long long trow = __shfl(tot, (2 * lane) & 63), tcol = __shfl(tot, (2 * lane + 1) & 63);
+    const BucketFinal f = bucket_final(trow, tcol, lane < 16 ? s_cnt[lane] : 0, lane, a.s_m, a.s_n, a.e_m, a.e_n);
+    STAMPW(11);
+    if (lane == 0) {
+        const float accl = f.acc;
+        const int Cn = f.C, nselected = f.nselected, nvalues = f.nvalues;
+        const float lv = bad || chain_tmo ? __builtin_nanf("") : (Cn ? accl / (float)Cn : 0.0f);
+        a.med_out[b] = med_fin;
+        a.loss[b] = lv;
+        a.info[b * 4 + 0] = Cn;
+        a.info[b * 4 + 1] = nselected;
+        a.info[b * 4 + 2] = nvalues;
+        a.info[b * 4 + 3] = st0;
+        st_agent(&ctl[MCTL_TICK2], 0u); st_agent(&ctl[MCTL_BAD], 0u);
+        if (ONE) { st_agent(&ctl[MCTL_MEDBITS], 0u); st_agent(&ctl[MCTL_PT_ARR], 0u); }
+        if (a.chain) *(uint4 *)(a.chain + 4 * (size_t)b) = make_uint4(0u, 0u, 0u, 0u);
+        if (do_bwd && a.payload && Cn > 0) tail_payload(a, lv);
+    }
+    STAMPW(6);
+    };
     if (tid < 32) s_sum[tid] = 0ull;
     if (tid < 2) s_flag[tid] = 0u;
     if (tid == 0) s_ncand = 0u;
     if (tid < 16) s_cnt[tid] = (int)bkt;
     __builtin_amdgcn_fence(__ATOMIC_ACQ_REL, "wavefront");
+    if constexpr (ONE) {
+        if (sub * G::LINES >= mycnt) {
+            if (wave == 0) finish();
+            return;
+        }
+    }
     if (vraw < 0) atomicOr(&s_flag[1], 1u);
     if (wave == 0) {
         const int incl = wave_incl_scan(bc), vincl = wave_incl_scan(vc);
         if (lane < nblk) { s_pref[lane + 1] = incl; s_vpref[lane + 1] = vincl; }
         if (lane == 0) { s_pref[0] = 0; s_vpref[0] = 0; }
-        const int wl = min((bc + TAIL_LINES - 1) / TAIL_LINES, TAIL_SUBS);
+        const int wl = min((bc + G::LINES - 1) / G::LINES, G::SUBS);
         const int nl = wave_sum_i(lane < nblk ? (lane == 0 && wl == 0 ? 1 : wl) : 0);
         const int vm = (int)wave_max((float)vc);
         const int kk = lane / 4 + 1, jj = (lane & 3) + 1;
@@ -172,14 +303,14 @@
         for (int o = 0; o < RRL_MAX_HITS; ++o) { qx[o] = qy[o] = qz[o] = 0.0f; }
         if (bwd_live) {
             const size_t gl = (size_t)b * a.L + (kl & 0xffffffu);
-            fhit = a.hs1[gl * 4 + h];
-            q1 = a.Q1[gl * 4 + h];
+            fhit = ld4<ONE>(&a.hs1[gl * 4 + h]);
+            q1 = ld16<ONE>(a.Q1, (gl * 4 + h) * 16);
             const float *w = a.w1 + (gl * 4 + h) * 3;
 #pragma unroll
-            for (int q = 0; q < 3; ++q) wq[q] = w[q];
+            for (int q = 0; q < 3; ++q) wq[q] = ld4<ONE>(&w[q]);
 #pragma unroll
             for (int o = 0; o < RRL_MAX_HITS; ++o)
-                if (o < j) { const float4 t = a.Q2[gl * 4 + o]; qx[o] = t.x; qy[o] = t.y; qz[o] = t.z; }
+                if (o < j) { const float4 t = ld16<ONE>(a.Q2, (gl * 4 + o) * 16); qx[o] = t.x; qy[o] = t.y; qz[o] = t.z; }
         }
     };
     auto request_source = [&]() {
@@ -195,7 +326,7 @@
     lds_barrier();
     if (wave == 0) STAMPW(8);
     const int myvc = vlane ? s_vpref[vt + 1] - s_vpref[vt] : 0;
-    const int nlive = s_misc[0], vmax = s_misc[1];
+    const int vmax = s_misc[1];
 
     auto pick_bin = [&](unsigned rank_in, bool have_rank) -> unsigned {
         unsigned tsum = 0;
@@ -249,7 +380,7 @@
             for (int u = 0; u < RPL; ++u) {
                 const int g = g0 + vq + LPT * u;
                 v[u] = make_float4(-1.0f, -1.0f, -1.0f, -1.0f);
-                if (g < myvc) v[u] = pre && g0 == 0 ? vpre[u] : vbase[g];
+                if (g < myvc) v[u] = pre && g0 == 0 ? vpre[u] : ld16<ONE>(vsample, vboff + 16 * (size_t)g);
             }
             if (first) { after_issue(); first = false; }
             fn(v);
@@ -294,7 +425,7 @@
             const unsigned dmask = (1u << width) - 1u;
             lds_barrier();
 #pragma unroll
-            for (int q = 0; q < BPL; ++q) s_vals[tid + TAIL_LANES * q] = 0u;
+            for (int q = 0; q < BPL; ++q) s_vals[tid + G::LANES * q] = 0u;
             lds_barrier();
             const unsigned pre = prefix;
             stream_rows(false, [&]() {}, [&](const float4 *v) {
@@ -310,71 +441,26 @@
             rk = s_pick[1];
         }
     }
-    const float med = __uint_as_float(prefix);
+    med = __uint_as_float(prefix);
+    have_med = true;
     if (wave == 0) STAMPW(2);
 
     const int C = s_misc[2];
-    auto finish = [&]() {
-    STAMPW(3);
-    if (lane < 32) {
-        const unsigned long long v = s_sum[lane];
-        if (v) atomicAdd(&a.msum[(size_t)b * 32 + lane], v);
-    }
-    if (lane == 32 && s_flag[1]) atomicOr(&ctl[MCTL_BAD], 1u);
-    asm volatile("s_waitcnt vmcnt(0)" ::: "memory");
-    STAMPW(4);
-    unsigned last = 0;
-    if (lane == 0)
-        last = __hip_atomic_fetch_add(&ctl[MCTL_TICK2], 1u, __ATOMIC_RELAXED, __HIP_MEMORY_SCOPE_AGENT) == (unsigned)(nlive - 1) ? 1u : 0u;
-    STAMPW(5);
-    if (!__builtin_amdgcn_readfirstlane((int)last)) return;
-
-    unsigned long long tot = 0ull;
-    unsigned anybad = 0u;
-    if (lane < 32) {
-        tot = __hip_atomic_load(&a.msum[(size_t)b * 32 + lane], __ATOMIC_RELAXED, __HIP_MEMORY_SCOPE_AGENT);
-        a.bsum_out[(size_t)b * 32 + lane] = (int64_t)tot;
-        __hip_atomic_store(&a.msum[(size_t)b * 32 + lane], 0ull, __ATOMIC_RELAXED, __HIP_MEMORY_SCOPE_AGENT);
-    } else if (lane < 48) {
-        a.bcnt_out[b * 16 + lane - 32] = s_cnt[lane - 32];
-    } else if (lane == 48) {
-        anybad = ld_agent(&ctl[MCTL_BAD]);
-    }
-    const bool bad = __builtin_amdgcn_readlane((int)anybad, 48) != 0;
-    const unsigned long long trow = __shfl(tot, (2 * lane) & 63), tcol = __shfl(tot, (2 * lane + 1) & 63);
-    const BucketFinal f = bucket_final(trow, tcol, lane < 16 ? s_cnt[lane] : 0, lane, a.s_m, a.s_n, a.e_m, a.e_n);
-    STAMPW(11);
-    if (lane == 0) {
-        const float accl = f.acc;
-        const int Cn = f.C, nselected = f.nselected, nvalues = f.nvalues;
-        const float lv = bad || chain_tmo ? __builtin_nanf("") : (Cn ? accl / (float)Cn : 0.0f);
-        a.med_out[b] = med;
-        a.loss[b] = lv;
-        a.info[b * 4 + 0] = Cn;
-        a.info[b * 4 + 1] = nselected;
-        a.info[b * 4 + 2] = nvalues;
-        a.info[b * 4 + 3] = st0;
-        st_agent(&ctl[MCTL_TICK2], 0u); st_agent(&ctl[MCTL_BAD], 0u);
-        if (a.chain) *(uint4 *)(a.chain + 4 * (size_t)b) = make_uint4(0u, 0u, 0u, 0u);
-        if (do_bwd && a.payload && Cn > 0) tail_payload(a, lv);
-    }
-    STAMPW(6);
-    };
-    const bool single_chunk = mycnt <= TAIL_SUBS * TAIL_LINES;
+    const bool single_chunk = mycnt <= G::SUBS * G::LINES;
     float acc[12];
 #pragma unroll
     for (int q = 0; q < 12; ++q) acc[q] = 0.0f;
-    for (int chunk = sub;; chunk += TAIL_SUBS) {
+    for (int chunk = sub;; chunk += G::SUBS) {
     if (chunk != sub) {
-        r = chunk * TAIL_LINES + (tid >> 2);
-        mine_on = tid < 4 * TAIL_LINES && r < mycnt;
+        r = chunk * G::LINES + (tid >> 2);
+        mine_on = tid < 4 * G::LINES && r < mycnt;
         load_line();
         request_line();
         request_source();
     }
     int arg_b_own = 0, arg_a[4] = {0, 0, 0, 0};
     float er[4] = {0.0f, 0.0f, 0.0f, 0.0f};
-    if (wave < 4) {
+    if (wave < LW) {
         const int jmax = (int)wave_max((float)j);
         float wr[4];
 #pragma unroll
@@ -478,11 +564,11 @@
         }
         }
     }
-    if (scatter && wave < 4)
+    if (scatter && wave < LW)
         wave_scatter_rows(sc_live, sv, (unsigned)fhit, a.grad_tri1 + (size_t)b * a.N * 9, nullptr, s_scat[wave], lane);
-    if ((chunk + TAIL_SUBS) * TAIL_LINES >= mycnt) break;
-    }
-    if (do_bwd && !scatter && wave < 4) {
+    if ((chunk + G::SUBS) * G::LINES >= mycnt) break;
+    }
+    if (do_bwd && !scatter && wave < LW) {
 #pragma unroll
         for (int q = 0; q < 12; ++q) acc[q] = wave_sum(acc[q]);
         if (lane == 0)
@@ -495,7 +581,9 @@
 #endif
     if (wave == 1 && do_bwd && !scatter && mycnt > 0 && lane < 12) {
         const int q = lane;
-        const float v = (s_red[0][q] + s_red[1][q]) + (s_red[2][q] + s_red[3][q]);
+        float v = (s_red[0][q] + s_red[1][q]) + (s_red[2][q] + s_red[3][q]);
+        if constexpr (LW == 8) v += (s_red[4][q] + s_red[5][q]) + (s_red[6][q] + s_red[7][q]);
+        static_assert(LW == 4 || LW == 8, "the sum above");
         int o = q;
         if (q < 9 && a.transpose_r) o = (q % 3) * 3 + q / 3;
         if (q < 9) atomicAdd(&a.gR[b * 9 + o], v); else atomicAdd(&a.gt[b * 3 + (q - 9)], v);
diff --git a/a-robust-registration-loss_amd/csrc/rrl_ws.h b/a-robust-registration-loss_amd/csrc/rrl_ws.h
--- a/a-robust-registration-loss_amd/csrc/rrl_ws.h
+++ b/a-robust-registration-loss_amd/csrc/rrl_ws.h
@@ -118,6 +118,7 @@
     int leave_clean;
     int fused_build;
     int count_rides, write_rides;
+    int pair_tail;
 };
 struct RrlCall {
     int flags;
diff --git a/a-robust-registration-loss_amd/rrl_hip/_lib.py b/a-robust-registration-loss_amd/rrl_hip/_lib.py
--- a/a-robust-registration-loss_amd/rrl_hip/_lib.py
+++ b/a-robust-registration-loss_amd/rrl_hip/_lib.py
@@ -43,6 +43,7 @@
     "rrl_set_scan_variant": [_I],
     "rrl_demo_epoch": [_P, _P],
     "rrl_set_spin_limit": [_c.c_longlong],
+    "rrl_set_pair_tail": [_I],
     "rrl_debug_occupy": [_I, _I, _c.c_longlong, _P],
     "rrl_set_deterministic": [_I],
     "rrl_set_reduce_mode": [_I],
diff --git a/a-robust-registration-loss_amd/rrl_hip/ops.py b/a-robust-registration-loss_amd/rrl_hip/ops.py
--- a/a-robust-registration-loss_amd/rrl_hip/ops.py
+++ b/a-robust-registration-loss_amd/rrl_hip/ops.py
@@ -403,7 +403,7 @@
               scan_variant=None, counters=None, chamfer=None, payload=None, problems=None, chain=0, chain_left=None):
     if order1 is None and order2 is None and not target_kept and reduce_mode is None and deterministic is None \
             and sort_parts is None and scan_variant is None and counters is None and chamfer is None and payload is None \
-            and not problems and not chain:
+            and not problems and not chain and chain_left is None:
         return None
     o = _lib.Opts(flags=(_lib.F_TARGET_KEPT if target_kept else 0) | int(chain),
                   chain_left=ctypes.addressof(chain_left) if chain_left is not None else None,
@@ -928,6 +928,7 @@
         self._chain_left = ctypes.c_int32(0)
         self._chain_ready = False
         self.fused = False
+        self.pair_tail = False
         self.order1 = self.order2 = None
         if self.prepared:
             self.order1 = _check_order(src_order, Bt, N, dev, "src_order") if src_order is not None else cloud_order(self.src)
@@ -939,6 +940,7 @@
 
     def _set_opts(self):
         kw = dict(order1=self.order1, order2=self.order2, **self._extra)
+        kw.setdefault("chain_left", self._chain_left)
         self._opts = make_opts(**kw)
         self._opts_kept = make_opts(target_kept=True, **kw) if self.prepared else self._opts
         self._optr, self._optr_kept = _optr(self._opts), _optr(self._opts_kept)
@@ -967,6 +969,7 @@
         self._kept_key = key
         self._chain_ready = self.prepared and bool(self._chain_left.value & 1)
         self.fused = bool(self._chain_left.value & 2)
+        self.pair_tail = bool(self._chain_left.value & 4)
         self.st.counts_cleared = self._chain_ready
         _IntersectionLoss.last_state = self.st
         if self.ride is not None:
@@ -1133,6 +1136,10 @@
     check(_lib.load().rrl_set_spin_limit(int(1 << 18 if polls is None else polls)), "rrl_set_spin_limit")
 
 
+def set_pair_tail(on):
+    check(_lib.load().rrl_set_pair_tail(-1 if on is None else int(bool(on))), "rrl_set_pair_tail")
+
+
 def debug_occupy(workgroups, lanes, seconds, stream=None):
     dev = require_gpu()
     raw = ctypes.c_void_p(stream.cuda_stream) if stream is not None else _stream(dev)
diff --git a/include/rrl.h b/include/rrl.h
--- a/include/rrl.h
+++ b/include/rrl.h
@@ -235,6 +235,7 @@
 int rrl_set_sort_parts(int parts);
 
 int rrl_set_spin_limit(long long polls);
+int rrl_set_pair_tail(int on);
 int rrl_debug_occupy(int workgroups, int lanes, long long ticks, void *stream);
 
 int rrl_set_scan_variant(int lines_per_lane);
```

Result: slower. 43890 billion, median of 2 (-1.6%).
